# XuZhang1211/PVPUFormer

Hardware: AMD Instinct MI355X
Metric: 448x448 images/sec fwd+bwd, ViT-B VPUFormer (higher is better)
Workload: dtype bf16

## Files before the change

### include/vpu_hip.h

```cpp
#ifndef VPU_HIP_H
#define VPU_HIP_H
#include <stdint.h>

#ifdef __cplusplus
extern "C" {
#endif

#define VPU_BF16 0
#define VPU_F32 1

#define VPU_EPI_BIAS 1
#define VPU_EPI_PREACT 2
#define VPU_EPI_GELU 4
#define VPU_EPI_RELU 8
#define VPU_EPI_DGELU 16
#define VPU_EPI_DRELU 32
#define VPU_EPI_RESID 64
#define VPU_EPI_AFFINE 128
#define VPU_EPI_ACCUM 256
#define VPU_EPI_OUT_F32 512
#define VPU_EPI_SAVE_DGELU 1024
#define VPU_EPI_MULAUX 2048

typedef struct vpu_gemm_desc {
    const void* A;
    const void* B;
    void* C;
    const float* bias;
    const void* resid;
    const void* aux;
    void* preact;
    int32_t M, N, K;
    int32_t lda, ldb, ldc, ldr, ldaux;
    int32_t batch, inner;
    int64_t sAo, sAi, sBo, sBi, sCo, sCi, sRo, sRi;
    int32_t transA, transB;
    int32_t dtype, flags;
    int32_t resid_period;
    float alpha, post_mul, post_add;
    void* workspace;
    int64_t workspace_bytes;
    float* colsum;
    int32_t cs_tn, cs_t0;
    int64_t cs_ld;
} vpu_gemm_desc;

#define VPU_GEMM_GROUP_MAX 16
typedef struct vpu_gemm_group {
    int32_t n;
    int32_t start[VPU_GEMM_GROUP_MAX + 1];
    vpu_gemm_desc d[VPU_GEMM_GROUP_MAX];
} vpu_gemm_group;

const char* vpu_last_error(void);
int vpu_abi_version(void);

int vpu_gemm(const vpu_gemm_desc* d, void* stream);
int vpu_gemm_set_option(const char* name, int32_t value);
int vpu_gemm_get_option(const char* name, int32_t* value);
const char* vpu_gemm_last_kernel(void);
int vpu_gemm_grouped(const vpu_gemm_desc* d, int32_t n, void* stream);

int vpu_layernorm_fwd(const void* x, const float* w, const float* b, void* y, float* mean, float* rstd,
                      int64_t rows, int32_t C, float eps, int32_t dtype, void* stream);
int vpu_layernorm_bwd_nblk(int64_t rows);
int vpu_layernorm_bwd(const void* dy, const void* x, const float* w, const float* mean, const float* rstd,
                      const void* dres, void* dx, float* part, int64_t rows, int32_t C, int32_t dtype, void* stream);
int vpu_layernorm_fwd_pe(const void* x, const float* w, const float* b, void* y, float* mean, float* rstd,
                         int64_t rows, int32_t C, float eps, const void* pe, int64_t pe_rows, void* y2,
                         int32_t dtype, void* stream);
int vpu_layernorm_bwd2(const void* dy, const void* dy2, const void* x, const float* w, const float* mean,
                       const float* rstd, const void* dres, void* dx, float* part, int64_t rows, int32_t C,
                       int32_t dtype, void* stream);
#define VPU_COLSUM_BATCH_MAX 64
typedef struct vpu_colsum_job { const float* in; float* out; int32_t nrows, ncols, row_len, out_ld; } vpu_colsum_job;
typedef struct vpu_colsum_batch { vpu_colsum_job job[VPU_COLSUM_BATCH_MAX]; } vpu_colsum_batch;
int vpu_colsum_batched(const vpu_colsum_job* jobs, int32_t n, void* stream);
int vpu_colsum_f32(const float* in, float* out, int64_t rows, int32_t C, float beta, void* stream);
int vpu_colsum(const void* in, int32_t ld, float* out, float* part, int64_t rows, int32_t C, float beta,
               int32_t dtype, void* stream);
int vpu_softmax_fwd(const float* S, int32_t lds, void* P, int32_t ldp, int64_t rows, int32_t ncols,
                    int32_t dtype, void* stream);
int vpu_softmax_bwd(const void* P, int32_t ldp, const float* dP, int32_t lddp, void* dS, int64_t rows,
                    int32_t ncols, float scale, int32_t dtype, void* stream);
int vpu_l2norm_fwd(const void* x, void* y, float* inv, int64_t rows, int32_t C, int32_t dtype, void* stream);
int vpu_l2norm_bwd(const void* dy, const void* y, const float* inv, void* dx, int64_t rows, int32_t C,
                   int32_t dtype, void* stream);

int vpu_attn_fwd(const void* q, const void* k, const void* v, void* out, float* lse, int32_t nb, int32_t H, int32_t n,
                 int32_t hd, int32_t ld, int32_t ldo, float scale, void* stream);
int vpu_attn_bwd(const void* q, const void* k, const void* v, const void* o, const void* d_o, const float* lse,
                 float* delta, void* dq, void* dk, void* dv, int32_t nb, int32_t H, int32_t n, int32_t hd, int32_t ld,
                 int32_t ldo, int32_t ldg, float scale, void* stream);
int vpu_attn_set_option(const char* name, int32_t value);
const char* vpu_attn_last_kernel(void);
int vpu_xattn_fwd(const void* q, const void* k, const void* v, void* out, float* lse, int32_t nb, int32_t H, int32_t nq,
                  int32_t nk, int32_t hd, int32_t ldq, int32_t ldk, int32_t ldo, float scale, void* stream);
int vpu_xattn_bwd(const void* q, const void* k, const void* v, const void* o, const void* d_o, const float* lse,
                  float* delta, void* dq, void* dk, void* dv, int32_t nb, int32_t H, int32_t nq, int32_t nk, int32_t hd,
                  int32_t ldq, int32_t ldk, int32_t ldo, int32_t ldgq, int32_t ldgk, float scale, void* stream);
int vpu_xattn_fwd_split(const void* q, const void* k, const void* v, void* out, float* lse, int32_t nb, int32_t H, int32_t nq,
                        int32_t nk, int32_t hd, int32_t ldq, int32_t ldk, int32_t ldo, float scale, int32_t qdiv, int32_t kdiv,
                        void* stream);
int vpu_xattn_bwd_split(const void* q, const void* k, const void* v, const void* o, const void* d_o, const float* lse,
                        float* delta, void* dq, void* dk, void* dv, int32_t nb, int32_t H, int32_t nq, int32_t nk, int32_t hd,
                        int32_t ldq, int32_t ldk, int32_t ldo, int32_t ldgq, int32_t ldgk, float scale, int32_t qdiv, int32_t kdiv,
                        void* stream);
int vpu_attn_combine(const void* o_s, const float* lse_s, void* out, float* lse, int32_t nb, int32_t H, int32_t nq, int32_t hd,
                     int32_t S, int32_t ld_s, int32_t ldo, void* stream);
int vpu_sum_groups(const void* in, void* out, int64_t G, int32_t S, int64_t n, int32_t dtype, void* stream);

int vpu_add_bcast(const void* a, const void* b, void* out, int64_t n, int64_t period_b, int32_t dtype, void* stream);
int vpu_add4(const void* a, const void* b, const void* c, const void* d, void* out, int64_t n, int32_t dtype,
             void* stream);
int vpu_fanout_add(const void* src, void* const* dst, const int32_t* accum, int32_t ndst, int64_t n, int32_t dtype, void* stream);
int vpu_cast2d(const void* src, int32_t src_dtype, int64_t ld_src, void* dst, int32_t dst_dtype, int64_t ld_dst,
               int64_t rows, int32_t cols, int32_t cols_pad, void* stream);
typedef struct vpu_cast_job {
    const float* src;
    const float* src2;
    void* dst;
    int64_t ld_src, ld_dst, rows;
    int32_t cols, cols_pad, dst_dtype, perm_g, perm_wg;
} vpu_cast_job;
int vpu_cast2d_batched(const vpu_cast_job* jobs, int32_t n, void* stream);
int vpu_dropout_mask(float* out, int32_t n, float keep, uint64_t seed, uint64_t* state, void* stream);
int vpu_fill_f32(float* p, float v, int64_t n, void* stream);
int vpu_fill_ranges_f32(float* base, const int64_t* off, const int64_t* len, int32_t n, float v, void* stream);
int vpu_debug_spin(float* sink, int32_t wgs, int64_t cycles, void* stream);
int vpu_debug_gemm_times(void* dev_buf);
int vpu_sigmoid_to_channel(const float* logits, float* out, int32_t B, int64_t HW, int32_t channels, int32_t channel,
                           void* stream);
int vpu_act_bwd(const void* dy, int64_t ld_dy, const void* aux, int64_t ld_aux, void* dz, int64_t ld_dz, int64_t rows,
                int32_t cols, int32_t kind, int32_t dtype, void* stream);

int vpu_pue_encode(const float* points, const int32_t* boxes, const float* lut, void* out, double* out64,
                   int32_t B, int32_t n, int32_t num_max, int32_t img, int32_t ld, int32_t dtype, void* stream);
int vpu_pue_scribble_rows(const float* points, const double* vec, void* out, double* out64, int32_t B, int32_t n,
                          int32_t num_max, int32_t img, int32_t ld, int32_t dtype, void* stream);
int vpu_draw_polyline(const int32_t* curve, float* disks, int32_t B, int32_t P, int32_t H, int32_t W, void* stream);
int vpu_pue_encode_rows(const float* points, const int32_t* kinds, const int32_t* boxes, const double* vec, const float* lut,
                        void* out, double* out64, int32_t B, int32_t n, int32_t num_max, int32_t img, int32_t ld,
                        int32_t dtype, void* stream);
int vpu_draw_prompt_rows(const int32_t* kinds, const int32_t* boxes, const int32_t* curve, const int32_t* counts, float* disks,
                         int32_t B, int32_t Pmax, int32_t n, int32_t H, int32_t W, void* stream);
int vpu_edt(const uint8_t* mask, int32_t* scratch, float* dist, int32_t B, int32_t H, int32_t W, int32_t zero_border,
            void* stream);
int vpu_chamfer5(const uint8_t* mask, int32_t* scratch, float* dist, int32_t B, int32_t H, int32_t W, int32_t zero_border,
                 void* stream);
int vpu_mask_bbox(const float* prob, float thr, const int32_t* pos_clicks, int32_t nclicks, int32_t* out, int32_t B,
                  int32_t H, int32_t W, void* stream);
int vpu_error_masks(const uint8_t* pred, const uint8_t* gt, const uint8_t* valid, uint8_t* out, int32_t H, int32_t W,
                    void* stream);
int vpu_masked_argmax(const float* dist, const uint8_t* keep, uint64_t* out, int32_t planes, int32_t H, int32_t W,
                      void* stream);
typedef struct vpu_eval_obj {
    const float* image;
    const float* prev;
    float* canvas;
    uint8_t* mask;
    const uint8_t* gt;
    const uint8_t* valid;
    uint8_t* keep;
    int64_t* out;
    int32_t H, W, r0, r1, c0, c1, src, clear_at;
} vpu_eval_obj;
int vpu_roi_resize_batched(const vpu_eval_obj* objs, int32_t n, float* out, int32_t S_h, int32_t S_w, int32_t flip,
                           int32_t channels, void* stream);
int vpu_roi_paste_batched(const vpu_eval_obj* objs, int32_t n, const float* probs, int32_t S_h, int32_t S_w, float pred_thr,
                          float box_thr, int32_t max_hw, void* stream);
int vpu_click_keys_batched(const vpu_eval_obj* objs, int32_t n, uint8_t* err, int32_t* scratch, float* dist, int32_t Hm,
                           int32_t Wm, int32_t max_hw, void* stream);
typedef struct vpu_session_obj {
    float* canvas;
    uint64_t* bits;
    int32_t* rec;
    int32_t H, W, r0, r1, c0, c1, src, reserved;
} vpu_session_obj;
int vpu_session_paste_batched(const vpu_session_obj* objs, int32_t n, const float* probs, int32_t S_h, int32_t S_w,
                              float pred_thr, float box_thr, int32_t max_hw, int32_t form, void* stream);
typedef struct vpu_annot_obj {
    const float* add;
    float* total;
    uint16_t* labels;
    uint64_t* bits;
    int32_t* rec;
    int32_t H, W, label, mode;
} vpu_annot_obj;
int vpu_annot_compose_batched(const vpu_annot_obj* objs, int32_t n, float thr, int32_t max_hw, void* stream);
int vpu_label_extract(uint16_t* labels, float* out, int32_t* rec, int32_t H, int32_t W, int32_t label, void* stream);
typedef struct vpu_runs_obj {
    const void* src;
    int32_t H, W, kind;
    float thr;
} vpu_runs_obj;
#define VPU_RUNS_BAND_ROWS 64
#define VPU_RUNS_COLS 64
int vpu_runs_count_batched(const vpu_runs_obj* objs, const vpu_runs_obj* host_objs, int32_t n, int32_t* scratch,
                           int64_t scratch_len, int32_t* header, void* stream);
int vpu_runs_write_batched(const vpu_runs_obj* objs, const vpu_runs_obj* host_objs, int32_t n, const int32_t* scratch,
                           int64_t scratch_len, int32_t* entries, int32_t cap, void* stream);
typedef struct vpu_unrun_obj {
    void* dst;
    const int32_t* entries;
    int32_t H, W, n_runs, kind, label, pad;
} vpu_unrun_obj;
int vpu_runs_decode_batched(const vpu_unrun_obj* objs, const vpu_unrun_obj* host_objs, int32_t n, void* stream);
#define VPU_TIDY_ALL 0
#define VPU_TIDY_SEEDED 1
#define VPU_TIDY_LARGEST 2
#define VPU_TIDY_SCRATCH_INTS(hw) (3 * (int64_t)(hw) + 4)
// ... 141 lines not shown
```

### pvpuformer_amd/_lib.py

```python
import ctypes as C
import os

_HERE = os.path.dirname(os.path.abspath(__file__))
LIB_PATH = os.path.join(_HERE, os.environ.get("VPU_LIB_FILE") or
                        ("libvpu_hip_diag.so" if os.environ.get("VPU_LIB_DIAG", "0") == "1" else "libvpu_hip.so"))

BF16, F32 = 0, 1

EPI_BIAS, EPI_PREACT, EPI_GELU, EPI_RELU, EPI_DGELU, EPI_DRELU = 1, 2, 4, 8, 16, 32
EPI_RESID, EPI_AFFINE, EPI_ACCUM, EPI_OUT_F32 = 64, 128, 256, 512
EPI_SAVE_DGELU, EPI_MULAUX = 1024, 2048


class GemmDesc(C.Structure):
    _fields_ = [
        ("A", C.c_void_p), ("B", C.c_void_p), ("C", C.c_void_p), ("bias", C.c_void_p), ("resid", C.c_void_p),
        ("aux", C.c_void_p), ("preact", C.c_void_p),
        ("M", C.c_int32), ("N", C.c_int32), ("K", C.c_int32),
        ("lda", C.c_int32), ("ldb", C.c_int32), ("ldc", C.c_int32), ("ldr", C.c_int32), ("ldaux", C.c_int32),
        ("batch", C.c_int32), ("inner", C.c_int32),
        ("sAo", C.c_int64), ("sAi", C.c_int64), ("sBo", C.c_int64), ("sBi", C.c_int64),
        ("sCo", C.c_int64), ("sCi", C.c_int64), ("sRo", C.c_int64), ("sRi", C.c_int64),
        ("transA", C.c_int32), ("transB", C.c_int32), ("dtype", C.c_int32), ("flags", C.c_int32),
        ("resid_period", C.c_int32),
        ("alpha", C.c_float), ("post_mul", C.c_float), ("post_add", C.c_float),
        ("workspace", C.c_void_p), ("workspace_bytes", C.c_int64), ("colsum", C.c_void_p),
        ("cs_tn", C.c_int32), ("cs_t0", C.c_int32), ("cs_ld", C.c_int64),
    ]


_P, _I, _L, _F = C.c_void_p, C.c_int32, C.c_int64, C.c_float

class ColsumJob(C.Structure):
    _fields_ = [("inp", C.c_void_p), ("out", C.c_void_p), ("nrows", C.c_int32), ("ncols", C.c_int32),
                ("row_len", C.c_int32), ("out_ld", C.c_int32)]


class CastJob(C.Structure):
    _fields_ = [("src", C.c_void_p), ("src2", C.c_void_p), ("dst", C.c_void_p), ("ld_src", C.c_int64), ("ld_dst", C.c_int64),
                ("rows", C.c_int64), ("cols", C.c_int32), ("cols_pad", C.c_int32), ("dst_dtype", C.c_int32),
                ("perm_g", C.c_int32), ("perm_wg", C.c_int32)]


class EvalObj(C.Structure):
    _fields_ = [("image", C.c_void_p), ("prev", C.c_void_p), ("canvas", C.c_void_p), ("mask", C.c_void_p),
                ("gt", C.c_void_p), ("valid", C.c_void_p), ("keep", C.c_void_p), ("out", C.c_void_p),
                ("H", C.c_int32), ("W", C.c_int32), ("r0", C.c_int32), ("r1", C.c_int32), ("c0", C.c_int32),
                ("c1", C.c_int32), ("src", C.c_int32), ("clear_at", C.c_int32)]


class BoxRow(C.Structure):
    _fields_ = [("prev", C.c_void_p), ("gt", C.c_void_p), ("valid", C.c_void_p),
                ("H", C.c_int32), ("W", C.c_int32), ("r0", C.c_int32), ("r1", C.c_int32), ("c0", C.c_int32),
                ("c1", C.c_int32), ("mirror", C.c_int32), ("n_obj", C.c_int32)]


class SessionObj(C.Structure):
    _fields_ = [("canvas", C.c_void_p), ("bits", C.c_void_p), ("rec", C.c_void_p),
                ("H", C.c_int32), ("W", C.c_int32), ("r0", C.c_int32), ("r1", C.c_int32), ("c0", C.c_int32),
                ("c1", C.c_int32), ("src", C.c_int32), ("reserved", C.c_int32)]


class AnnotObj(C.Structure):
    _fields_ = [("add", C.c_void_p), ("total", C.c_void_p), ("labels", C.c_void_p), ("bits", C.c_void_p), ("rec", C.c_void_p),
                ("H", C.c_int32), ("W", C.c_int32), ("label", C.c_int32), ("mode", C.c_int32)]


class RunsObj(C.Structure):
    _fields_ = [("src", C.c_void_p), ("H", C.c_int32), ("W", C.c_int32), ("kind", C.c_int32), ("thr", C.c_float)]


class UnrunObj(C.Structure):
    _fields_ = [("dst", C.c_void_p), ("entries", C.c_void_p), ("H", C.c_int32), ("W", C.c_int32), ("n_runs", C.c_int32),
                ("kind", C.c_int32), ("label", C.c_int32), ("pad", C.c_int32)]


class OutlineObj(C.Structure):
    _fields_ = [("src", C.c_void_p), ("H", C.c_int32), ("W", C.c_int32), ("kind", C.c_int32), ("thr", C.c_float),
                ("label", C.c_int32), ("pad", C.c_int32)]


class TidyObj(C.Structure):
    _fields_ = [("add", C.c_void_p), ("total", C.c_void_p), ("add_out", C.c_void_p), ("total_out", C.c_void_p),
                ("bits", C.c_void_p), ("rec", C.c_void_p), ("seeds", C.c_void_p), ("scratch", C.c_void_p),
                ("H", C.c_int32), ("W", C.c_int32), ("n_seeds", C.c_int32), ("min_area", C.c_int32), ("max_hole", C.c_int32),
                ("keep", C.c_int32), ("pad0", C.c_int32), ("pad1", C.c_int32)]


SIGNATURES = {
    "vpu_gemm": [C.POINTER(GemmDesc), _P],
    "vpu_layernorm_fwd": [_P, _P, _P, _P, _P, _P, _L, _I, _F, _I, _P],
    "vpu_layernorm_bwd_nblk": [_L],
    "vpu_layernorm_bwd": [_P, _P, _P, _P, _P, _P, _P, _P, _L, _I, _I, _P],
    "vpu_layernorm_fwd_pe": [_P, _P, _P, _P, _P, _P, _L, _I, _F, _P, _L, _P, _I, _P],
    "vpu_layernorm_bwd2": [_P, _P, _P, _P, _P, _P, _P, _P, _P, _L, _I, _I, _P],
    "vpu_colsum_batched": [C.POINTER(ColsumJob), _I, _P],
    "vpu_colsum_f32": [_P, _P, _L, _I, _F, _P],
    "vpu_colsum": [_P, _I, _P, _P, _L, _I, _F, _I, _P],
    "vpu_softmax_fwd": [_P, _I, _P, _I, _L, _I, _I, _P],
    "vpu_softmax_bwd": [_P, _I, _P, _I, _P, _L, _I, _F, _I, _P],
    "vpu_l2norm_fwd": [_P, _P, _P, _L, _I, _I, _P],
    "vpu_l2norm_bwd": [_P, _P, _P, _P, _L, _I, _I, _P],
    "vpu_attn_fwd": [_P, _P, _P, _P, _P, _I, _I, _I, _I, _I, _I, _F, _P],
    "vpu_attn_bwd": [_P, _P, _P, _P, _P, _P, _P, _P, _P, _P, _I, _I, _I, _I, _I, _I, _I, _F, _P],
    "vpu_xattn_fwd": [_P, _P, _P, _P, _P, _I, _I, _I, _I, _I, _I, _I, _I, _F, _P],
    "vpu_xattn_bwd": [_P, _P, _P, _P, _P, _P, _P, _P, _P, _P, _I, _I, _I, _I, _I, _I, _I, _I, _I, _I, _F, _P],
    "vpu_xattn_fwd_split": [_P, _P, _P, _P, _P, _I, _I, _I, _I, _I, _I, _I, _I, _F, _I, _I, _P],
    "vpu_xattn_bwd_split": [_P, _P, _P, _P, _P, _P, _P, _P, _P, _P, _I, _I, _I, _I, _I, _I, _I, _I, _I, _I, _F, _I, _I, _P],
    "vpu_attn_combine": [_P, _P, _P, _P, _I, _I, _I, _I, _I, _I, _I, _P],
    "vpu_sum_groups": [_P, _P, _L, _I, _L, _I, _P],
    "vpu_add_bcast": [_P, _P, _P, _L, _L, _I, _P],
    "vpu_add4": [_P, _P, _P, _P, _P, _L, _I, _P],
    "vpu_cast2d": [_P, _I, _L, _P, _I, _L, _L, _I, _I, _P],
    "vpu_cast2d_batched": [C.POINTER(CastJob), _I, _P],
    "vpu_fanout_add": [_P, C.POINTER(C.c_void_p), C.POINTER(C.c_int32), _I, _L, _I, _P],
    "vpu_dropout_mask": [_P, _I, _F, C.c_uint64, _P, _P],
    "vpu_fill_f32": [_P, _F, _L, _P],
    "vpu_fill_ranges_f32": [_P, C.POINTER(C.c_int64), C.POINTER(C.c_int64), _I, _F, _P],
    "vpu_debug_spin": [_P, _I, _L, _P],
    "vpu_debug_gemm_times": [_P],
    "vpu_sigmoid_to_channel": [_P, _P, _I, _L, _I, _I, _P],
    "vpu_act_bwd": [_P, _L, _P, _L, _P, _L, _L, _I, _I, _I, _P],
    "vpu_pue_encode": [_P, _P, _P, _P, _P, _I, _I, _I, _I, _I, _I, _P],
    "vpu_cc_roots": [_P, _P, _I, _I, _I, _P],
    "vpu_cc_table": [_P, _P, _P, _I, _I, _I, _I, _P],
    "vpu_edt": [_P, _P, _P, _I, _I, _I, _I, _P],
    "vpu_chamfer5": [_P, _P, _P, _I, _I, _I, _I, _P],
    "vpu_pue_scribble_rows": [_P, _P, _P, _P, _I, _I, _I, _I, _I, _I, _P],
    "vpu_draw_polyline": [_P, _P, _I, _I, _I, _I, _P],
    "vpu_pue_encode_rows": [_P, _P, _P, _P, _P, _P, _P, _I, _I, _I, _I, _I, _I, _P],
    "vpu_draw_prompt_rows": [_P, _P, _P, _P, _P, _I, _I, _I, _I, _I, _P],
    "vpu_mask_bbox": [_P, _F, _P, _I, _P, _I, _I, _I, _P],
    "vpu_masked_argmax": [_P, _P, _P, _I, _I, _I, _P],
    "vpu_error_masks": [_P, _P, _P, _P, _I, _I, _P],
    "vpu_roi_resize_batched": [_P, _I, _P, _I, _I, _I, _I, _P],
    "vpu_roi_paste_batched": [_P, _I, _P, _I, _I, _F, _F, _I, _P],
    "vpu_session_paste_batched": [_P, _I, _P, _I, _I, _F, _F, _I, _I, _P],
    "vpu_annot_compose_batched": [_P, _I, _F, _I, _P],
    "vpu_label_extract": [_P, _P, _P, _I, _I, _I, _P],
    "vpu_runs_count_batched": [_P, _P, _I, _P, _L, _P, _P],
    "vpu_runs_write_batched": [_P, _P, _I, _P, _L, _P, _I, _P],
    "vpu_runs_decode_batched": [_P, _P, _I, _P],
    "vpu_regions_tidy_batched": [_P, _P, _I, _F, _P],
    "vpu_outline_count_batched": [_P, _P, _I, _P, _L, _P, _P],
    "vpu_outline_trace_batched": [_P, _P, _I, _P, _L, _P, _P, _P, _L, _P, _I, _P, _I, _P, _P],
    "vpu_outline_simplify_batched": [_P, _P, _P, _I, _I, _I, _I, _I, _P, _L, _P, _I, _P, _I, _P, _P, _P],
    "vpu_click_keys_batched": [_P, _I, _P, _P, _P, _I, _I, _I, _P],
    "vpu_box_prompts_batched": [_P, _I, _P, _I, _I, _I, _F, _P, _P, _P, _P, _P, _I, _P, _P, _P],
    "vpu_crops_gather": [_P, _P, _P, _P, _I, _I, _I, _I, _I, _I, _I, _P],
    "vpu_crops_blend": [_P, _P, _P, _P, _I, _I, _I, _I, _I, _I, _P],
    "vpu_disk_maps": [_P, _P, _P, _I, _I, _I, _I, _F, _P],
    "vpu_patch_im2col": [_P, _P, _P, _I, _I, _I, _I, _I, _I, _P],
    "vpu_patch_im2col_prenorm": [_P, _P, _P, _I, _I, _I, _I, _I, _I, _P],
    "vpu_patch_im2col_floor": [_P, _P, _P, _I, _I, _I, _I, _I, _I, _I, _P],
    "vpu_window_permute": [_P, _P, _I, _I, _I, _I, _I, _I, _P],
    "vpu_space_to_depth2_crop": [_P, _P, _I, _I, _I, _I, _I, _P],
    "vpu_pixel_shuffle2": [_P, _P, _P, _I, _I, _I, _I, _I, _I, _P],
    "vpu_pixel_shuffle2_gn_stats": [_P, _P, _P, _P, _I, _I, _I, _I, _I, _P],
    "vpu_groupnorm_apply": [_P, _P, _P, _P, _P, _P, _P, _I, _L, _I, _F, _I, _I, _P],
    "vpu_pixel_unshuffle2_nblk": [_I],
    "vpu_pixel_unshuffle2_sums": [_P, _P, _P, _I, _I, _I, _I, _I, _P],
    "vpu_groupnorm_nchunk": [],
    "vpu_groupnorm_fwd": [_P, _P, _P, _P, _P, _P, _P, _I, _L, _I, _F, _I, _I, _P],
    "vpu_groupnorm_bwd": [_P, _P, _P, _P, _P, _P, _P, _P, _P, _I, _L, _I, _I, _I, _P],
    "vpu_bilinear_cl_fwd": [_P, _I, _P, _I, _I, _I, _I, _I, _I, _I, _I, _P],
    "vpu_bilinear_cl_bwd": [_P, _I, _P, _I, _I, _I, _I, _I, _I, _I, _I, _P],
    "vpu_head_grad_fused": [_P, _P, _P, _P, _P, _P, _P, _P, _P, _P, _L, _L, _I, _I, _P],
    "vpu_upsum_relu": [_P, C.POINTER(C.c_void_p), C.POINTER(C.c_int32), C.POINTER(C.c_int32), _I, _I, _I, _I, _I, _I, _P],
    "vpu_gate_stats": [_P, _P, _P, _P, _P, _P, _I, _I, _I, _I, _I, _P],
    "vpu_gate_apply": [_P, _P, _P, _P, _I, _I, _I, _I, _P],
    "vpu_gate_bwd": [_P, _P, _P, _P, _P, _P, _P, _I, _P, _P, _P, _I, _I, _I, _I, _I, _P],
    "vpu_gate_fwd_n": [C.POINTER(C.c_void_p), C.POINTER(C.c_void_p), _P, C.POINTER(C.c_void_p), _P, _P, _P, _P, _I, _I, _I, _I, _I, _I, _P],
    "vpu_gate_bwd_n": [C.POINTER(C.c_void_p), _P, _P, _P, _P, _P, _P, _I, C.POINTER(C.c_void_p), C.POINTER(C.c_void_p), _P, _I, _I, _I,
                       _I, _I, _I, _P],
    "vpu_convseg_fwd": [_P, _P, _P, _P, _P, _L, _L, _I, _I, _P],
    "vpu_convseg_bwd_nblk": [_L],
    "vpu_convseg_bwd": [_P, _P, _P, _P, _P, _I, _P, _P, _L, _L, _I, _I, _P],
    "vpu_upsample_ac_fwd": [_P, _P, _L, _I, _I, _I, _I, _P],
    "vpu_upsample_ac_bwd": [_P, _P, _L, _I, _I, _I, _I, _P],
    "vpu_p2cl_fwd_bwd": [_P, _P, _P, _P, _P, _P, _F, _I, _I, _I, _I, _P],
    "vpu_p2cl_up_nband": [_I, _I],
    "vpu_p2cl_up_fwd_bwd": [_P, _P, _P, _P, _P, _P, _F, _I, _I, _I, _I, _I, _I, _P],
    "vpu_nfl_dice_scratch_doubles": [_I],
    "vpu_nfl_dice_fwd_bwd": [_P, _P, _P, _P, _P, _F, _F, _I, _L, _P],
    "vpu_loss_finalize": [_P, _P, _I, _I, C.c_double, _F, _F, _F, _F, _P, _P],
    "vpu_adam_step": [_P, _P, _P, _P, _P, _L, _F, _F, _F, _F, _F, _I, _F, _P],
    "vpu_adam_step_groups": [_P, _P, _P, _P, _P, _L, _P, _P, _P, _I, _F, _F, _F, _I, _I, _F, _P],
    "vpu_adam_step_hyper": [_P, _P, _P, _P, _P, _L, _P, _P, _P, _P, _I, _F, _F, _F, _F, _I, _P],
    "vpu_gemm_set_option": [C.c_char_p, _I],
    "vpu_gemm_get_option": [C.c_char_p, C.POINTER(C.c_int32)],
    "vpu_gemm_last_kernel": [],
    "vpu_attn_last_kernel": [],
    "vpu_attn_set_option": [C.c_char_p, _I],
    "vpu_gemm_grouped": [C.POINTER(GemmDesc), _I, _P],
    "vpu_last_error": [],
    "vpu_abi_version": [],
}
_RET = {"vpu_last_error": C.c_char_p, "vpu_gemm_last_kernel": C.c_char_p, "vpu_attn_last_kernel": C.c_char_p}

_lib = None

# ... 29 lines not shown
```

### pvpuformer_amd/csrc/gemm.hip

```cpp
#include <stdio.h>
#include <stdlib.h>
#include <string.h>
#include <atomic>
#include "vpu_common.h"
#include "../../include/vpu_hip.h"
#include "gemm_tiles.h"

int vpu_k5_option();
void vpu_k5_set_option(int v);
void vpu_k5_set_grid(int v);
void vpu_k5_set_split(int v);
void vpu_k5_set_noepi(int v);
int vpu_k5_launch(const vpu_gemm_desc* d, int rb, int ncu, int vec, void* stream, char* name, size_t name_len);
#ifdef VPU_DIAG
void vpu_k5_set_dbg(unsigned long long* p);
#endif

namespace {


template <typename T>
__device__ __forceinline__ void epilogue_store(const vpu_gemm_desc& p, int64_t coff, int64_t roff, int m, int n,
                                               float acc) {
    const int flags = p.flags;
// ... 417 lines not shown
    if (CS && TA == 1 && p.colsum != nullptr && tile_n == 0) {
        float* red = reinterpret_cast<float*>(lds);
        if (do_cs && fr == 0) {
#pragma unroll
            for (int i = 0; i < 4; ++i)
#pragma unroll
                for (int r = 0; r < 4; ++r) red[wm * 64 + i * 16 + fq * 4 + r] = acc_cs[i][r];
        }
        __syncthreads();
        if (tid < 128 && m0 + tid < p.M) {
            const float t = red[tid];
            if (splitk > 1) {
                float* cp = ws + (int64_t)nbatch * splitk * p.M * p.N + ((int64_t)z * splitk + split) * p.M + m0 + tid;
                if (SLAB && cnt) __hip_atomic_store(cp, t, __ATOMIC_RELAXED, __HIP_MEMORY_SCOPE_AGENT);
                else *cp = t;
            } else p.colsum[m0 + tid] += t;
        }
        __syncthreads();
    }
    const __amdgpu_buffer_rsrc_t rws = __builtin_amdgcn_make_buffer_rsrc(wsz, 0, 0x7FFFFFFF, 0x00020000);
#pragma unroll
    for (int pass = 0; pass < 2; ++pass) {
#pragma unroll
        for (int ii = 0; ii < 2; ++ii)
#pragma unroll
            for (int j = 0; j < 4; ++j)
#pragma unroll
                for (int r = 0; r < 4; ++r) {
                    const int row = ii * 16 + fq * 4 + r;
                    wl[row * 64 + ((j * 16 + fr) ^ (fq << 4))] = acc[pass * 2 + ii][j][r];
                }
        asm volatile("s_waitcnt lgkmcnt(0)" ::: "memory");
#pragma unroll
        for (int t = 0; t < 4; ++t) {
            const int u = lane + 64 * t;
            const int row = u >> 3, c8 = (u & 7) * 8;
            const int m = m0 + wm * 64 + pass * 32 + row;
            const int n = n0 + wn * 64 + c8;
            if (SLAB) {
                if (m < p.M && n < p.N) {
                    float v[8];
                    load8(wl + row * 64 + (c8 ^ (((row >> 2) & 3) << 4)), v);
                    if (cnt) store8_sc1(rws, (m * p.N + n) * 4, v);
                    else store8(wsz + (int64_t)m * p.N + n, v);
                }
            } else if (!GEN) {
                if (m < p.M && n < p.N) {
                    float v[8];
                    load8(wl + row * 64 + (c8 ^ (((row >> 2) & 3) << 4)), v);
                    EpiPre e;
                    e.has_pre = use_pre; e.has_bias = use_bias8; e.pre = pre[pass][t];
#pragma unroll
                    for (int j = 0; j < 8; ++j) e.bias[j] = bias8[j];
                    epilogue_store8(p, FLG, coff, roff, m, n, v, e);
                }
            } else if (m < p.M && n < p.N) {
                float v[8];
                load8(wl + row * 64 + (c8 ^ (((row >> 2) & 3) << 4)), v);
                if (splitk > 1) {
                    float* o = wsz + (int64_t)m * p.N + n;
                    if ((p.N & 3) == 0 && n + 8 <= p.N) store8(o, v);
                    else
                        for (int j = 0; j < 8 && n + j < p.N; ++j) o[j] = v[j];
                } else if (vec == 8) {
                    float tsum = 0.f;
#pragma unroll
                    for (int j = 0; j < 8; ++j) tsum += v[j];
                    if (tsum == 1.2345678e30f) reinterpret_cast<float*>(p.C)[0] = tsum;
                } else if (vec && n + 8 <= p.N) {
                    {
                        EpiPre e;
                        e.has_pre = use_pre; e.has_bias = use_bias8; e.pre = pre[pass][t];
#pragma unroll
                        for (int j = 0; j < 8; ++j) e.bias[j] = bias8[j];
                        epilogue_store8(p, FLG, coff, roff, m, n, v, e);
                    }
                } else {
                    for (int j = 0; j < 8 && n + j < p.N; ++j) epilogue_store<bf16_t>(p, coff, roff, m, n + j, v[j]);
                }
            }
        }
        asm volatile("s_waitcnt lgkmcnt(0)" ::: "memory");
    }
    if constexpr (SLAB) {
        if (cnt) {
            asm volatile("s_waitcnt vmcnt(0)" ::: "memory");
            __syncthreads();
            unsigned* flag = reinterpret_cast<unsigned*>(lds);
            unsigned* tc = cnt + (int64_t)z * ntiles + tile_lin;
            if (tid == 0) *flag = __hip_atomic_fetch_add(tc, 1u, __ATOMIC_RELAXED, __HIP_MEMORY_SCOPE_AGENT);
            __syncthreads();
            const bool last = *flag == (unsigned)(splitk - 1);
            if (last) {
                if (tid == 0) __hip_atomic_store(tc, 0u, __ATOMIC_RELAXED, __HIP_MEMORY_SCOPE_AGENT);
                __builtin_amdgcn_fence(__ATOMIC_ACQUIRE, "wavefront");
                const int64_t mn = (int64_t)p.M * p.N;
#pragma unroll
                for (int pass = 0; pass < 2; ++pass)
#pragma unroll
                    for (int t = 0; t < 4; ++t) {
                        const int u = lane + 64 * t;
                        const int row = u >> 3, c8 = (u & 7) * 8;
                        const int m = m0 + wm * 64 + pass * 32 + row;
                        const int n = n0 + wn * 64 + c8;
                        if (m < p.M && n < p.N) {
                            float v[8] = {0.f, 0.f, 0.f, 0.f, 0.f, 0.f, 0.f, 0.f};
                            for (int sl = 0; sl < splitk; ++sl) {
                                const unsigned long long* sp = reinterpret_cast<const unsigned long long*>(
                                    ws + ((int64_t)z * splitk + sl) * mn + (int64_t)m * p.N + n);
#pragma unroll
                                for (int j = 0; j < 4; ++j) {
                                    const unsigned long long q = __hip_atomic_load(sp + j, __ATOMIC_RELAXED, __HIP_MEMORY_SCOPE_AGENT);
                                    v[2 * j] += __builtin_bit_cast(float, (unsigned)(q & 0xFFFFFFFFull));
                                    v[2 * j + 1] += __builtin_bit_cast(float, (unsigned)(q >> 32));
                                }
                            }
                            if (vec) {
                                EpiPre e;
                                e.has_pre = false; e.has_bias = false; e.pre = make_uint4(0, 0, 0, 0);
                                epilogue_store8(p, p.flags, coff, roff, m, n, v, e);
                            } else {
                                for (int j = 0; j < 8; ++j) epilogue_store<bf16_t>(p, coff, roff, m, n + j, v[j]);
                            }
                        }
                    }
                if (CS && TA == 1 && p.colsum != nullptr && tile_n == 0 && tid < 128 && m0 + tid < p.M) {
                    const float* wb = ws + (int64_t)nbatch * splitk * mn + (int64_t)z * splitk * p.M + m0 + tid;
                    float t = 0.f;
                    for (int sl = 0; sl < splitk; ++sl)
                        t += __hip_atomic_load(wb + (int64_t)sl * p.M, __ATOMIC_RELAXED, __HIP_MEMORY_SCOPE_AGENT);
                    p.colsum[m0 + tid] += t;
                }
            }
            __syncthreads();
        }
    }
    __builtin_amdgcn_s_barrier();
    }
}

template <int TA, int TB, bool DMA, bool CS, int FL, int RING = 0>
__global__ __launch_bounds__(256, 2) void gemm_bf16_kernel(const vpu_gemm_desc p, const int tiles_n, const int splitk,
                                                        const int kchunk, float* __restrict__ ws, const int vec_in,
                                                        const int tiles_m_arg, const int nbatch,
                                                        unsigned* __restrict__ cnt) {
    gemm_bf16_body<TA, TB, DMA, CS, FL, RING, false>(p, nullptr, tiles_n, splitk, kchunk, ws, vec_in, tiles_m_arg, nbatch, cnt);
}
template <int TA, int TB, bool CS>
__global__ __launch_bounds__(256, 2) void gemm_bf16_grouped_kernel(const vpu_gemm_group ga, const int vec_in) {
    gemm_bf16_body<TA, TB, true, CS, -1, 0, true>(ga.d[0], &ga, 0, 1, 0, nullptr, vec_in, 0, 1, nullptr);
}

constexpr int BM2 = 256;
constexpr int STAGE2 = 3 * TILE_BYTES;

template <int TA, int TB>
__global__ __launch_bounds__(512) void gemm_bf16_big_kernel(const vpu_gemm_desc p, const int tiles_n, const int splitk,
                                                            const int kchunk, float* __restrict__ ws, const int vec) {
    extern __shared__ __attribute__((aligned(16))) char lds[];
    const int tid = threadIdx.x, lane = tid & 63;
    const int wave = __builtin_amdgcn_readfirstlane(tid >> 6);
    const int wm = wave >> 1, wn = wave & 1;
    int tile_m, tile_n;
    tile_coords(blockIdx.x, gridDim.x, tiles_n, tile_m, tile_n);
    const int m0 = tile_m * BM2, n0 = tile_n * BN;
    const int z = blockIdx.z, zo = z / p.inner, zi = z % p.inner;
    const bf16_t* A = reinterpret_cast<const bf16_t*>(p.A) + zo * p.sAo + zi * p.sAi;
    const bf16_t* B = reinterpret_cast<const bf16_t*>(p.B) + zo * p.sBo + zi * p.sBi;
    const int64_t coff = zo * p.sCo + zi * p.sCi;
    const int64_t roff = zo * p.sRo + zi * p.sRi;
    const int kbeg = blockIdx.y * kchunk;
    const int kend = (kbeg + kchunk < p.K) ? kbeg + kchunk : p.K;
    const __amdgpu_buffer_rsrc_t rA = __builtin_amdgcn_make_buffer_rsrc(const_cast<bf16_t*>(A), 0, 0x7FFFFFFF, 0x00020000);
    const __amdgpu_buffer_rsrc_t rB = __builtin_amdgcn_make_buffer_rsrc(const_cast<bf16_t*>(B), 0, 0x7FFFFFFF, 0x00020000);

    const int FLG = p.flags;
    const bool use_pre = false && vec == 1 && splitk == 1 &&
                         (p.flags & (VPU_EPI_RESID | VPU_EPI_MULAUX | VPU_EPI_DGELU | VPU_EPI_DRELU)) != 0 &&
                         !((p.flags & VPU_EPI_RESID) && (p.flags & (VPU_EPI_MULAUX | VPU_EPI_DGELU | VPU_EPI_DRELU)));
    uint4 pre[2][4];
    if (use_pre) prefetch_epi(p, FLG, coff, roff, m0 + wm * 64, n0 + wn * 64, lane, pre);

    f32x4_t acc[4][4];
#pragma unroll
    for (int i = 0; i < 4; ++i)
#pragma unroll
        for (int j = 0; j < 4; ++j) acc[i][j] = (f32x4_t){0.f, 0.f, 0.f, 0.f};
    const bool do_cs = TA == 1 && p.colsum != nullptr && tile_n == 0 && wn == 0;
    f32x4_t acc_cs[4];
#pragma unroll
    for (int i = 0; i < 4; ++i) acc_cs[i] = (f32x4_t){0.f, 0.f, 0.f, 0.f};
    bf16x8_t ones;
#pragma unroll
    for (int j = 0; j < 8; ++j) ones[j] = (bf16_t)(((lane & 15) == 0) ? 1.0f : 0.0f);

    auto issue = [&](int kt_, char* st) {
        const int k0 = kbeg + kt_ * BK;
#pragma unroll
        for (int i = 0; i < 6; ++i) {
            const int pc = wave + 8 * i;
            if (i < 4) stage_piece<TA>(rA, p.lda, m0 + (pc >> 4) * 128, p.M, k0, kend, st + (pc >> 4) * TILE_BYTES, pc & 15, lane);
            else stage_piece<TB>(rB, p.ldb, n0, p.N, k0, kend, st + 2 * TILE_BYTES, pc - 32, lane);
        }
    };
    const int nk = (kend - kbeg + BK - 1) / BK;
    char* s0 = lds;
    char* s1 = lds + STAGE2;
    char* s2 = lds + 2 * STAGE2;
    issue(0, s0);
    if (nk > 1) {
        issue(1, s1);
        asm volatile("s_waitcnt vmcnt(6)" ::: "memory");
    } else {
// ... 1388 lines not shown
    const int64_t coff = zo * p.sCo + zi * p.sCi;
    const int64_t roff = zo * p.sRo + zi * p.sRi;

    f32x4_t acc[2][2];
#pragma unroll
    for (int i = 0; i < 2; ++i)
#pragma unroll
        for (int j = 0; j < 2; ++j) acc[i][j] = (f32x4_t){0.f, 0.f, 0.f, 0.f};
    const int fr = lane & 15, fq = lane >> 4;
    const int nk = (p.K + FK - 1) / FK;
    for (int kt = 0; kt < nk; ++kt) {
        f32_stage<TA>(A, p.lda, m0, p.M, kt * FK, p.K, ldsA, tid);
        f32_stage<TB>(B, p.ldb, n0, p.N, kt * FK, p.K, ldsB, tid);
        __syncthreads();
#pragma unroll
        for (int ks = 0; ks < 4; ++ks) {
            const int k = ks * 4 + fq;
            float a[2], b[2];
#pragma unroll
            for (int i = 0; i < 2; ++i) a[i] = ldsA[k * FLD + wm * 32 + i * 16 + fr];
#pragma unroll
            for (int j = 0; j < 2; ++j) b[j] = ldsB[k * FLD + wn * 32 + j * 16 + fr];
#pragma unroll
            for (int i = 0; i < 2; ++i)
#pragma unroll
                for (int j = 0; j < 2; ++j)
                    acc[i][j] = __builtin_amdgcn_mfma_f32_16x16x4f32(a[i], b[j], acc[i][j], 0, 0, 0);
        }
        __syncthreads();
    }
#pragma unroll
    for (int i = 0; i < 2; ++i)
#pragma unroll
        for (int r = 0; r < 4; ++r) {
            const int m = m0 + wm * 32 + i * 16 + fq * 4 + r;
            if (m >= p.M) continue;
#pragma unroll
            for (int j = 0; j < 2; ++j) {
                const int n = n0 + wn * 32 + j * 16 + fr;
                if (n < p.N) epilogue_store<float>(p, coff, roff, m, n, acc[i][j][r]);
            }
        }
}

inline bool aligned_to(const void* p, size_t a) { return (reinterpret_cast<uintptr_t>(p) % a) == 0; }

thread_local char g_last_kernel[160] = "";
#define NOTE_KERNEL(...) snprintf(g_last_kernel, sizeof(g_last_kernel), __VA_ARGS__)
std::atomic<int> g_opt_ring{-1};
std::atomic<int> g_opt_inlaunch{-1};
std::atomic<int> g_opt_skinny{-1};
std::atomic<int> g_opt_skinny_group{-1};
std::atomic<int> g_opt_k2{-1};
std::atomic<int> g_opt_k3{-1};
inline int k3_env0() {
    static const int v = [] { const char* e = getenv("VPU_GEMM_K3"); return e ? atoi(e) : 28; }();
    return v;
}
inline int k3_opt() {
    int v = g_opt_k3.load(std::memory_order_relaxed);
    v = v >= 0 ? v : k3_env0();
#ifndef VPU_LAB
    v &= ~3;
    if (v & 8) v |= 16;
#endif
    return v;
}
inline int k2_env0() {
    static const int v = [] { const char* e = getenv("VPU_GEMM_K2"); return e ? atoi(e) : 2; }();
    return v;
}
inline int k2_opt() { const int v = g_opt_k2.load(std::memory_order_relaxed); return v >= 0 ? v : k2_env0(); }
std::atomic<int> g_opt_reserve{0};
#ifdef VPU_DIAG
std::atomic<unsigned long long*> g_dbg_times{nullptr};
#endif
inline int cu_count() {
    static const int v = [] { int dev = 0, n = 0; (void)hipGetDevice(&dev); (void)hipDeviceGetAttribute(&n, hipDeviceAttributeMultiprocessorCount, dev); return n > 0 ? n : 256; }();
    const int r = g_opt_reserve.load(std::memory_order_relaxed);
    const int left = (v - r) & ~7;
    return left >= 64 ? left : v;
}
inline int inlaunch_env0() {
    static const int v = [] { const char* e = vpu_lab_getenv("VPU_GEMM_INLAUNCH"); return e ? atoi(e) : 0; }();
    return v;
}
constexpr int64_t CNT_BYTES = 256 << 10;
inline int ring_env0() {
    static const int v = [] { const char* e = vpu_lab_getenv("VPU_GEMM_RING"); return e ? atoi(e) : 0; }();
    return v;
}

}

extern "C" int vpu_gemm(const vpu_gemm_desc* d, void* stream) {
    vpu_clear_stale_error();
    if (!d || !d->A || !d->B || !d->C) { vpu_set_error("vpu_gemm: null operand"); return VPU_ERR_ARG; }
    if (d->M <= 0 || d->N <= 0 || d->K <= 0 || d->batch <= 0 || d->inner <= 0 || d->batch % d->inner) {
        vpu_set_error("vpu_gemm: bad sizes (M,N,K,batch > 0; batch % inner == 0)");
        return VPU_ERR_ARG;
    }
    if (d->colsum && d->cs_tn > 1) {
        vpu_set_error("vpu_gemm: cs_tn > 1 (distributed column sums) is a vpu_gemm_grouped form");
        return VPU_ERR_ARG;
    }
    const int f = d->flags;
    if (((f & VPU_EPI_BIAS) && !d->bias) || ((f & VPU_EPI_RESID) && !d->resid) ||
        ((f & (VPU_EPI_DGELU | VPU_EPI_DRELU | VPU_EPI_MULAUX)) && !d->aux) ||
        ((f & (VPU_EPI_PREACT | VPU_EPI_SAVE_DGELU)) && !d->preact) ||
        ((f & VPU_EPI_SAVE_DGELU) && (!(f & VPU_EPI_GELU) || (f & VPU_EPI_PREACT)))) {
        vpu_set_error("vpu_gemm: epilogue flag set but its pointer is null");
        return VPU_ERR_ARG;
    }
    const bool bf = d->dtype == VPU_BF16;
    if (!bf && d->dtype != VPU_F32) { vpu_set_error("vpu_gemm: dtype"); return VPU_ERR_ARG; }
    if (d->colsum && (!bf || !d->transA || d->batch != 1)) {
        vpu_set_error("vpu_gemm: colsum needs the bf16 path, transA=1 and batch=1");
        return VPU_ERR_ARG;
    }
    const int64_t q = bf ? 8 : 4;
    const bool strides_ok = d->lda % q == 0 && d->ldb % q == 0 && d->sAo % q == 0 && d->sAi % q == 0 &&
                            d->sBo % q == 0 && d->sBi % q == 0;
    if (!strides_ok || !aligned_to(d->A, 16) || !aligned_to(d->B, 16)) {
        vpu_set_error("vpu_gemm: A/B base, leading dimensions and batch strides must be 16-byte multiples");
        return VPU_ERR_ALIGN;
    }
    if (bf) {
        const int64_t ea = d->transA ? (int64_t)d->K * d->lda : (int64_t)d->M * d->lda;
        const int64_t eb = d->transB ? (int64_t)d->K * d->ldb : (int64_t)d->N * d->ldb;
        if (ea * 2 >= 0x7FFFFFF0LL || eb * 2 >= 0x7FFFFFF0LL) {
            vpu_set_error("vpu_gemm: an operand spans more than 2 GiB per batch entry");
            return VPU_ERR_ARG;
        }
    }
    hipStream_t s = reinterpret_cast<hipStream_t>(stream);
    static const int force_big = [] { const char* e = vpu_lab_getenv("VPU_GEMM_BIG"); return e ? (e[0] == '1' ? 1 : 0) : -1; }();
#ifdef VPU_LAB
    const bool big = bf && force_big == 1 && d->M >= 1024 && d->N >= 128 && d->K >= 256;
#else
    const bool big = false;
    (void)force_big;
#endif
    const int tm = bf ? (big ? BM2 : BM) : FM, tn = bf ? BN : FN;
    const int tiles_m = (d->M + tm - 1) / tm, tiles_n = (d->N + tn - 1) / tn;
    const int key = (d->transA ? 2 : 0) | (d->transB ? 1 : 0);
    if (bf) {
        const size_t cbytes = (f & VPU_EPI_OUT_F32) ? 32 : 16;
        bool vec = d->ldc % 8 == 0 && d->sCo % 8 == 0 && d->sCi % 8 == 0 && aligned_to(d->C, cbytes);
        if (f & VPU_EPI_BIAS) vec = vec && aligned_to(d->bias, 32);
        if (f & (VPU_EPI_PREACT | VPU_EPI_SAVE_DGELU)) vec = vec && aligned_to(d->preact, 16);
        if (f & (VPU_EPI_DGELU | VPU_EPI_DRELU | VPU_EPI_MULAUX)) vec = vec && d->ldaux % 8 == 0 && aligned_to(d->aux, 16);
        if (f & VPU_EPI_RESID)
            vec = vec && d->ldr % 8 == 0 && d->sRo % 8 == 0 && d->sRi % 8 == 0 && aligned_to(d->resid, 16);
        const int64_t tiles = (int64_t)tiles_m * tiles_n * d->batch;
        int splitk = 1, kchunk = (d->K + BK - 1) / BK * BK;
        const int ring_env = g_opt_ring.load(std::memory_order_relaxed) >= 0 ? g_opt_ring.load(std::memory_order_relaxed) : ring_env0();
        static const int ring_min = [] { const char* e = vpu_lab_getenv("VPU_GEMM_RING_MIN"); return e ? atoi(e) : 96; }();
#ifdef VPU_LAB
        const bool ring = !big && (ring_env == 2 || (ring_env == 1 && tiles >= ring_min && tiles <= 256 && d->K <= 24 * BK && d->K > 2 * BK));
#else
        const bool ring = false;
        (void)ring_env; (void)ring_min;
#endif
        if (!ring && d->workspace && (tiles < 192 || (tiles <= 256 && d->K >= 32 * BK)) && d->K >= 8 * BK) {
            int64_t want = (384 + tiles - 1) / tiles;
            const int64_t max_by_k = d->K / (4 * BK);
            const int64_t max_by_ws = (d->workspace_bytes - CNT_BYTES) / ((int64_t)d->batch * d->M * (d->N + 1) * 4);
// ... 121 lines not shown
        else if (rb_ == 7) VPU_LAUNCH_K2_RB(TA_, TB_, 2, FL_, 7);                                                     \
        else VPU_LAUNCH_K2_RB(TA_, TB_, 2, FL_, 8);                                                                   \
    } while (0)
#define VPU_K2_BOTH(TA_, TB_, FL_) do { if (wide) VPU_LAUNCH_K2(TA_, TB_, 4, FL_); else if (narrow_ok) VPU_LAUNCH_K2N(TA_, TB_, FL_); else done = false; } while (0)
                {
                    const int k5 = vpu_k5_option();
                    if (k5 > 0 && (k2 == 2 || k5 == 2) && d->K >= 9 * BK && !((f & VPU_EPI_RESID) && d->resid_period > 0)) {
                        int rb5 = 8;
                        int64_t best5 = cost(256, 128);
                        for (int rb = 7; rb >= 6; --rb) {
                            const int64_t c5 = cost(32 * rb, 128);
                            if (c5 < best5) { best5 = c5; rb5 = rb; }
                        }
                        const bool gelu5 = (f & VPU_EPI_GELU) != 0 && d->M > 6272;
                        if (k5 == 2 || !gelu5) {
                            const int r5 = vpu_k5_launch(d, rb5, ncu, vec2, stream, g_last_kernel, sizeof(g_last_kernel));
                            if (r5 < 0) return r5;
                            if (r5 == 1) return vpu_check_launch("vpu_gemm");
                        }
                    }
                }
                if (key == 0 && f == F_B) VPU_K2_BOTH(0, 0, F_B);
                else if (key == 0 && f == F_BR) VPU_K2_BOTH(0, 0, F_BR);
                else if (key == 0 && f == F_G) VPU_K2_BOTH(0, 0, F_G);
                else if (key == 0 && f == 0) VPU_K2_BOTH(0, 0, 0);
                else if (key == 1 && f == 0) VPU_K2_BOTH(0, 1, 0);
                else if (key == 1 && f == F_M) VPU_K2_BOTH(0, 1, F_M);
                else done = false;
#undef VPU_K2_BOTH
#undef VPU_LAUNCH_K2N
#undef VPU_LAUNCH_K2
#undef VPU_LAUNCH_K2_RB
#undef VPU_LAUNCH_K2_SW
                if (done) return vpu_check_launch("vpu_gemm");
            }
        }
        static const int skinny_env = [] { const char* e = vpu_lab_getenv("VPU_GEMM_SKINNY"); return e ? atoi(e) : 1; }();
        const int skinny_opt = g_opt_skinny.load(std::memory_order_relaxed) >= 0 ? g_opt_skinny.load(std::memory_order_relaxed) : skinny_env;
        static const int skinny_m = [] { const char* e = vpu_lab_getenv("VPU_GEMM_SKINNY_M"); return e ? atoi(e) : 4096; }();
        static const int skinny_n = [] { const char* e = vpu_lab_getenv("VPU_GEMM_SKINNY_N"); return e ? atoi(e) : 4096; }();
        static const int skinny_k = [] { const char* e = vpu_lab_getenv("VPU_GEMM_SKINNY_K"); return e ? atoi(e) : 4096; }();
        if (skinny_opt && !big && !d->transA && d->batch == 1 && !d->colsum && d->M <= skinny_m && d->N <= skinny_n &&
            d->K >= 64 && d->K <= skinny_k && (int64_t)tiles_m * tiles_n < 192) {
            const int tn64 = (d->N + SK_T - 1) / SK_T, tm64 = (d->M + SK_T - 1) / SK_T;
            const int kw = (int)(((d->K + 3) / 4 + 63) / 64 * 64);
            static VpuDevOnce attr_sk;
            if (auto todo_ = attr_sk.pending()) {
                VPU_SET_LDS(4 * TILE_BYTES, gemm_bf16_skinny_kernel<0>);
                VPU_SET_LDS(8 * TILE_BYTES, gemm_bf16_skinny_kernel<1>);
            }
            dim3 sgrid((unsigned)(tm64 * tn64)), sblock(256);
            NOTE_KERNEL("gemm_bf16_skinny_kernel<%d>", d->transB ? 1 : 0);
            if (d->transB) gemm_bf16_skinny_kernel<1><<<sgrid, sblock, 8 * TILE_BYTES, s>>>(*d, tn64, kw, vec ? 1 : 0);
            else gemm_bf16_skinny_kernel<0><<<sgrid, sblock, 4 * TILE_BYTES, s>>>(*d, tn64, kw, vec ? 1 : 0);
            return vpu_check_launch("vpu_gemm");
        }
        static const bool noepi = [] { const char* e = vpu_lab_getenv("VPU_GEMM_NOEPI"); return e && e[0] == '1'; }();
        static const bool nostore = [] { const char* e = vpu_lab_getenv("VPU_GEMM_NOSTORE"); return e && e[0] == '1'; }();
        static const int stagger = [] { const char* e = vpu_lab_getenv("VPU_GEMM_STAGGER"); return e ? atoi(e) : 0; }();
        const int vec_arg = (noepi ? 9 : (nostore ? 8 : (vec ? 1 : 0))) | (stagger << 8);
        float* ws = splitk > 1 ? reinterpret_cast<float*>(d->workspace) : nullptr;
        dim3 grid((unsigned)(tiles_m * tiles_n), (unsigned)splitk, (unsigned)d->batch), block(256);
        const int64_t total_work = (int64_t)tiles_m * tiles_n * splitk * d->batch;
        static const int persist_env = [] { const char* e = vpu_lab_getenv("VPU_GEMM_PERSIST"); return e ? atoi(e) : 0; }();
        const int persist_cap = persist_env > 0 ? persist_env : 2 * cu_count();
        dim3 pgrid((unsigned)(total_work < persist_cap ? total_work : persist_cap), 1, 1);
        static const int force_dma = [] { const char* e = vpu_lab_getenv("VPU_GEMM_DMA"); return e ? (e[0] == '1' ? 1 : 0) : -1; }();
        const bool use_dma = force_dma != 0;
#define VPU_LAUNCH(TA_, TB_)                                                                                         \
    do {                                                                                                             \
        NOTE_KERNEL("gemm_bf16_kernel<%d, %d, %s, false, -1, 0>", TA_, TB_, use_dma ? "true" : "false");              \
        if (use_dma) gemm_bf16_kernel<TA_, TB_, true, false, -1><<<pgrid, block, 4 * TILE_BYTES, s>>>(*d, tiles_n, splitk, kchunk, ws, vec_arg, tiles_m, d->batch, cnt_arg); \
        else gemm_bf16_kernel<TA_, TB_, false, false, -1><<<pgrid, block, 2 * TILE_BYTES, s>>>(*d, tiles_n, splitk, kchunk, ws, vec_arg, tiles_m, d->batch, cnt_arg);       \
    } while (0)
#define VPU_LAUNCH_FL(TA_, TB_, FL_)                                                                  \
    do {                                                                                              \
        NOTE_KERNEL("gemm_bf16_kernel<%d, %d, true, false, %d, 0>", TA_, TB_, FL_);                    \
        gemm_bf16_kernel<TA_, TB_, true, false, FL_><<<pgrid, block, 4 * TILE_BYTES, s>>>(*d, tiles_n, splitk, kchunk, ws, vec_arg, tiles_m, d->batch, cnt_arg); \
    } while (0)
        static const bool no_spec = [] { const char* e = vpu_lab_getenv("VPU_GEMM_GENERIC"); return e && e[0] == '1'; }();
        const bool spec_ok = use_dma && !no_spec && !big && !d->colsum && vec && splitk == 1 && d->N % 8 == 0 && (vec_arg & 255) == 1;
        bool launched = false, inlaunch = false;
        unsigned* cnt_arg = nullptr;
#define VPU_LAUNCH_RING(TA_, TB_, CS_, FL_)                                                                            \
    do {                                                                                                             \
        static VpuDevOnce attr_;                                                                                   \
        auto kern_ = gemm_bf16_kernel<TA_, TB_, true, CS_, FL_, 3>;                                                   \
        if (auto todo_ = attr_.pending()) {                                                                                                \
            VPU_SET_LDS(6 * TILE_BYTES, kern_); \
        }                                                                                                            \
        NOTE_KERNEL("gemm_bf16_kernel<%d, %d, true, %s, %d, 3>", TA_, TB_, CS_ ? "true" : "false", FL_);              \
        kern_<<<pgrid, block, 6 * TILE_BYTES, s>>>(*d, tiles_n, splitk, kchunk, ws, vec_arg, tiles_m, d->batch, cnt_arg);       \
    } while (0)
#ifdef VPU_LAB
        if (ring && use_dma && vec_arg <= 1) {
            launched = true;
            if (d->colsum && key == 3) VPU_LAUNCH_RING(1, 1, true, -1);
            else if (d->colsum) launched = false;
            else if (key == 0) VPU_LAUNCH_RING(0, 0, false, -1);
            else if (key == 1) VPU_LAUNCH_RING(0, 1, false, -1);
            else if (key == 2) VPU_LAUNCH_RING(1, 0, false, -1);
            else VPU_LAUNCH_RING(1, 1, false, -1);
        }
#endif
#undef VPU_LAUNCH_RING
        if (!launched && spec_ok && (k3_opt() & 4) && (d->K <= 384 || (k3_opt() & 32)) && d->batch == 1 && d->K % K3_BK == 0 && d->K >= 128 && d->alpha == 1.0f &&
            (int64_t)d->M * d->ldc * 2 < 0x7FFFFFF0LL && (int64_t)d->M * (d->ldr > d->ldaux ? d->ldr : d->ldaux) * 2 < 0x7FFFFFF0LL) {
            constexpr int F_B = VPU_EPI_BIAS, F_BR = VPU_EPI_BIAS | VPU_EPI_RESID, F_BL = VPU_EPI_BIAS | VPU_EPI_RELU,
                          F_G = VPU_EPI_BIAS | VPU_EPI_GELU | VPU_EPI_SAVE_DGELU, F_M = VPU_EPI_MULAUX, F_D = VPU_EPI_DRELU;
            const int cap3s = 3 * cu_count();
            const int tot3s = tiles_m * tiles_n;
            launched = true;
            vpu_gemm_desc dacc = *d;
            const bool acc_as_res = key == 1 && f == VPU_EPI_ACCUM && d->dtype == VPU_BF16 && !d->resid;
            if (acc_as_res) {
                dacc.flags = VPU_EPI_RESID; dacc.resid = d->C; dacc.ldr = d->ldc; dacc.resid_period = 0;
                dacc.sRo = d->sCo; dacc.sRi = d->sCi;
            }
            const vpu_gemm_desc* dk = acc_as_res ? &dacc : d;
#define VPU_LAUNCH_K3S(TA_, TB_, FL_)                                                                                \
    do {                                                                                                             \
        static VpuDevOnce attr_;                                                                                   \
        auto kern_ = gemm_bf16_k3s_kernel<TA_, TB_, FL_>;                                                             \
        if (auto todo_ = attr_.pending()) {                                                                                                \
            VPU_SET_LDS((K3Cfg<2, 128>::LDS), kern_); \
        }                                                                                                            \
        NOTE_KERNEL("gemm_bf16_k3s_kernel<%d, %d, %d>", TA_, TB_, FL_);                                                \
        kern_<<<dim3((unsigned)(tot3s < cap3s ? tot3s : cap3s)), dim3(256), K3Cfg<2, 128>::LDS, s>>>(*dk, tiles_m, tiles_n, 1); \
    } while (0)
            if (key == 0 && f == F_B) VPU_LAUNCH_K3S(0, 0, F_B);
            else if (key == 0 && f == F_BR) VPU_LAUNCH_K3S(0, 0, F_BR);
            else if (key == 0 && f == F_G) VPU_LAUNCH_K3S(0, 0, F_G);
            else if (key == 0 && f == F_BL) VPU_LAUNCH_K3S(0, 0, F_BL);
            else if (key == 0 && f == 0) VPU_LAUNCH_K3S(0, 0, 0);
            else if (key == 1 && f == F_D) VPU_LAUNCH_K3S(0, 1, F_D);
            else if (key == 1 && f == 0) VPU_LAUNCH_K3S(0, 1, 0);
            else if (key == 1 && f == F_M) VPU_LAUNCH_K3S(0, 1, F_M);
            else if (acc_as_res) VPU_LAUNCH_K3S(0, 1, VPU_EPI_RESID);
            else launched = false;
#undef VPU_LAUNCH_K3S
        }
        if (!launched && spec_ok) {
            launched = true;
            constexpr int F_B = VPU_EPI_BIAS, F_BR = VPU_EPI_BIAS | VPU_EPI_RESID,
                          F_G = VPU_EPI_BIAS | VPU_EPI_GELU | VPU_EPI_SAVE_DGELU, F_M = VPU_EPI_MULAUX;
            if (key == 0 && f == F_B) VPU_LAUNCH_FL(0, 0, F_B);
            else if (key == 0 && f == F_BR) VPU_LAUNCH_FL(0, 0, F_BR);
            else if (key == 0 && f == F_G) VPU_LAUNCH_FL(0, 0, F_G);
            else if (key == 0 && f == (VPU_EPI_BIAS | VPU_EPI_RELU)) VPU_LAUNCH_FL(0, 0, VPU_EPI_BIAS | VPU_EPI_RELU);
            else if (key == 0 && f == 0) VPU_LAUNCH_FL(0, 0, 0);
            else if (key == 1 && f == VPU_EPI_DRELU) VPU_LAUNCH_FL(0, 1, VPU_EPI_DRELU);
            else if (key == 1 && f == 0) VPU_LAUNCH_FL(0, 1, 0);
            else if (key == 1 && f == F_M) VPU_LAUNCH_FL(0, 1, F_M);
            else if (key == 1 && f == VPU_EPI_ACCUM) VPU_LAUNCH_FL(0, 1, VPU_EPI_ACCUM);
            else launched = false;
        }
        const bool slab_ok = use_dma && !no_spec && !big && splitk > 1 && d->N % 8 == 0 && vec_arg <= 1;
        if (!launched && slab_ok) {
            launched = true;
            const int inl = g_opt_inlaunch.load(std::memory_order_relaxed) >= 0 ? g_opt_inlaunch.load(std::memory_order_relaxed) : inlaunch_env0();
            const int64_t slab_bytes = (int64_t)d->batch * splitk * d->M * d->N * 4;
            if (inl && (inl == 1 || slab_bytes <= ((int64_t)inl << 20)) && tiles <= CNT_BYTES / 4 &&
                (int64_t)d->M * d->N * 4 < 0x7FFFFFF0LL && d->workspace_bytes > 2 * CNT_BYTES) {
                cnt_arg = reinterpret_cast<unsigned*>(reinterpret_cast<char*>(d->workspace) + d->workspace_bytes - CNT_BYTES);
                inlaunch = true;
            }
            if (d->colsum && key == 3) NOTE_KERNEL("gemm_bf16_kernel<1, 1, true, true, 65536, 0>");
            if (d->colsum && key == 3) gemm_bf16_kernel<1, 1, true, true, FL_SLAB><<<pgrid, block, 4 * TILE_BYTES, s>>>(*d, tiles_n, splitk, kchunk, ws, vec_arg, tiles_m, d->batch, cnt_arg);
            else if (d->colsum) launched = false;
            else if (key == 3) VPU_LAUNCH_FL(1, 1, FL_SLAB);
            else if (key == 0) VPU_LAUNCH_FL(0, 0, FL_SLAB);
            else if (key == 1) VPU_LAUNCH_FL(0, 1, FL_SLAB);
            else launched = false;
            if (!launched) { inlaunch = false; cnt_arg = nullptr; }
        }
        if (launched) {
        } else
#ifdef VPU_LAB
        if (big) {
            static VpuDevOnce attr_done;
            if (auto todo_ = attr_done.pending()) {
                const int sz = 3 * STAGE2;
                VPU_SET_LDS(sz, gemm_bf16_big_kernel<0, 0>);
                VPU_SET_LDS(sz, gemm_bf16_big_kernel<0, 1>);
                VPU_SET_LDS(sz, gemm_bf16_big_kernel<1, 0>);
                VPU_SET_LDS(sz, gemm_bf16_big_kernel<1, 1>);
            }
            dim3 block2(512);
            NOTE_KERNEL("gemm_bf16_big_kernel<%d, %d>", key >> 1, key & 1);
            switch (key) {
                case 0: gemm_bf16_big_kernel<0, 0><<<grid, block2, 3 * STAGE2, s>>>(*d, tiles_n, splitk, kchunk, ws, vec_arg); break;
                case 1: gemm_bf16_big_kernel<0, 1><<<grid, block2, 3 * STAGE2, s>>>(*d, tiles_n, splitk, kchunk, ws, vec_arg); break;
                case 2: gemm_bf16_big_kernel<1, 0><<<grid, block2, 3 * STAGE2, s>>>(*d, tiles_n, splitk, kchunk, ws, vec_arg); break;
                default: gemm_bf16_big_kernel<1, 1><<<grid, block2, 3 * STAGE2, s>>>(*d, tiles_n, splitk, kchunk, ws, vec_arg); break;
            }
        } else
#endif
        {
            if (d->colsum) {
                NOTE_KERNEL("gemm_bf16_kernel<1, %d, true, true, -1, 0>", key == 3 ? 1 : 0);
                if (key == 3) gemm_bf16_kernel<1, 1, true, true, -1><<<pgrid, block, 4 * TILE_BYTES, s>>>(*d, tiles_n, splitk, kchunk, ws, vec_arg, tiles_m, d->batch, cnt_arg);
                else gemm_bf16_kernel<1, 0, true, true, -1><<<pgrid, block, 4 * TILE_BYTES, s>>>(*d, tiles_n, splitk, kchunk, ws, vec_arg, tiles_m, d->batch, cnt_arg);
            } else
            switch (key) {
                case 0: VPU_LAUNCH(0, 0); break;
                case 1: VPU_LAUNCH(0, 1); break;
                case 2: VPU_LAUNCH(1, 0); break;
                default: VPU_LAUNCH(1, 1); break;
            }
        }
#undef VPU_LAUNCH
#undef VPU_LAUNCH_FL
        if (splitk > 1 && !inlaunch) {
            const int64_t mn = (int64_t)d->M * d->N;
            int vec8 = vec && d->N % 8 == 0 ? 1 : 0;
            if (vec8 && splitk >= 16 && mn / 8 <= 8 * 65535) vec8 = 2;
            dim3 rgrid((unsigned)(vec8 == 2 ? (mn / 8 + 7) / 8 : vpu_grid_for(vec8 ? mn / 8 : mn, 256, 4096)), 1,
                       (unsigned)d->batch);
            splitk_reduce_kernel<bf16_t><<<rgrid, block, 0, s>>>(*d, splitk, ws, vec8);
        }
    } else {
        dim3 grid((unsigned)(tiles_m * tiles_n), 1, (unsigned)d->batch), block(256);
        NOTE_KERNEL("gemm_f32_kernel<%d, %d>", key >> 1, key & 1);
        switch (key) {
            case 0: gemm_f32_kernel<0, 0><<<grid, block, 0, s>>>(*d, tiles_n); break;
            case 1: gemm_f32_kernel<0, 1><<<grid, block, 0, s>>>(*d, tiles_n); break;
            case 2: gemm_f32_kernel<1, 0><<<grid, block, 0, s>>>(*d, tiles_n); break;
            default: gemm_f32_kernel<1, 1><<<grid, block, 0, s>>>(*d, tiles_n); break;
        }
    }
    return vpu_check_launch("vpu_gemm");
}

extern "C" const char* vpu_gemm_last_kernel(void) { return g_last_kernel; }

extern "C" int vpu_gemm_set_option(const char* name, int32_t value) {
    vpu_clear_stale_error();
#ifndef VPU_LAB
    if (name && ((!strcmp(name, "ring") && value > 0) || (!strcmp(name, "k3") && value > 0 && (value & 3)))) {
        vpu_set_error("vpu_gemm_set_option: the three-stage ring forms and the K3 forward / grouped forms (k3 bits 0-1) are compiled "
                      "into the laboratory library only (build.sh diag, VPU_LIB_DIAG=1)");
        return VPU_ERR_ARG;
    }
#endif
    if (name && !strcmp(name, "ring") && value >= -1 && value <= 2) {
        g_opt_ring.store(value, std::memory_order_relaxed);
        return VPU_OK;
    }
    if (name && !strcmp(name, "skinny") && value >= -1 && value <= 1) {
        g_opt_skinny.store(value, std::memory_order_relaxed);
        return VPU_OK;
    }
    if (name && !strcmp(name, "k2") && value >= -1 && value <= 3) {
        g_opt_k2.store(value, std::memory_order_relaxed);
        return VPU_OK;
    }
    if (name && !strcmp(name, "k3") && value >= -1 && value <= 63) {
// ... 308 lines not shown
```

### pvpuformer_amd/csrc/rowops.hip

```cpp
#include <stdlib.h>
#include "vpu_common.h"
#include "../../include/vpu_hip.h"

#define DISPATCH_T(dtype, ...)                                   \
    if ((dtype) == VPU_BF16) { using T = bf16_t; __VA_ARGS__ }   \
    else if ((dtype) == VPU_F32) { using T = float; __VA_ARGS__ } \
    else { vpu_set_error("bad dtype"); return VPU_ERR_ARG; }

namespace {

constexpr int LN_MAXCH = 4;
constexpr int LN_BWD_WAVES = 8;

template <typename T, int NCH, bool PE, int RW>
__global__ __launch_bounds__(256) void layernorm_fwd_kernel(const T* __restrict__ x, const float* __restrict__ w,
                                                            const float* __restrict__ b, T* __restrict__ y,
                                                            float* __restrict__ mean, float* __restrict__ rstd,
                                                            int64_t rows, int C, float eps, const T* __restrict__ pe,
                                                            int64_t pe_rows, T* __restrict__ y2) {
    const int lane = threadIdx.x & 63;
    const int64_t half = (int64_t)gridDim.x * 4, stride = half * RW;
    int64_t row0 = (int64_t)blockIdx.x * 4 + (threadIdx.x >> 6);
    if (row0 >= rows) return;
    float ww[NCH][8], bb[NCH][8];
// ... 6 lines not shown
#pragma unroll
            for (int k = 0; k < RW; ++k)
                if (row0 + k * half < rows) cur[k][i].load(x + (row0 + k * half) * C + c);
        }
    }
    for (; row0 < rows; row0 += stride) {
        const int64_t nr = row0 + stride;
#pragma unroll
        for (int k = 0; k < RW; ++k)
            if (nr + k * half < rows) {
#pragma unroll
                for (int i = 0; i < NCH; ++i) {
                    const int c = (lane + i * 64) * 8;
                    if (c < C) nxt[k][i].load(x + (nr + k * half) * C + c);
                }
            }
        float v[RW][NCH][8];
        float s[RW], q[RW], mu[RW], rs[RW];
#pragma unroll
        for (int k = 0; k < RW; ++k) {
            s[k] = 0.f;
            if (row0 + k * half < rows) {
#pragma unroll
                for (int i = 0; i < NCH; ++i) {
                    const int c = (lane + i * 64) * 8;
                    if (c < C) {
                        cur[k][i].get(v[k][i]);
#pragma unroll
                        for (int j = 0; j < 8; ++j) s[k] += v[k][i][j];
                    }
                }
            }
        }
#pragma unroll
        for (int k = 0; k < RW; ++k) mu[k] = wave_sum(s[k]) / C;
#pragma unroll
        for (int k = 0; k < RW; ++k) {
            q[k] = 0.f;
            if (row0 + k * half < rows) {
#pragma unroll
                for (int i = 0; i < NCH; ++i) {
                    const int c = (lane + i * 64) * 8;
                    if (c < C) {
#pragma unroll
                        for (int j = 0; j < 8; ++j) { const float d = v[k][i][j] - mu[k]; q[k] += d * d; }
                    }
                }
            }
        }
#pragma unroll
        for (int k = 0; k < RW; ++k) rs[k] = rsqrtf(wave_sum(q[k]) / C + eps);
#pragma unroll
        for (int k = 0; k < RW; ++k) {
            const int64_t row = row0 + k * half;
            if (row < rows) {
                if (lane == 0) { mean[row] = mu[k]; rstd[row] = rs[k]; }
                T* yr = y + row * C;
#pragma unroll
                for (int i = 0; i < NCH; ++i) {
                    const int c = (lane + i * 64) * 8;
                    if (c < C) {
                        float o[8];
#pragma unroll
                        for (int j = 0; j < 8; ++j) o[j] = (v[k][i][j] - mu[k]) * rs[k] * ww[i][j] + bb[i][j];
                        store8(yr + c, o);
                        if (PE) {
                            float pv[8];
                            load8(pe + (row % pe_rows) * C + c, pv);
#pragma unroll
                            for (int j = 0; j < 8; ++j) o[j] = to_f32(from_f32<T>(o[j])) + pv[j];
                            store8(y2 + row * C + c, o);
                        }
                    }
                }
            }
        }
#pragma unroll
        for (int k = 0; k < RW; ++k)
#pragma unroll
            for (int i = 0; i < NCH; ++i) cur[k][i] = nxt[k][i];
    }
}

template <typename T, int NCH, int NW, bool PF, bool D2, int RW>
__global__ __launch_bounds__(64 * NW) void layernorm_bwd_kernel(const T* __restrict__ dy, const T* __restrict__ dy2,
                                                            const T* __restrict__ x,
                                                            const float* __restrict__ w,
                                                            const float* __restrict__ mean,
                                                            const float* __restrict__ rstd, const T* __restrict__ dres,
                                                            T* __restrict__ dx, float* __restrict__ part, int64_t rows,
                                                            int C, int nblk) {
    __shared__ float red[NW][8 * 64];
    const int lane = threadIdx.x & 63, wave = threadIdx.x >> 6;
    float dwa[NCH][8], dba[NCH][8];
#pragma unroll
    for (int i = 0; i < NCH; ++i)
#pragma unroll
        for (int j = 0; j < 8; ++j) { dwa[i][j] = 0.f; dba[i][j] = 0.f; }
    float ww[NCH][8];
#pragma unroll
    for (int i = 0; i < NCH; ++i) {
        const int c = (lane + i * 64) * 8;
        if (c < C) load8(w + c, ww[i]);
    }
    const int64_t half = (int64_t)nblk * NW, stride = half * RW;
    int64_t row0 = (int64_t)blockIdx.x * NW + wave;
    Raw8<T> cx[RW][NCH], cd[RW][NCH], cr[RW][NCH], nx[RW][NCH], nd[RW][NCH], nres[RW][NCH];
    Raw8<T> cd2[RW][D2 ? NCH : 1], nd2[RW][D2 ? NCH : 1];
    float mu[RW], rs[RW], nmu[RW], nrs[RW];
#pragma unroll
    for (int k = 0; k < RW; ++k) { mu[k] = 0.f; rs[k] = 0.f; nmu[k] = 0.f; nrs[k] = 0.f; }
    auto request = [&](int64_t r0, Raw8<T> (&ox)[RW][NCH], Raw8<T> (&od)[RW][NCH], Raw8<T> (&orr)[RW][NCH],
                       Raw8<T> (&od2)[RW][D2 ? NCH : 1], float (&om)[RW], float (&os)[RW]) {
#pragma unroll
        for (int k = 0; k < RW; ++k) {
            const int64_t r = r0 + k * half;
            if (r < rows) {
                om[k] = mean[r]; os[k] = rstd[r];
#pragma unroll
                for (int i = 0; i < NCH; ++i) {
                    const int c = (lane + i * 64) * 8;
                    if (c < C) {
                        ox[k][i].load(x + r * C + c);
                        od[k][i].load(dy + r * C + c);
                        if (D2) od2[k][i].load(dy2 + r * C + c);
                        if (dres) orr[k][i].load(dres + r * C + c);
                    }
                }
            }
        }
    };
    if (PF && row0 < rows) request(row0, cx, cd, cr, cd2, mu, rs);
    for (; row0 < rows; row0 += stride) {
        if (PF && row0 + stride < rows) request(row0 + stride, nx, nd, nres, nd2, nmu, nrs);
        if (!PF) request(row0, cx, cd, cr, cd2, mu, rs);
        float s1[RW], s2[RW];
#pragma unroll
        for (int k = 0; k < RW; ++k) {
            s1[k] = 0.f; s2[k] = 0.f;
            if (row0 + k * half < rows) {
#pragma unroll
                for (int i = 0; i < NCH; ++i) {
                    const int c = (lane + i * 64) * 8;
                    if (c < C) {
                        float xv[8], dv[8];
                        cx[k][i].get(xv);
                        cd[k][i].get(dv);
                        if (D2) {
                            float d2[8];
                            cd2[k][i].get(d2);
#pragma unroll
                            for (int j = 0; j < 8; ++j) dv[j] += d2[j];
                        }
#pragma unroll
                        for (int j = 0; j < 8; ++j) {
                            const float xh = (xv[j] - mu[k]) * rs[k], g = dv[j] * ww[i][j];
                            s1[k] += g;
                            s2[k] += g * xh;
                            dwa[i][j] += dv[j] * xh;
                            dba[i][j] += dv[j];
                        }
                    }
                }
            }
        }
#pragma unroll
        for (int k = 0; k < RW; ++k) { s1[k] = wave_sum(s1[k]) / C; s2[k] = wave_sum(s2[k]) / C; }
#pragma unroll
        for (int k = 0; k < RW; ++k) {
            const int64_t row = row0 + k * half;
            if (row < rows) {
#pragma unroll
                for (int i = 0; i < NCH; ++i) {
                    const int c = (lane + i * 64) * 8;
                    if (c < C) {
                        float o[8], xv[8], dv[8];
                        if (dres) cr[k][i].get(o);
                        else {
#pragma unroll
                            for (int j = 0; j < 8; ++j) o[j] = 0.f;
                        }
                        cx[k][i].get(xv);
                        cd[k][i].get(dv);
                        if (D2) {
                            float d2[8];
                            cd2[k][i].get(d2);
#pragma unroll
                            for (int j = 0; j < 8; ++j) dv[j] += d2[j];
                        }
#pragma unroll
                        for (int j = 0; j < 8; ++j) {
                            const float xh = (xv[j] - mu[k]) * rs[k], g = dv[j] * ww[i][j];
                            o[j] += rs[k] * (g - s1[k] - xh * s2[k]);
                        }
                        store8(dx + row * C + c, o);
                    }
                }
            }
        }
        if (PF) {
#pragma unroll
            for (int k = 0; k < RW; ++k) {
                mu[k] = nmu[k]; rs[k] = nrs[k];
#pragma unroll
                for (int i = 0; i < NCH; ++i) {
                    cx[k][i] = nx[k][i]; cd[k][i] = nd[k][i]; cr[k][i] = nres[k][i];
                    if (D2) cd2[k][i] = nd2[k][i];
                }
            }
        }
    }
#pragma unroll
    for (int which = 0; which < 2; ++which) {
#pragma unroll
        for (int i = 0; i < NCH; ++i) {
            const int c = (lane + i * 64) * 8;
            __syncthreads();
#pragma unroll
            for (int j = 0; j < 8; ++j) red[wave][j * 64 + lane] = which ? dba[i][j] : dwa[i][j];
            __syncthreads();
            if (wave == 0 && c < C) {
                float o[8];
#pragma unroll
                for (int j = 0; j < 8; ++j) {
                    float t = 0.f;
#pragma unroll
                    for (int w_ = 0; w_ < NW; ++w_) t += red[w_][j * 64 + lane];
                    o[j] = t;
                }
                store8(part + ((int64_t)blockIdx.x * 2 + which) * C + c, o);
            }
        }
    }
}

__global__ __launch_bounds__(256) void colsum_f32_kernel(const float* __restrict__ in, float* __restrict__ out,
                                                         int64_t rows, int C, float beta) {
    __shared__ float red[8][33];
    const int cl = threadIdx.x & 31, grp = threadIdx.x >> 5;
    const int c = blockIdx.x * 32 + cl;
    float s0 = 0.f, s1 = 0.f;
    if (c < C) {
        int64_t r = grp;
        for (; r + 8 < rows; r += 16) { s0 += in[r * C + c]; s1 += in[(r + 8) * C + c]; }
        if (r < rows) s0 += in[r * C + c];
    }
    red[grp][cl] = s0 + s1;
    __syncthreads();
    if (grp == 0 && c < C) {
        float t = 0.f;
#pragma unroll
        for (int g = 0; g < 8; ++g) t += red[g][cl];
        out[c] = (beta != 0.f ? beta * out[c] : 0.f) + t;
    }
}

__global__ __launch_bounds__(256) void colsum_batched_kernel(const vpu_colsum_batch jb) {
    __shared__ float red[8][33];
    const vpu_colsum_job& j = jb.job[blockIdx.y];
    const int cl = threadIdx.x & 31, grp = threadIdx.x >> 5;
    const int C = j.ncols;
    const int64_t rows = j.nrows;
    const float* __restrict__ in = j.in;
    if (rows <= 16 && (C & 3) == 0 && !(j.row_len > 0 && ((j.row_len | j.out_ld) & 3)) &&
        ((reinterpret_cast<uintptr_t>(in) | reinterpret_cast<uintptr_t>(j.out)) & 15) == 0) {
        const int C4 = C >> 2;
        const int rl = j.row_len;
        for (int c4 = blockIdx.x * 256 + threadIdx.x; c4 < C4; c4 += gridDim.x * 256) {
            const int64_t c = 4 * (int64_t)c4;
            float* o = j.out + (rl > 0 ? (c / rl) * j.out_ld + c % rl : c);
            f32x4_t a = *reinterpret_cast<const f32x4_t*>(o);
            for (int64_t r = 0; r < rows; ++r) a += *reinterpret_cast<const f32x4_t*>(in + r * C + c);
            *reinterpret_cast<f32x4_t*>(o) = a;
        }
        return;
    }
    for (int c0 = blockIdx.x * 32; c0 < C; c0 += gridDim.x * 32) {
        const int c = c0 + cl;
// ... 301 lines not shown
    const float* src2;
    void* dst;
    long long ld_src, ld_dst, rows;
    int cols, cols_pad, dst_dtype, perm_g, perm_wg;
};
struct CastBatch { CastJob j[CAST_MAXJ]; };
__global__ __launch_bounds__(256) void cast2d_batched_kernel(const CastBatch b) {
    const CastJob& q = b.j[blockIdx.y];
    const int64_t total = q.rows * q.cols_pad;
    for (int64_t i = (int64_t)blockIdx.x * 256 + threadIdx.x; i < total; i += (int64_t)gridDim.x * 256) {
        const int64_t r = i / q.cols_pad;
        const int c = (int)(i - r * q.cols_pad);
        float v = 0.f;
        if (c < q.cols) {
            v = q.src[r * q.ld_src + c];
            if (q.src2) v += q.src2[r * q.ld_src + c];
        }
        int64_t ro = r;
        if (q.perm_g > 0) {
            const int g = q.perm_g, wg = q.perm_wg, nw = g / wg, t = (int)r, ty = t / g, tx = t % g;
            ro = ((ty / wg) * nw + tx / wg) * wg * wg + (ty % wg) * wg + tx % wg;
        }
        if (q.dst_dtype == VPU_BF16) reinterpret_cast<bf16_t*>(q.dst)[ro * q.ld_dst + c] = (bf16_t)v;
        else reinterpret_cast<float*>(q.dst)[ro * q.ld_dst + c] = v;
    }
}
template <typename T>
__global__ __launch_bounds__(256) void act_bwd_kernel(const T* __restrict__ dy, int64_t ld_dy, const T* __restrict__ aux,
                                                      int64_t ld_aux, T* __restrict__ dz, int64_t ld_dz, int64_t rows,
                                                      int cols, int kind) {
    const int chunks = cols / 8;
    const int64_t total = rows * chunks;
    for (int64_t i = (int64_t)blockIdx.x * 256 + threadIdx.x; i < total; i += (int64_t)gridDim.x * 256) {
        const int64_t r = i / chunks;
        const int c = (int)(i - r * chunks) * 8;
        float d[8], a[8];
        load8(dy + r * ld_dy + c, d);
        load8(aux + r * ld_aux + c, a);
#pragma unroll
        for (int j = 0; j < 8; ++j) d[j] *= kind ? dgelu_f(a[j]) : (a[j] > 0.f ? 1.f : 0.f);
        store8(dz + r * ld_dz + c, d);
    }
}
__global__ __launch_bounds__(256) void sigmoid_to_channel_kernel(const float* __restrict__ logits, float* __restrict__ out,
                                                                 int64_t HW, int64_t batch_stride, int64_t ch_off,
                                                                 int64_t total) {
    for (int64_t i = (int64_t)blockIdx.x * 256 + threadIdx.x; i < total; i += (int64_t)gridDim.x * 256) {
        const int64_t b = i / HW, r = i - b * HW;
        out[b * batch_stride + ch_off + r] = 1.0f / (1.0f + expf(-logits[i]));
    }
}
__global__ __launch_bounds__(256) void dropout_mask_kernel(float* __restrict__ out, int n, float keep, float inv_keep,
                                                           unsigned long long seed, unsigned long long* __restrict__ state) {
    const unsigned long long call = state[0];
    seed ^= state[1];
    __syncthreads();
    if (threadIdx.x == 0) state[0] = call + 1;
    for (int i = threadIdx.x; i < n; i += 256) {
        unsigned long long x = seed + call * 0x9E3779B97F4A7C15ULL + (unsigned long long)(i + 1) * 0xD1B54A32D192ED03ULL;
        x ^= x >> 30; x *= 0xBF58476D1CE4E5B9ULL;
        x ^= x >> 27; x *= 0x94D049BB133111EBULL;
        x ^= x >> 31;
        const float u = (float)(x >> 40) * (1.0f / 16777216.0f);
        out[i] = u < keep ? inv_keep : 0.f;
    }
}
__global__ __launch_bounds__(256) void fill_kernel(float* p, float v, int64_t n) {
    const int64_t head = ((16 - (reinterpret_cast<uintptr_t>(p) & 15)) & 15) >> 2;
    const int64_t h = head < n ? head : n, n4 = (n - h) >> 2;
    float4* q = reinterpret_cast<float4*>(p + h);
    const float4 v4 = make_float4(v, v, v, v);
    const int64_t tid = (int64_t)blockIdx.x * 256 + threadIdx.x, nth = (int64_t)gridDim.x * 256;
    for (int64_t i = tid; i < n4; i += nth) q[i] = v4;
    if (tid < h) p[tid] = v;
    const int64_t tail = h + 4 * n4;
    if (tail + tid < n) p[tail + tid] = v;
}

constexpr int FILL_MAX_RANGES = 160;
constexpr int FILL_CHUNK = 16384;
struct FillRanges {
    int n;
    int first_chunk[FILL_MAX_RANGES + 1];
    long long off[FILL_MAX_RANGES], len[FILL_MAX_RANGES];
};
__global__ __launch_bounds__(256) void fill_ranges_kernel(float* __restrict__ base, const FillRanges r, const float v) {
    const int c = blockIdx.x;
    int lo = 0, hi = r.n;
    while (hi - lo > 1) {
        const int mid = (lo + hi) >> 1;
        if (r.first_chunk[mid] <= c) lo = mid; else hi = mid;
    }
    const long long start = (long long)(c - r.first_chunk[lo]) * FILL_CHUNK;
    const long long end = start + FILL_CHUNK < r.len[lo] ? start + FILL_CHUNK : r.len[lo];
    float4* q = reinterpret_cast<float4*>(base + r.off[lo]);
    const float4 v4 = make_float4(v, v, v, v);
    for (long long i = (start >> 2) + threadIdx.x; i < (end >> 2); i += 256) q[i] = v4;
}

}

#define ST reinterpret_cast<hipStream_t>(stream)

extern "C" int vpu_layernorm_fwd_pe(const void* x, const float* w, const float* b, void* y, float* mean, float* rstd,
                                    int64_t rows, int32_t C, float eps, const void* pe, int64_t pe_rows, void* y2,
                                    int32_t dtype, void* stream) {
    vpu_clear_stale_error();
    if (C % 8 || C > LN_MAXCH * 512 || rows <= 0) { vpu_set_error("layernorm: C % 8 == 0, C <= 2048"); return VPU_ERR_ARG; }
    if ((pe != nullptr) != (y2 != nullptr) || (pe && pe_rows <= 0)) {
        vpu_set_error("layernorm_fwd_pe: pe, pe_rows > 0 and y2 go together");
        return VPU_ERR_ARG;
    }
    static const int64_t capf = [] { const char* e = vpu_lab_getenv("VPU_LN_FWD_CAP"); const int v = e ? atoi(e) : 2048; return (int64_t)(v < 256 ? 256 : v); }();
    static const int rwf = [] { const char* e = vpu_lab_getenv("VPU_LN_FWD_RW"); return e ? atoi(e) : 1; }();
    const int rw = (rwf == 2 && C <= 1024 && dtype == VPU_BF16 && !pe && rows >= 4096) ? 2 : 1;
    const int64_t nb = (rows + 4 * rw - 1) / (4 * rw), trips = (nb + capf - 1) / capf;
    const unsigned grid = (unsigned)((nb + trips - 1) / trips);
#define VPU_LN_FWD_(NCH_, RW_)                                                                                        \
    if (pe) { DISPATCH_T(dtype, (layernorm_fwd_kernel<T, NCH_, true, RW_><<<grid, 256, 0, ST>>>((const T*)x, w, b, (T*)y, mean, rstd, rows, C, eps, (const T*)pe, pe_rows, (T*)y2));) } \
    else { DISPATCH_T(dtype, (layernorm_fwd_kernel<T, NCH_, false, RW_><<<grid, 256, 0, ST>>>((const T*)x, w, b, (T*)y, mean, rstd, rows, C, eps, (const T*)nullptr, 1, (T*)nullptr));) }
#define VPU_LN_FWD(NCH_) if (rw == 2) { VPU_LN_FWD_(NCH_, 2) } else { VPU_LN_FWD_(NCH_, 1) }
    if (C <= 512) { VPU_LN_FWD(1) } else if (C <= 1024) { VPU_LN_FWD(2) } else { VPU_LN_FWD_(4, 1) }
#undef VPU_LN_FWD
#undef VPU_LN_FWD_
    return vpu_check_launch("vpu_layernorm_fwd");
}
extern "C" int vpu_layernorm_fwd(const void* x, const float* w, const float* b, void* y, float* mean, float* rstd,
                                 int64_t rows, int32_t C, float eps, int32_t dtype, void* stream) {
    return vpu_layernorm_fwd_pe(x, w, b, y, mean, rstd, rows, C, eps, nullptr, 0, nullptr, dtype, stream);
}
extern "C" int vpu_layernorm_bwd_nblk(int64_t rows) {
    vpu_clear_stale_error();
    int64_t n = rows / (2 * LN_BWD_WAVES);
    static const int cap = [] { const char* e = vpu_lab_getenv("VPU_LN_BWD_WGS"); const int v = e ? atoi(e) : 2; return 256 * (v < 1 ? 1 : (v > 4 ? 4 : v)); }();
    return (int)(n < 1 ? 1 : (n > cap ? cap : n));
}
extern "C" int vpu_layernorm_bwd2(const void* dy, const void* dy2, const void* x, const float* w, const float* mean,
                                  const float* rstd, const void* dres, void* dx, float* part, int64_t rows, int32_t C,
                                  int32_t dtype, void* stream) {
    vpu_clear_stale_error();
    if (C % 8 || C > LN_MAXCH * 512 || rows <= 0) { vpu_set_error("layernorm_bwd: C"); return VPU_ERR_ARG; }
    const int nblk = vpu_layernorm_bwd_nblk(rows);
    static const int rw2 = [] { const char* e = vpu_lab_getenv("VPU_LN_BWD_RW"); return e ? atoi(e) : 2; }();
#define VPU_LN_BWD_(NCH_, NW_, RW_)                                                                                   \
    if (dy2) { DISPATCH_T(dtype, (layernorm_bwd_kernel<T, NCH_, NW_, (NCH_ <= 2), true, RW_><<<nblk, 64 * NW_, 0, ST>>>(   \
                          (const T*)dy, (const T*)dy2, (const T*)x, w, mean, rstd, (const T*)dres, (T*)dx, part, rows, C, nblk));) } \
    else { DISPATCH_T(dtype, (layernorm_bwd_kernel<T, NCH_, NW_, (NCH_ <= 2), false, RW_><<<nblk, 64 * NW_, 0, ST>>>(      \
                          (const T*)dy, (const T*)nullptr, (const T*)x, w, mean, rstd, (const T*)dres, (T*)dx, part, rows, C, nblk));) }
#define VPU_LN_BWD(NCH_, NW_)                                                                                         \
    if (NCH_ <= 2 && rw2 == 2 && dtype == VPU_BF16 && !dy2) { VPU_LN_BWD_(NCH_, NW_, 2) } else { VPU_LN_BWD_(NCH_, NW_, 1) }
    if (C <= 512) { VPU_LN_BWD(1, 4) } else if (C <= 1024) { VPU_LN_BWD(2, 4) } else { VPU_LN_BWD(4, 8) }
#undef VPU_LN_BWD
#undef VPU_LN_BWD_
    return vpu_check_launch("vpu_layernorm_bwd");
}
extern "C" int vpu_layernorm_bwd(const void* dy, const void* x, const float* w, const float* mean, const float* rstd,
                                 const void* dres, void* dx, float* part, int64_t rows, int32_t C, int32_t dtype,
                                 void* stream) {
    return vpu_layernorm_bwd2(dy, nullptr, x, w, mean, rstd, dres, dx, part, rows, C, dtype, stream);
}
extern "C" int vpu_colsum_f32(const float* in, float* out, int64_t rows, int32_t C, float beta, void* stream) {
    vpu_clear_stale_error();
    colsum_f32_kernel<<<(C + 31) / 32, 256, 0, ST>>>(in, out, rows, C, beta);
    return vpu_check_launch("vpu_colsum_f32");
}
extern "C" int vpu_colsum_batched(const vpu_colsum_job* jobs, int32_t n, void* stream) {
    vpu_clear_stale_error();
    if (!jobs || n < 1 || n > VPU_COLSUM_BATCH_MAX) { vpu_set_error("colsum_batched: 1 <= n <= VPU_COLSUM_BATCH_MAX"); return VPU_ERR_ARG; }
    vpu_colsum_batch jb;
    int cmax = 0;
    for (int i = 0; i < n; ++i) {
        if (!jobs[i].in || !jobs[i].out || jobs[i].nrows < 1 || jobs[i].ncols < 1) {
            vpu_set_error("colsum_batched: null pointer or empty job");
            return VPU_ERR_ARG;
        }
        if (jobs[i].row_len < 0 || (jobs[i].row_len > 0 && (jobs[i].ncols % jobs[i].row_len || jobs[i].out_ld < jobs[i].row_len))) {
            vpu_set_error("colsum_batched: row_len must divide ncols and out_ld >= row_len");
            return VPU_ERR_ARG;
        }
        jb.job[i] = jobs[i];
        const bool few = jobs[i].nrows <= 16 && (jobs[i].ncols & 3) == 0 && !(jobs[i].row_len > 0 && ((jobs[i].row_len | jobs[i].out_ld) & 3)) &&
                         ((reinterpret_cast<uintptr_t>(jobs[i].in) | reinterpret_cast<uintptr_t>(jobs[i].out)) & 15) == 0;
        const int need = few ? (jobs[i].ncols + 1023) / 1024 : (jobs[i].ncols + 31) / 32;
        cmax = need > cmax ? need : cmax;
    }
    dim3 grid(cmax, n);
    colsum_batched_kernel<<<grid, 256, 0, ST>>>(jb);
    return vpu_check_launch("vpu_colsum_batched");
}
extern "C" int vpu_colsum(const void* in, int32_t ld, float* out, float* part, int64_t rows, int32_t C, float beta,
                          int32_t dtype, void* stream) {
    vpu_clear_stale_error();
    if (C % 8 || ld % 8) { vpu_set_error("colsum: C, ld % 8"); return VPU_ERR_ARG; }
    if (rows <= 64) {
        const unsigned g = (unsigned)((C / 8 + 255) / 256);
        DISPATCH_T(dtype, colsum_small_kernel<T><<<g, 256, 0, ST>>>((const T*)in, ld, out, (int)rows, C, beta);)
        return vpu_check_launch("vpu_colsum");
    }
    if (C <= 128) {
        dim3 grid((C + 31) / 32, CS_SLABS);
        DISPATCH_T(dtype, colsum_part_kernel<T, 4><<<grid, 256, 0, ST>>>((const T*)in, ld, part, rows, C);)
    } else if (C <= 256) {
        dim3 grid((C + 63) / 64, CS_SLABS);
        DISPATCH_T(dtype, colsum_part_kernel<T, 8><<<grid, 256, 0, ST>>>((const T*)in, ld, part, rows, C);)
    } else {
        dim3 grid((C + 127) / 128, CS_SLABS);
        DISPATCH_T(dtype, colsum_part_kernel<T, 16><<<grid, 256, 0, ST>>>((const T*)in, ld, part, rows, C);)
    }
    colsum_f32_kernel<<<(C + 31) / 32, 256, 0, ST>>>(part, out, CS_SLABS, C, beta);
    return vpu_check_launch("vpu_colsum");
}
extern "C" int vpu_softmax_fwd(const float* S, int32_t lds_, void* P, int32_t ldp, int64_t rows, int32_t ncols,
                               int32_t dtype, void* stream) {
    vpu_clear_stale_error();
    if (ncols > 4096 || ldp > 4096 || ldp < ncols) { vpu_set_error("softmax: ncols <= 4096"); return VPU_ERR_ARG; }
    if (ldp <= 1024) { DISPATCH_T(dtype, (softmax_fwd_kernel<T, 16><<<(unsigned)((rows + 3) / 4), 256, 0, ST>>>(S, lds_, (T*)P, ldp, rows, ncols));) }
    else { DISPATCH_T(dtype, (softmax_fwd_kernel<T, 64><<<(unsigned)((rows + 3) / 4), 256, 0, ST>>>(S, lds_, (T*)P, ldp, rows, ncols));) }
    return vpu_check_launch("vpu_softmax_fwd");
}
extern "C" int vpu_softmax_bwd(const void* P, int32_t ldp, const float* dP, int32_t lddp, void* dS, int64_t rows,
                               int32_t ncols, float scale, int32_t dtype, void* stream) {
    vpu_clear_stale_error();
    if (ncols > 4096 || ldp > 4096 || ldp < ncols) { vpu_set_error("softmax_bwd: ncols <= 4096"); return VPU_ERR_ARG; }
    if (ldp <= 1024) { DISPATCH_T(dtype, (softmax_bwd_kernel<T, 16><<<(unsigned)((rows + 3) / 4), 256, 0, ST>>>((const T*)P, ldp, dP, lddp, (T*)dS, rows, ncols, scale));) }
    else { DISPATCH_T(dtype, (softmax_bwd_kernel<T, 64><<<(unsigned)((rows + 3) / 4), 256, 0, ST>>>((const T*)P, ldp, dP, lddp, (T*)dS, rows, ncols, scale));) }
    return vpu_check_launch("vpu_softmax_bwd");
}
extern "C" int vpu_l2norm_fwd(const void* x, void* y, float* inv, int64_t rows, int32_t C, int32_t dtype, void* stream) {
    vpu_clear_stale_error();
    if ((C == 64 || C == 128 || C == 256 || C == 512) && (reinterpret_cast<uintptr_t>(x) | reinterpret_cast<uintptr_t>(y)) % 32 == 0) {
        const int64_t trips = (rows * (C / 8) + 63) / 64;
        const unsigned grid = (unsigned)(trips / 4 < 1 ? 1 : (trips / 4 > 8192 ? 8192 : trips / 4));
        DISPATCH_T(dtype, l2norm_fwd_vec_kernel<T><<<grid, 256, 0, ST>>>((const T*)x, (T*)y, inv, rows, C);)
        return vpu_check_launch("vpu_l2norm_fwd");
    }
    DISPATCH_T(dtype, l2norm_fwd_kernel<T><<<(unsigned)((rows + 3) / 4), 256, 0, ST>>>((const T*)x, (T*)y, inv, rows, C);)
    return vpu_check_launch("vpu_l2norm_fwd");
// ... 51 lines not shown
extern "C" int vpu_cast2d(const void* src, int32_t src_dtype, int64_t ld_src, void* dst, int32_t dst_dtype,
                          int64_t ld_dst, int64_t rows, int32_t cols, int32_t cols_pad, void* stream) {
    vpu_clear_stale_error();
    const int grid = vpu_grid_for(rows * cols_pad, 256, 8192);
    if (src_dtype == VPU_F32 && dst_dtype == VPU_BF16)
        cast2d_kernel<float, bf16_t><<<grid, 256, 0, ST>>>((const float*)src, ld_src, (bf16_t*)dst, ld_dst, rows, cols, cols_pad);
    else if (src_dtype == VPU_F32 && dst_dtype == VPU_F32)
        cast2d_kernel<float, float><<<grid, 256, 0, ST>>>((const float*)src, ld_src, (float*)dst, ld_dst, rows, cols, cols_pad);
    else if (src_dtype == VPU_BF16 && dst_dtype == VPU_F32)
        cast2d_kernel<bf16_t, float><<<grid, 256, 0, ST>>>((const bf16_t*)src, ld_src, (float*)dst, ld_dst, rows, cols, cols_pad);
    else if (src_dtype == VPU_BF16 && dst_dtype == VPU_BF16)
        cast2d_kernel<bf16_t, bf16_t><<<grid, 256, 0, ST>>>((const bf16_t*)src, ld_src, (bf16_t*)dst, ld_dst, rows, cols, cols_pad);
    else { vpu_set_error("cast2d: dtype"); return VPU_ERR_ARG; }
    return vpu_check_launch("vpu_cast2d");
}
extern "C" int vpu_cast2d_batched(const vpu_cast_job* jobs, int32_t n, void* stream) {
    vpu_clear_stale_error();
    if (!jobs || n < 1 || n > CAST_MAXJ) { vpu_set_error("cast2d_batched: 1 <= n <= 8 jobs"); return VPU_ERR_ARG; }
    CastBatch b{};
    int64_t most = 1;
    for (int i = 0; i < n; ++i) {
        const vpu_cast_job& j = jobs[i];
        if (!j.src || !j.dst || j.rows < 1 || j.cols < 1 || j.cols_pad < j.cols || (j.dst_dtype != VPU_BF16 && j.dst_dtype != VPU_F32) ||
            (j.perm_g > 0 && (j.perm_wg < 1 || j.perm_g % j.perm_wg || j.rows != (int64_t)j.perm_g * j.perm_g))) {
            vpu_set_error("cast2d_batched: null operand, empty job, dtype, or a row map that does not fit the rows");
            return VPU_ERR_ARG;
        }
        b.j[i] = CastJob{j.src, j.src2, j.dst, j.ld_src, j.ld_dst, j.rows, j.cols, j.cols_pad, j.dst_dtype, j.perm_g, j.perm_wg};
        most = most > j.rows * j.cols_pad ? most : j.rows * j.cols_pad;
    }
    cast2d_batched_kernel<<<dim3(vpu_grid_for(most, 256, 2048), n), 256, 0, ST>>>(b);
    return vpu_check_launch("vpu_cast2d_batched");
}
extern "C" int vpu_act_bwd(const void* dy, int64_t ld_dy, const void* aux, int64_t ld_aux, void* dz, int64_t ld_dz,
                           int64_t rows, int32_t cols, int32_t kind, int32_t dtype, void* stream) {
    vpu_clear_stale_error();
    if (cols % 8 || ld_dy % 8 || ld_aux % 8 || ld_dz % 8) { vpu_set_error("act_bwd: cols, ld % 8"); return VPU_ERR_ARG; }
    const int grid = vpu_grid_for(rows * (cols / 8), 256, 8192);
    DISPATCH_T(dtype, act_bwd_kernel<T><<<grid, 256, 0, ST>>>((const T*)dy, ld_dy, (const T*)aux, ld_aux, (T*)dz, ld_dz,
                                                             rows, cols, kind);)
    return vpu_check_launch("vpu_act_bwd");
}
extern "C" int vpu_sigmoid_to_channel(const float* logits, float* out, int32_t B, int64_t HW, int32_t channels,
                                      int32_t channel, void* stream) {
    vpu_clear_stale_error();
    const int64_t total = (int64_t)B * HW;
    sigmoid_to_channel_kernel<<<vpu_grid_for(total, 256, 4096), 256, 0, ST>>>(logits, out, HW, (int64_t)channels * HW,
                                                                             (int64_t)channel * HW, total);
    return vpu_check_launch("vpu_sigmoid_to_channel");
}
namespace {
__global__ __launch_bounds__(512) void debug_spin_kernel(float* sink, long long cycles) {
    __shared__ float pad[4096];
    float r[80];
#pragma unroll
    for (int i = 0; i < 80; ++i) r[i] = (float)(threadIdx.x + i);
    pad[threadIdx.x] = r[3];
    const long long t0 = wall_clock64();
    while (wall_clock64() - t0 < cycles / 24) {
#pragma unroll
        for (int i = 0; i < 80; ++i) r[i] = r[i] * 1.0001f + pad[(threadIdx.x + i) & 4095];
    }
    float t = 0.f;
#pragma unroll
    for (int i = 0; i < 80; ++i) t += r[i];
    if (t == 1.2345e30f) sink[0] = t;
}
}
extern "C" int vpu_debug_spin(float* sink, int32_t wgs, int64_t cycles, void* stream) {
    vpu_clear_stale_error();
    if (wgs < 1 || wgs > 256 || cycles < 0 || cycles > 240000000LL) { vpu_set_error("debug_spin: 1 <= wgs <= 256, cycles <= 2.4e8"); return VPU_ERR_ARG; }
    debug_spin_kernel<<<wgs, 512, 0, ST>>>(sink, (long long)cycles);
    return vpu_check_launch("vpu_debug_spin");
}
extern "C" int vpu_dropout_mask(float* out, int32_t n, float keep, uint64_t seed, uint64_t* state, void* stream) {
    vpu_clear_stale_error();
    if (!out || !state || n < 1 || n > (1 << 22) || !(keep > 0.f && keep <= 1.f)) {
        vpu_set_error("dropout_mask: non-null out / state, 1 <= n <= 2^22, 0 < keep <= 1");
        return VPU_ERR_ARG;
    }
    dropout_mask_kernel<<<1, 256, 0, ST>>>(out, n, keep, 1.0f / keep, (unsigned long long)seed, reinterpret_cast<unsigned long long*>(state));
    return vpu_check_launch("vpu_dropout_mask");
}
extern "C" int vpu_fill_ranges_f32(float* base, const int64_t* off, const int64_t* len, int32_t n, float v, void* stream) {
    vpu_clear_stale_error();
    if (!base || !off || !len || n < 1 || n > FILL_MAX_RANGES || (reinterpret_cast<uintptr_t>(base) & 15)) {
        vpu_set_error("fill_ranges: 1 <= n <= 160 ranges, 16-byte aligned base");
        return VPU_ERR_ARG;
    }
    FillRanges r;
    r.n = n;
    int chunks = 0;
    for (int i = 0; i < n; ++i) {
        if (off[i] < 0 || len[i] <= 0 || (off[i] & 3) || (len[i] & 3)) {
            vpu_set_error("fill_ranges: offsets and lengths must be positive multiples of 4 floats");
            return VPU_ERR_ARG;
        }
        r.first_chunk[i] = chunks;
        r.off[i] = off[i];
        r.len[i] = len[i];
        chunks += (int)((len[i] + FILL_CHUNK - 1) / FILL_CHUNK);
    }
    r.first_chunk[n] = chunks;
    fill_ranges_kernel<<<(unsigned)chunks, 256, 0, ST>>>(base, r, v);
    return vpu_check_launch("vpu_fill_ranges_f32");
}
extern "C" int vpu_fill_f32(float* p, float v, int64_t n, void* stream) {
    vpu_clear_stale_error();
    const int64_t n4 = (n >> 2) + 8;
    fill_kernel<<<(unsigned)((n4 + 255) / 256 < 0x7FFFFFFF ? (n4 + 255) / 256 : 0x7FFFFFFF), 256, 0, ST>>>(p, v, n);
    return vpu_check_launch("vpu_fill_f32");
}
```

### pvpuformer_amd/engine.py

```python
import contextlib
import math
import os
from collections import OrderedDict
from types import SimpleNamespace

import numpy as np
import torch

from . import ops
from ._lib import (BF16, F32, EPI_BIAS, EPI_PREACT, EPI_GELU, EPI_RELU, EPI_DGELU, EPI_DRELU, EPI_RESID, EPI_AFFINE,
                   EPI_ACCUM, EPI_OUT_F32, EPI_SAVE_DGELU, EPI_MULAUX)


class Tape:
    __slots__ = ("fns", "out_grads", "done", "sim_low", "lane")

    def __init__(self):
        self.fns = []
        self.out_grads = [None, None, None]
        self.done = False
        self.sim_low = None
        self.lane = None

    def append(self, fn):
        s = self.lane
        if s is not None:
            inner = fn

            def fn():
                with torch.cuda.stream(s):
                    inner()
        self.fns.append(fn)

    def __len__(self):
        return len(self.fns)


class Var:
    __slots__ = ("t", "g", "gn_stats")

    def __init__(self, t):
        self.t = t
        self.g = None
        self.gn_stats = None


def _rup(x, m):
    return (x + m - 1) // m * m


def click_lut():
    t = np.arange(0, 19, 1, np.float32)
    lut = np.exp(-((t - 9) ** 2) / (2 * 3 ** 2))
    lut[9] += 1
    return lut


def pos2d_table(d_model, height, width):
    pe = torch.zeros(d_model, height, width)
    half = d_model // 2
    div = torch.exp(torch.arange(0., half, 2) * -(math.log(10000.0) / half))
    pw = torch.arange(0., width).unsqueeze(1) * div
    ph = torch.arange(0., height).unsqueeze(1) * div
    pe[0:half:2] = torch.sin(pw).t().unsqueeze(1).expand(-1, height, -1)
    pe[1:half:2] = torch.cos(pw).t().unsqueeze(1).expand(-1, height, -1)
    pe[half::2] = torch.sin(ph).t().unsqueeze(2).expand(-1, -1, width)
    pe[half + 1::2] = torch.cos(ph).t().unsqueeze(2).expand(-1, -1, width)
    return pe.reshape(d_model, height * width).t().contiguous()


def window_geometry(S, P):
    S, P = int(S), int(P)
    wg = 224 // P
    g = S // P if P > 0 else 0
    if P < 1 or wg < 1 or g < wg:
        raise ValueError(f"input side {S} with patch {P}: the token grid S // P = {g} must hold at least one "
                         f"{wg}-token window (S >= {wg * P})")
    nwin = g // wg
    if g % nwin:
        raise ValueError(f"input side {S} with patch {P}: the token grid g = S // P = {g} must split into nwin = g // {wg} = "
                         f"{nwin} equal windows per side (g % nwin == 0), as the reference's patchify requires")
    return g, nwin, g // nwin


def check_square(H, W):
    if H != W:
        raise ValueError(f"input {H}x{W}: only square inputs are supported (the reference's neck takes h = w = sqrt(HW))")


class Engine:
    def __init__(self, cfg, dtype="bf16", device="cuda"):
        self.cfg = dict(cfg)
        self.dt = BF16 if dtype in ("bf16", BF16) else F32
        self.td = torch.bfloat16 if self.dt == BF16 else torch.float32
        self.dev = torch.device(device)
        c = self.cfg
        self.D, self.P, self.img = c["embed_dim"], c["patch"], c["img"]
        self.g, _, self.wside = window_geometry(self.img, self.P)
        self.NT = self.g * self.g
        self.heads = c["num_heads"]
        self.depth = c["depth"]
        self.group = 6 if self.depth == 12 else self.depth // 4
        self.nmax = c["num_max_points"]
        self.E = 2 * self.img + 3
        self.Epad = _rup(self.E, 8)
        self.C = c["head_channels"]
        self.out_dims = tuple(c["out_dims"])
        self.names = None
        self.tape = Tape()
        self.last_tape = None
        self.params = []
        self.norm_radius = float(c.get("norm_radius", 5))
        self.training = False
        self.shadow_valid = False
        self._const_ready = False
        self.use_flash = True
        self.use_side = os.environ.get("VPU_WGRAD_STREAM", "0") == "1"
        self.side = None
        self.fuse_ln_pe = True
        self.group_wgrad = True
        self.ride_wgrad = True
        self.wgrad_fill = 0.8
        hid = self.D * c["mlp_ratio"]
        blk = sum(((n + 255) // 256) * ((k + 127) // 128) for n, k in ((3 * self.D, self.D), (self.D, self.D), (hid, self.D), (self.D, hid)))
        pk = os.environ.get("VPU_WGRAD_PACK", "")
        k3 = ops.gemm_get_option("k3")
        k4_default = (k3 & 8) != 0
        self.pack_wgrad = pk == "1" or (pk != "0" and (blk < 0.95 * 256 or k4_default))
        self.k3_wgrad = (k3 & 1) != 0
        self.k4_wgrad = (k3 & 8) != 0
        self.wgrad_round = 256 if (self.k4_wgrad or not self.k3_wgrad) else 512
        self.wgrad_tn = 256 if self.k4_wgrad else 128
        self.unify_wgrad = True
        self.lazy_zero = True
        self.xattn_split = max(1, int(os.environ.get("VPU_XATTN_SPLIT", "1")))
        self.neck_lanes = int(os.environ.get("VPU_NECK_LANES", "0"))
        self._tok_stream = None
        self._in_lanes = False
        self.dist_colsum = True
        self._pack_seen, self._pack_total = {}, {}
        self._pending_reports, self._reporting = [], False
        self.group_tiles = 256
        self.split_wgrad = True
        self._wq = []
        self._csq = []
        self._gq = []
        self._gq_out = set()
        self._frozen = set()
        self._token_rows = 0
        self.grad_ready_hook = None
        self.report_lag = max(1, int(os.environ.get("VPU_DIST_REPORT_LAG", "2")))

    def bind(self, named_params):
        self.names = OrderedDict()
        off = 0
        for n, p in named_params.items():
            self.names[n] = (off, tuple(p.shape), p.numel())
            off = _rup(off + p.numel(), 8)
        self.total = off
        self.flat = torch.zeros(off, device=self.dev, dtype=torch.float32)
        self.gflat = torch.zeros(off, device=self.dev, dtype=torch.float32)
        self.params = []
        for n, p in named_params.items():
            o, shape, numel = self.names[n]
            view = self.flat[o:o + numel].view(shape)
            view.copy_(p.data)
            p.data = view
            p.grad = self.gflat[o:o + numel].view(shape)
            self.params.append((p, o, shape, numel))
        self.shadow = torch.zeros(off, device=self.dev, dtype=torch.bfloat16) if self.dt == BF16 else None
        self._lazy = set()
        self._lazy_names, self._lazy_ranges = self._lazy_plan()
        D, P = self.D, self.P
        self.k3p = _rup(3 * P * P, 8)
        self.w_patch = torch.zeros(D, 2 * self.k3p, device=self.dev, dtype=self.td)
        self.b_patch = torch.zeros(D, device=self.dev, dtype=torch.float32)
        self.w_lin1p = torch.zeros(2048, self.Epad, device=self.dev, dtype=self.td)
        self.pos_win = torch.zeros(self.NT, D, device=self.dev, dtype=self.td)
        self._pos_cache, self._kpe_cache, self._regrid_cache = {}, {}, {}
        self.shadow_valid = False
        if not self._const_ready:
            self.kpe = pos2d_table(D, self.g, self.g).to(self.dev).to(self.td)
            self.lut = torch.from_numpy(click_lut()).to(self.dev)
            self._const_ready = True

    def W(self, name):
        o = self.names[name][0]
        return (self.shadow, o) if self.dt == BF16 else (self.flat, o)

    def Pm(self, name):
        return (self.flat, self.names[name][0])

    def G(self, name):
        return (self.gflat, self.names[name][0])

    def refresh_weights(self, shadow_is_fresh=False):
        D, P = self.D, self.P
        if self.dt == BF16 and not shadow_is_fresh:
            ops.cast2d(self.flat, self.total, self.shadow, self.total, 1, self.total)
        k3 = 3 * P * P
        po = self.names["backbone.pos_embed"][0]
        ops.cast2d_batched([
            dict(src=self.Pm("backbone.patch_embed.proj.weight"), dst=(self.w_patch, 0), ld_src=k3, ld_dst=2 * self.k3p, rows=D, cols=k3),
            dict(src=self.Pm("patch_embed_coords.proj.weight"), dst=(self.w_patch, self.k3p), ld_src=k3, ld_dst=2 * self.k3p, rows=D,
                 cols=k3),
            dict(src=self.Pm("backbone.patch_embed.proj.bias"), src2=self.Pm("patch_embed_coords.proj.bias"), dst=self.b_patch,
                 ld_src=D, ld_dst=D, rows=1, cols=D),
            dict(src=self.Pm("neck.ffn_layer.lin1.weight"), dst=self.w_lin1p, ld_src=self.E, ld_dst=self.Epad, rows=2048, cols=self.E,
                 cols_pad=self.Epad),
            dict(src=(self.flat, po + D), dst=self.pos_win, ld_src=D, ld_dst=D, rows=self.NT, cols=D, perm=(self.g, self.wside)),
        ])
        self._pos_cache = {(self.g, self.wside): self.pos_win}
        self.shadow_valid = True

    def _regrid_adjoint(self, g):
        Rt = self._regrid_cache.get(g)
        if Rt is None:
            import torch.nn.functional as F
            g0 = self.g
            basis = torch.eye(g0 * g0, dtype=torch.float32).view(1, g0 * g0, g0, g0)
            Rt = F.interpolate(basis, size=(g, g), mode="bicubic", align_corners=False).reshape(g0 * g0, g * g)
            Rt = Rt.contiguous().to(self.dev)
            self._regrid_cache[g] = Rt
        return Rt

    def _pos_for(self, g, wside):
        pw = self._pos_cache.get((g, wside))
        if pw is None:
            import torch.nn.functional as F
            D, g0 = self.D, self.g
            po = self.names["backbone.pos_embed"][0]
            grid = self.flat[po + D: po + D + g0 * g0 * D].view(1, g0, g0, D).permute(0, 3, 1, 2)
            new = F.interpolate(grid, size=(g, g), mode="bicubic", align_corners=False).permute(0, 2, 3, 1)
            tmp = new.reshape(g * g, D).to(self.td).contiguous()
            pw = torch.empty(g * g, D, device=self.dev, dtype=self.td)
            ops.window_permute(tmp, pw, 1, g, wside, D, to_raster=False)
            self._pos_cache[(g, wside)] = pw
        return pw

    def _kpe_for(self, g):
        k = self._kpe_cache.get(g)
        if k is None:
            k = self.kpe if g == self.g else pos2d_table(self.D, g, g).to(self.dev).to(self.td)
            self._kpe_cache[g] = k
        return k

    def zero_grad(self, lazy=False):
        self._lazy = set()
        if (lazy and self.lazy_zero and self.group_wgrad and self.dt == BF16 and not self.use_side and self.pack_wgrad
                and self._lazy_ranges is not None):
            ops.zero_ranges_(self.gflat, self._lazy_ranges)
            self._lazy = set(self._lazy_names)
        else:
            ops.zero_(self.gflat)

    def _lazy_plan(self):
        names = [n for n in self.names if n.startswith("backbone.blocks.") and
                 n.endswith((".attn.qkv.weight", ".attn.proj.weight", ".mlp.fc1.weight", ".mlp.fc2.weight"))]
        ranges, pos = [], 0
        for n in names:
            o, _, numel = self.names[n]
            if o % 4 or numel % 4:
                return [], None
            if o > pos:
                ranges.append((pos, o - pos))
            pos = o + numel
        if self.total > pos:
            ranges.append((pos, self.total - pos))
        return names, (ranges if names else None)

    def _lazy_finish(self):
        if self._lazy:
            ops.zero_ranges_(self.gflat, [(self.names[n][0], self.names[n][2]) for n in sorted(self._lazy, key=lambda k: self.names[k][0])])
            self._lazy = set()

    def attach_grads(self):
        if not self.params:
            return
        def ok(e):
            p, o, shape, numel = e
            return p.grad is not None and p.grad.data_ptr() == self.gflat.data_ptr() + 4 * o
        if ok(self.params[0]) and ok(self.params[-1]):
            return
        for e in self.params:
            p, o, shape, numel = e
            if ok(e):
                continue
            seg = self.gflat[o:o + numel]
            if p.grad is None:
                seg.zero_()
            else:
                seg.copy_(p.grad.reshape(-1))
            p.grad = seg.view(shape)

    def _new(self, *shape, dtype=None):
        return torch.empty(shape, device=self.dev, dtype=dtype or self.td)

    def _upload(self, t, dtype):
        if t.is_cuda:
            return t.to(dtype=dtype).contiguous()
        return t.to(dtype).contiguous().pin_memory().to(self.dev, non_blocking=True)

    def acc(self, var, g, take=False):
        if var.g is None:
            if take:
                var.g = g
            else:
                var.g = torch.empty_like(g)
                ops.add4(g, None, None, None, var.g, g.numel())
        else:
            self._writable(var.g)
            ops.add4(var.g, g, None, None, var.g, g.numel())

    def _reduce_wb(self, part, nrows, prefix, Cdim):
        ow, ob = self.names[prefix + ".weight"][0], self.names[prefix + ".bias"][0]
        if ob == ow + Cdim:
            self._csq.append((part, self.G(prefix + ".weight"), nrows, 2 * Cdim))
        else:
            ops.colsum_f32(part.view(nrows, 2 * Cdim)[:, :Cdim].contiguous(), self.G(prefix + ".weight"), nrows, Cdim, beta=1.0)
            ops.colsum_f32(part.view(nrows, 2 * Cdim)[:, Cdim:].contiguous(), self.G(prefix + ".bias"), nrows, Cdim, beta=1.0)

    def _colsum_to(self, dy, ld, gname, rows, N):
        part = self._new(64, N, dtype=torch.float32)
        ops.colsum(dy, ld, self.G(gname), part, rows, N, beta=1.0)

    def _wgrad(self, dy, ld_dy, x, ld_x, gname, N, K, M, ldc=None, bias=None):
        fuse = bias is not None and self.dt == BF16
        gout = self.G(gname) if isinstance(gname, str) else gname
        if self.group_wgrad and self.dt == BF16 and not self.use_side:
            ldc_ = K if ldc is None else ldc
            args = (dy, x, gout, N, K, M, ld_dy, ld_x, ldc_, self.dt)
            acc = EPI_ACCUM
            if isinstance(gname, str) and gname in self._lazy:
                self._lazy.discard(gname)
                acc = 0
            kw = dict(transA=True, transB=True, flags=EPI_OUT_F32 | acc, colsum=self.G(bias) if fuse else None)
            L = self._token_rows
            ctn = (K + 255) // 256
            al16 = lambda t: (ops.ptr(t) & 15) == 0
            dcs = (fuse and self.dist_colsum and self.k4_wgrad and self.pack_wgrad and ctn > 1 and M % 64 == 0 and M > 2048
                   and N % 8 == 0 and K % 8 == 0 and ld_dy % 8 == 0 and ld_x % 8 == 0 and al16(dy) and al16(x))
            if (self.unify_wgrad and self.pack_wgrad and (self.k3_wgrad or self.k4_wgrad) and L > 2048 and M > L and M % L == 0
                    and L % 64 == 0 and N % 8 == 0 and K % 8 == 0 and ld_dy % 8 == 0 and ld_x % 8 == 0 and ldc_ % 4 == 0):
                S = M // L
                slab = self._new(S * N * K, dtype=torch.float32)
                post = [((slab, 0), gout, S, N * K, K, ldc_)]
                cs = None
                if fuse and dcs:
                    cs = (self._new(S * ctn * N, dtype=torch.float32), 0)
                    post.append((cs, self.G(bias), S * ctn, N))
                elif fuse:
                    cs = (ops.zero_(self._new(S * N, dtype=torch.float32)), 0)
                    post.append((cs, self.G(bias), S, N))
                args = (dy, x, (slab, 0), N, K, L, ld_dy, ld_x, K, self.dt)
                kw = dict(transA=True, transB=True, flags=EPI_OUT_F32, colsum=cs, batch=S, sA=(L * ld_dy, 0), sB=(L * ld_x, 0),
                          sC=(N * K, 0), _post=post, _target=[gout] + ([self.G(bias)] if fuse else []))
                if fuse and dcs:
                    kw.update(cs_tn=ctn, cs_t0=0, cs_ld=N)
                M = L
            elif dcs and self.unify_wgrad:
                cs = (self._new(ctn * N, dtype=torch.float32), 0)
                kw.update(colsum=cs, cs_tn=ctn, cs_t0=0, cs_ld=N, _post=[(cs, self.G(bias), ctn, N)],
                          _target=[gout, self.G(bias)])
            self._wq.append((args, kw, ((N + 127) // 128) * ((K + 127) // 128) * kw.get("batch", 1), M))
            for t in (dy, x):
                tt = t[0] if isinstance(t, tuple) else t
                self._frozen.add(tt.data_ptr())
            kind = 0 if M <= 2048 else M
            if kind and self.ride_wgrad and self.pack_wgrad:
                self._pack_seen[kind] = self._pack_seen.get(kind, 0) + self._k2_tiles(self._wq[-1])
            if not self._in_lanes:
                self._wgrad_autoflush(kind)
            return
        if not self.use_side:
            ops.gemm(dy, x, gout, N, K, M, ld_dy, ld_x, K if ldc is None else ldc, self.dt, transA=True,
                     transB=True, flags=EPI_OUT_F32 | EPI_ACCUM, colsum=self.G(bias) if fuse else None)
            if bias is not None and not fuse:
                self._colsum_to(dy, ld_dy, bias, M, N)
            return
        if self.side is None:
            self.side = torch.cuda.Stream(device=self.dev)
        main = torch.cuda.current_stream(self.dev)
        self.side.wait_stream(main)
        for t in (dy, x):
            tt = t[0] if isinstance(t, tuple) else t
            tt.record_stream(self.side)
            self._frozen.add(tt.data_ptr())
        with torch.cuda.stream(self.side):
            ops.gemm(dy, x, gout, N, K, M, ld_dy, ld_x, K if ldc is None else ldc, self.dt, transA=True,
                     transB=True, flags=EPI_OUT_F32 | EPI_ACCUM, colsum=self.G(bias) if fuse else None)
            if bias is not None and not fuse:
                self._colsum_to(dy, ld_dy, bias, M, N)

    def _wgrad_autoflush(self, kind):
        same = [e for e in self._wq if (0 if e[3] <= 2048 else e[3]) == kind]
        if kind and self.ride_wgrad:
            anchors = [e for e in same if not self._is_rider(e)]
            T = sum(self._k2_tiles(e) for e in anchors)
            if self.pack_wgrad:
                budget = self.pack_tiles(None, self.wgrad_round - (self.wgrad_round // 256) * self._reserved_cus())
                while True:
                    mine = [e for e in self._wq if e[3] == kind]
                    T = sum(self._k2_tiles(e) for e in mine)
                    t_small = sum(self._k2_tiles(e) for e in [e for e in mine if self._pack_small(e)][:9])
                    t_big = sum(self._k2_tiles(e) for e in mine if not self._pack_small(e))
                    if not (T >= budget and (t_small + t_big >= budget or T >= 2 * budget)):
                        break
                    self.flush_wgrads(kind, ride=True, budget=budget)
                    if sum(self._k2_tiles(e) for e in self._wq if e[3] == kind) >= T:
                        break
            elif (T >= 200 and T >= self.wgrad_fill * 256 * ((T + 255) // 256)) or len(anchors) >= 8:
                self.flush_wgrads(kind, ride=True)
        elif len(same) >= 16:
            self.flush_wgrads(kind)

    def _dgrad(self, dy, ld_dy, w, ldw, xvar, M, K, N, flags=0, aux=None, ldaux=0, defer=False):
        f = flags
        if xvar.g is None:
            xvar.g = torch.empty_like(xvar.t)
        else:
            self._writable(xvar.g)
            f |= EPI_ACCUM
        args = (dy, w, xvar.g, M, K, N, ld_dy, ldw, K, self.dt)
        kw = dict(transB=True, flags=f, aux=aux, ldaux=ldaux)
        if defer:
            self._gemm_deferred(xvar.g.data_ptr(), args, kw)
        else:
            ops.gemm(*args, **kw)

    def _gemm_deferred(self, out_ptr, args, kw):
        if out_ptr in self._gq_out:
            self.flush_group()
        self._gq.append((args, kw))
        self._gq_out.add(out_ptr)

    def flush_group(self):
        q, self._gq = self._gq, []
        self._gq_out = set()
        is_small = [((a[3] + 127) // 128) * ((a[4] + 127) // 128) <= self.group_tiles and a[5] <= 2048 for a, _ in q]
        if sum(is_small) >= 2:
            ops.gemm_grouped([e for e, sm in zip(q, is_small) if sm])
            q = [e for e, sm in zip(q, is_small) if not sm]
        for args, kw in q:
            ops.gemm(*args, **kw)

    @contextlib.contextmanager
    def _lane(self, s):
        if s is None:
            yield
            return
        prev, self.tape.lane = self.tape.lane, s
        try:
            with torch.cuda.stream(s):
                yield
        finally:
            self.tape.lane = prev

    def _cur(self, s):
        return torch.cuda.current_stream(self.dev) if s is None else s

    def _xrec(self, src, on_bwd=None):
        h = {"ev": torch.cuda.Event(), "bev": None}
        h["ev"].record(self._cur(src))
        if self.training:
            def bwd():
                if h["bev"] is not None:
                    self._cur(src).wait_event(h["bev"])
                if on_bwd is not None:
                    on_bwd()
            self.tape.fns.append(bwd)
        return h

    def _xwait(self, h, dst, on_bwd=None):
        self._cur(dst).wait_event(h["ev"])
        if self.training:
            def bwd():
                if on_bwd is not None:
                    on_bwd()
                h["bev"] = torch.cuda.Event()
                h["bev"].record(self._cur(dst))
            self.tape.fns.append(bwd)

    def linear(self, x, wname, bname, M, N, K, act=None, resid=None, out=None, x_grad=True, group=False, pre_masked=None):
        assert not (act and resid is not None)
        if out is None:
            y = Var(self._new(M, N))
            yt, yoff, ldc = y.t, 0, N
        else:
            y, yoff, ldc = out
            yt = y.t
        flags = EPI_BIAS | (EPI_RELU if act == "relu" else 0) | (EPI_RESID if resid is not None else 0)
        group = group and self.dt == BF16 and act is None and resid is None and out is None
        g_args = (x.t, self.W(wname), (yt, yoff), M, N, K, K, K, ldc, self.dt)
        g_kw = dict(flags=flags, bias=self.Pm(bname), resid=None if resid is None else resid.t, ldr=N)
        if group:
            self._gemm_deferred(yt.data_ptr(), g_args, g_kw)
        else:
            ops.gemm(*g_args, **g_kw)
        if self.training:
            def bwd():
                if y.g is None:
                    return
                dy = (y.g, yoff)
                if resid is not None:
                    assert out is None
                    self.acc(resid, y.g, take=True)
                if act == "relu" and not (pre_masked is not None and pre_masked[0]):
                    dz = self._new(M, N)
                    ops.act_bwd(dy, ldc, (yt, yoff), ldc, dz, N, M, N, 0, self.dt)
                    dy, ld = dz, N
                else:
                    ld = ldc
                self._wgrad(dy, ld, x.t, K, wname, N, K, M, bias=bname)
                if x_grad:
                    self._dgrad(dy, ld, self.W(wname), K, x, M, K, N, defer=group)
            self.tape.append(bwd)
        return y

    def mlp(self, x, p1, p2, M, K, Hd, N, act, resid=None, w1=None, k_grad=None, x_grad=True):
        Kp = K
        h = self._new(M, Hd)
        if act == "gelu":
            pre = self._new(M, Hd)
            ops.gemm(x.t, self.W(p1 + ".weight") if w1 is None else w1, h, M, Hd, Kp, Kp, Kp, Hd, self.dt,
                     flags=EPI_BIAS | EPI_SAVE_DGELU | EPI_GELU, bias=self.Pm(p1 + ".bias"), preact=pre)
        else:
            pre = None
            ops.gemm(x.t, self.W(p1 + ".weight") if w1 is None else w1, h, M, Hd, Kp, Kp, Kp, Hd, self.dt,
                     flags=EPI_BIAS | EPI_RELU, bias=self.Pm(p1 + ".bias"))
        y = Var(self._new(M, N))
        ops.gemm(h, self.W(p2 + ".weight"), y.t, M, N, Hd, Hd, Hd, N, self.dt,
                 flags=EPI_BIAS | (EPI_RESID if resid is not None else 0), bias=self.Pm(p2 + ".bias"),
                 resid=None if resid is None else resid.t, ldr=N)
        if self.training:
            def bwd():
                dy = y.g
                if dy is None:
                    return
                if resid is not None:
                    self.acc(resid, dy, take=True)
                self._wgrad(dy, N, h, Hd, p2 + ".weight", N, Hd, M, bias=p2 + ".bias")
                dpre = self._new(M, Hd)
                ops.gemm(dy, self.W(p2 + ".weight"), dpre, M, Hd, N, N, Hd, Hd, self.dt, transB=True,
                         flags=EPI_MULAUX if act == "gelu" else EPI_DRELU, aux=pre if act == "gelu" else h, ldaux=Hd)
                kg = K if k_grad is None else k_grad
                self._wgrad(dpre, Hd, x.t, Kp, p1 + ".weight", Hd, kg, M, bias=p1 + ".bias")
                if x_grad:
                    self._dgrad(dpre, Hd, self.W(p1 + ".weight") if w1 is None else w1, Kp, x, M, Kp, Hd)
            self.tape.append(bwd)
        return y

    def layernorm(self, x, prefix, rows, Cdim, eps, pe=None, pe_rows=0, pe_var=None):
        if pe is not None and not self.fuse_ln_pe:
            y = self.layernorm(x, prefix, rows, Cdim, eps)
            return y, self.add_pe(y, pe, rows * Cdim, pe_rows * Cdim, pe_var=pe_var)
        y = Var(self._new(rows, Cdim))
        yy = Var(self._new(rows, Cdim)) if pe is not None else None
        mean, rstd = self._new(rows, dtype=torch.float32), self._new(rows, dtype=torch.float32)
        if pe is None:
            ops.layernorm_fwd(x.t, self.Pm(prefix + ".weight"), self.Pm(prefix + ".bias"), y.t, mean, rstd, rows, Cdim, eps)
        else:
            ops.layernorm_fwd_pe(x.t, self.Pm(prefix + ".weight"), self.Pm(prefix + ".bias"), y.t, mean, rstd, rows, Cdim,
                                 eps, pe, pe_rows, yy.t)
        if self.training:
            def bwd():
                dy, dy2 = y.g, (yy.g if yy is not None else None)
                if dy is None and dy2 is None:
                    return
                if dy2 is not None and pe_var is not None:
                    self.acc(pe_var, dy2)
                if dy is None:
                    dy, dy2 = dy2, None
                nblk = ops.layernorm_bwd_nblk(rows)
                part = self._new(nblk, 2, Cdim, dtype=torch.float32)
                dres = x.g
                if x.g is None or x.g.data_ptr() in self._frozen:
                    x.g = torch.empty_like(x.t)
                ops.layernorm_bwd(dy, x.t, self.Pm(prefix + ".weight"), mean, rstd, dres, x.g, part, rows, Cdim, dy2=dy2)
                self._reduce_wb(part, nblk, prefix, Cdim)
            self.tape.append(bwd)
        return y if pe is None else (y, yy)

    def sdpa(self, q, k, v, o, nb, H, nq, nk, hd, scale):
        (qv, qo, qld, qrows), (kv, ko, kld, krows), (vv, vo, vld, vrows), (ov, oo, old, orows) = q, k, v, o
        ldS = _rup(nk, 8)
        S = self._new(nb * H, nq, ldS, dtype=torch.float32)
        sS = (H * nq * ldS, nq * ldS)
        ops.gemm((qv.t, qo), (kv.t, ko), S, nq, nk, hd, qld, kld, ldS, self.dt, flags=EPI_OUT_F32, alpha=scale,
                 batch=nb * H, inner=H, sA=(qrows * qld, hd), sB=(krows * kld, hd), sC=sS)
        Pm = self._new(nb * H, nq, ldS)
        ops.softmax_fwd(S, ldS, Pm, ldS, nb * H * nq, nk)
        del S
        ops.gemm(Pm, (vv.t, vo), (ov.t, oo), nq, hd, nk, ldS, vld, old, self.dt, transB=True, batch=nb * H, inner=H,
                 sA=sS, sB=(vrows * vld, hd), sC=(orows * old, hd))
        if self.training:
            def bwd():
                if ov.g is None:
                    return
                for var in {id(qv): qv, id(kv): kv, id(vv): vv}.values():
                    assert var.g is None, "sdpa inputs must be single-use projections"
                    var.g = torch.empty_like(var.t)
                dO = (ov.g, oo)
                dP = self._new(nb * H, nq, ldS, dtype=torch.float32)
                ops.gemm(dO, (vv.t, vo), dP, nq, nk, hd, old, vld, ldS, self.dt, flags=EPI_OUT_F32, batch=nb * H,
                         inner=H, sA=(orows * old, hd), sB=(vrows * vld, hd), sC=sS)
                ops.gemm(Pm, dO, (vv.g, vo), nk, hd, nq, ldS, old, vld, self.dt, transA=True, transB=True, batch=nb * H,
                         inner=H, sA=sS, sB=(orows * old, hd), sC=(vrows * vld, hd))
                dS = self._new(nb * H, nq, ldS)
                ops.softmax_bwd(Pm, ldS, dP, ldS, dS, nb * H * nq, nk, scale)
                del dP
                ops.gemm(dS, (kv.t, ko), (qv.g, qo), nq, hd, nk, ldS, kld, qld, self.dt, transB=True, batch=nb * H,
                         inner=H, sA=sS, sB=(krows * kld, hd), sC=(qrows * qld, hd))
                ops.gemm(dS, (qv.t, qo), (kv.g, ko), nk, hd, nq, ldS, qld, kld, self.dt, transA=True, transB=True,
                         batch=nb * H, inner=H, sA=sS, sB=(qrows * qld, hd), sC=(krows * kld, hd))
            self.tape.append(bwd)

    def flash_attention(self, qkv, O, nb, H, n, hd, D, scale):
        lse = self._new(nb * H, n, dtype=torch.float32)
        ops.attn_fwd((qkv.t, 0), (qkv.t, D), (qkv.t, 2 * D), O.t, lse, nb, H, n, hd, 3 * D, D, scale)
        if self.training:
            def bwd():
                if O.g is None:
                    return
                assert qkv.g is None
                qkv.g = torch.empty_like(qkv.t)
                delta = self._new(nb * H, n, dtype=torch.float32)
                ops.attn_bwd((qkv.t, 0), (qkv.t, D), (qkv.t, 2 * D), O.t, O.g, lse, delta, (qkv.g, 0), (qkv.g, D),
                             (qkv.g, 2 * D), nb, H, n, hd, 3 * D, D, 3 * D, scale)
            self.tape.append(bwd)

    def cross_attention(self, Qp, Kp, Vp, O, nb, H, nq, nk, hd, ld, scale):
        S = self.xattn_split
        long_q = S > 1 and nq >= 4 * nk and nq % (4 * S) == 0 and nq // S >= 64
        long_k = S > 1 and not long_q and nk >= 4 * nq and nk % S == 0 and nk // S >= 64 and nq % 4 == 0
        if long_q:
            lse = self._new(nb * S * H, nq // S, dtype=torch.float32)
            ops.xattn_fwd_split(Qp.t, Kp.t, Vp.t, O.t, lse, nb * S, H, nq // S, nk, hd, ld, ld, ld, scale, 1, S)
        elif long_k:
            lse = self._new(nb * H, nq, dtype=torch.float32)
            o_s, lse_s = self._new(nb * S * nq, ld), self._new(nb * S * H, nq, dtype=torch.float32)
            ops.xattn_fwd_split(Qp.t, Kp.t, Vp.t, o_s, lse_s, nb * S, H, nq, nk // S, hd, ld, ld, ld, scale, S, 1)
            ops.attn_combine(o_s, lse_s, O.t, lse, nb, H, nq, hd, S, ld, ld)
        else:
            lse = self._new(nb * H, nq, dtype=torch.float32)
            ops.xattn_fwd(Qp.t, Kp.t, Vp.t, O.t, lse, nb, H, nq, nk, hd, ld, ld, ld, scale)
        if self.training:
            def bwd():
                if O.g is None:
                    return
                for var in {id(Qp): Qp, id(Kp): Kp, id(Vp): Vp}.values():
                    assert var.g is None, "attention inputs must be single-use projections"
                    var.g = torch.empty_like(var.t)
                if long_q:
                    delta = self._new(nb * S * H, nq // S, dtype=torch.float32)
                    dkp, dvp = self._new(nb * S * nk, ld), self._new(nb * S * nk, ld)
                    ops.xattn_bwd_split(Qp.t, Kp.t, Vp.t, O.t, O.g, lse, delta, Qp.g, dkp, dvp, nb * S, H, nq // S, nk, hd, ld, ld,
                                        ld, ld, ld, scale, 1, S)
                    ops.sum_groups(dkp, Kp.g, nb, S, nk * ld)
                    ops.sum_groups(dvp, Vp.g, nb, S, nk * ld)
                elif long_k:
                    delta = self._new(nb * H, nq, dtype=torch.float32)
# ... 212 lines not shown
        else:
            ops.patch_im2col_floor(image4, disks, cols, B, H, W_, P, wside, prenorm=prenorm)
        x = Var(self._new(M, D))
        ops.gemm(cols, self.w_patch, x.t, M, D, KP, KP, KP, D, self.dt,
                 flags=EPI_BIAS | EPI_RESID, bias=self.b_patch, resid=pos_win, ldr=D, resid_period=NT)
        if cx.training:
            def bwd_patch():
                if x.g is None:
                    return
                k3 = 3 * P * P
                for nm, co in (("backbone.patch_embed.proj", 0), ("patch_embed_coords.proj", self.k3p)):
                    self._wgrad(x.g, D, (cols, co), KP, nm + ".weight", D, k3, M, bias=nm + ".bias")
                s = self._new(NT * D, dtype=torch.float32)
                ops.colsum(x.g, NT * D, s, None, B, NT * D, beta=0.0)
                r = self._new(NT * D, dtype=torch.float32)
                ops.window_permute(s, r, 1, g, wside, D, to_raster=True)
                gp = (self.gflat, self.names["backbone.pos_embed"][0] + D)
                if g == self.g:
                    ops.add4(gp, r, None, None, gp, NT * D)
                else:
                    ops.gemm(self._regrid_adjoint(g), r, gp, self.g * self.g, D, NT, NT, D, D, F32, transB=True,
                             flags=EPI_OUT_F32 | EPI_ACCUM)
            self.tape.append(bwd_patch)
        if cx.taps is not None:
            cx.taps["tokens0_win"] = x.t
        return x

    def _blocks(self, cx, x):
        B, g, wside, NT, M, D, heads = cx.B, cx.g, cx.wside, cx.NT, cx.M, self.D, self.heads
        hd = D // heads
        for i in range(1, self.depth + 1):
            if cx.training:
                self._mark_ready(f"backbone.blocks.{i - 1}.norm1.weight",
                                 f"backbone.blocks.{i}.norm1.weight" if i < self.depth else "backbone.fc_norm.weight")
            nwin = 1 if i % self.group == 0 else cx.nw_side * cx.nw_side
            nt = NT // nwin
            p = f"backbone.blocks.{i - 1}."
            h1 = self.layernorm(x, p + "norm1", M, D, 1e-6)
            qkv = self.linear(h1, p + "attn.qkv.weight", p + "attn.qkv.bias", M, 3 * D, D)
            O = Var(self._new(M, D))
            if self.dt == BF16 and hd % 16 == 0 and hd <= 128 and self.use_flash:
                self.flash_attention(qkv, O, B * nwin, heads, nt, hd, D, hd ** -0.5)
            else:
                self.sdpa((qkv, 0, 3 * D, nt), (qkv, D, 3 * D, nt), (qkv, 2 * D, 3 * D, nt), (O, 0, D, nt), B * nwin,
                          heads, nt, nt, hd, hd ** -0.5)
            x1 = self.linear(O, p + "attn.proj.weight", p + "attn.proj.bias", M, D, D, resid=x)
            h2 = self.layernorm(x1, p + "norm2", M, D, 1e-6)
            x = self.mlp(h2, p + "mlp.fc1", p + "mlp.fc2", M, D, D * self.cfg["mlp_ratio"], D, "gelu", resid=x1)
        xr = Var(self._new(M, D))
        ops.window_permute(x.t, xr.t, B, g, wside, D, to_raster=True)
        if cx.training:
            def bwd_perm():
                if xr.g is None:
                    return
                gw = torch.empty_like(xr.g)
                ops.window_permute(xr.g, gw, B, g, wside, D, to_raster=False)
                self.acc(x, gw, take=True)
            self.tape.append(bwd_perm)
        if cx.taps is not None:
            cx.taps["backbone"] = xr.t
        if cx.training:
            self._mark_ready("backbone.fc_norm.weight", None)
        return xr

    def _prompt_vectors(self, cx, prompts):
        B, n, nq = cx.B, cx.n, cx.nq
        points, boxes, _, prof = prompts
        pue = Var(self._new(B * nq, self.Epad))
        if cx.rows is not None:
            ops.pue_encode_rows(points, cx.rows[0], boxes, prof, self.lut, pue.t, None, B, n, self.nmax, self.img, self.Epad)
        else:
            ops.pue_encode(points, boxes, self.lut, pue.t, None, B, n, self.nmax, self.img, self.Epad)
            if prof is not None:
                ops.pue_scribble_rows(points, prof, pue.t, None, B, n, self.nmax, self.img, self.Epad)
        return self.mlp(pue, "neck.ffn_layer.lin1", "neck.ffn_layer.lin2", B * nq, self.Epad, 2048, self.D, "relu",
                        w1=self.w_lin1p, k_grad=self.E, x_grad=False)

    def _neck_layer_tokens(self, cx, l, q, qq, q0):
        B, nq, D, p = cx.B, cx.nq, self.D, f"neck.att.layers.{l}"
        if l == 0:
            q = self.mha(p + ".self_attn", q, q, q, B, nq, nq, D)
        else:
            q = self.mha(p + ".self_attn", qq, qq, q, B, nq, nq, D, resid=q)
        return self.layernorm(q, p + ".norm1", B * nq, D, 1e-5, pe=q0.t, pe_rows=B * nq, pe_var=q0)

    def _neck(self, cx, prompts, xr, kpe_tab):
        B, NT, M, nq, D = cx.B, cx.NT, cx.M, cx.nq, self.D
        q0 = self._prompt_vectors(cx, prompts)
        q, k, qq, hs = q0, xr, None, []
        kk = self.add_pe(k, kpe_tab, M * D, NT * D)
        for l in range(3):
            p = f"neck.att.layers.{l}"
            q, qq = self._neck_layer_tokens(cx, l, q, qq, q0)
            q = self.mha(p + ".cross_attn_token_to_image", qq, kk, k, B, nq, NT, D // 2, resid=q)
            q = self.layernorm(q, p + ".norm2", B * nq, D, 1e-5)
            q = self.mlp(q, p + ".mlp.lin1", p + ".mlp.lin2", B * nq, D, 1024, D, "relu", resid=q)
            q, qq = self.layernorm(q, p + ".norm3", B * nq, D, 1e-5, pe=q0.t, pe_rows=B * nq, pe_var=q0)
            k2 = self.mha(p + ".cross_attn_image_to_token", kk, qq, q, B, NT, nq, D // 2, resid=k)
            k, kk = self.layernorm(k2, p + ".norm4", M, D, 1e-5, pe=kpe_tab, pe_rows=NT)
            if l != 2:
                hs.append((q, k))
        q = self.mha("neck.att.final_attn_token_to_image", qq, kk, k, B, nq, NT, D // 2, resid=q)
        q = self.layernorm(q, "neck.att.norm_final_attn", B * nq, D, 1e-5)
        hs.append((q, k))
        return q0, hs

    def _start_token_lane(self, cx, prompts):
        T = cx.T
        fns_main, self.tape.fns = self.tape.fns, []

        def lanes_done():
            self._in_lanes = False
            for kind in sorted({0 if e[3] <= 2048 else e[3] for e in self._wq}):
                self._wgrad_autoflush(kind)
        h_fork = self._xrec(None, on_bwd=lanes_done)
        self._xwait(h_fork, T)
        with self._lane(T):
            q0 = self._prompt_vectors(cx, prompts)
            q, qq = self._neck_layer_tokens(cx, 0, q0, None, q0)
            Qt = self._group(lambda: self._proj("neck.att.layers.0.cross_attn_token_to_image", "q", qq, cx.B * cx.nq, self.D // 2))
        early, self.tape.fns = self.tape.fns, fns_main
        return early, q0, (q, qq, Qt)

    def _neck_two_lane(self, cx, prompts, xr, kpe_tab, started):
        B, NT, M, nq, D, T = cx.B, cx.NT, cx.M, cx.nq, self.D, cx.T
        group, proj = self._group, self._proj
        if started is None:
            started = self._start_token_lane(cx, prompts)
        early, q0, (q, qq, Qt) = started
        self.tape.fns.extend(early)
        if self.neck_lanes == 2:
            h_early = self._xrec(T)
            self._xwait(h_early, None)
            T = None
        k, hs = xr, []
        kk = self.add_pe(k, kpe_tab, M * D, NT * D)
        for l in range(4):
            p = f"neck.att.layers.{l}"
            t2i = p + ".cross_attn_token_to_image" if l < 3 else "neck.att.final_attn_token_to_image"
            i2t = p + ".cross_attn_image_to_token"
            Kt, Vt = group(lambda: (proj(t2i, "k", kk, M, D // 2), proj(t2i, "v", k, M, D // 2)))
            h_kv = self._xrec(None)
            if l < 3:
                Qi = group(lambda: proj(i2t, "q", kk, M, D // 2))
            with self._lane(T):
                if 0 < l < 3:
                    q, qq = self._neck_layer_tokens(cx, l, q, qq, q0)
                if l > 0:
                    Qt = group(lambda: proj(t2i, "q", qq, B * nq, D // 2))
            self._xwait(h_kv, T)
            with self._lane(T):
                q = self._attend(B, t2i, Qt, Kt, Vt, nq, NT, D // 2, q)
                if l == 3:
                    q = self.layernorm(q, "neck.att.norm_final_attn", B * nq, D, 1e-5)
                else:
                    q = self.layernorm(q, p + ".norm2", B * nq, D, 1e-5)
                    q = self.mlp(q, p + ".mlp.lin1", p + ".mlp.lin2", B * nq, D, 1024, D, "relu", resid=q)
                    q, qq = self.layernorm(q, p + ".norm3", B * nq, D, 1e-5, pe=q0.t, pe_rows=B * nq, pe_var=q0)
                    Ki, Vi = group(lambda: (proj(i2t, "k", qq, B * nq, D // 2), proj(i2t, "v", q, B * nq, D // 2)))
            if l == 3:
                break
            h_tok = self._xrec(T)
            self._xwait(h_tok, None)
            k2 = self._attend(B, i2t, Qi, Ki, Vi, NT, nq, D // 2, k)
            k, kk = self.layernorm(k2, p + ".norm4", M, D, 1e-5, pe=kpe_tab, pe_rows=NT)
            if l != 2:
                hs.append((q, k))
        hs.append((q, k))

        def lanes_begin():
            self._in_lanes = True
        h_join = self._xrec(T)
        self._xwait(h_join, None, on_bwd=lanes_begin)
        return q0, hs

    def _gates(self, cx, xr, q0, hs):
        B, NT, M, nq, D = cx.B, cx.NT, cx.M, cx.nq, self.D
        q_out = Var(self._new(B * nq, D))
        ops.add4(q0.t, hs[0][0].t, hs[1][0].t, hs[2][0].t, q_out.t, B * nq * D)
        if cx.training:
            def bwd_qout():
                if q_out.g is None:
                    return
                vs = (q0, hs[0][0], hs[1][0], hs[2][0])
                had = [v.g is not None for v in vs]
                for v, h_ in zip(vs, had):
                    if h_:
                        self._writable(v.g)
                    else:
                        v.g = torch.empty_like(q_out.g)
                ops.fanout_add(q_out.g, [v.g for v in vs], had, q_out.g.numel())
            self.tape.append(bwd_qout)
        ng = len(hs)
        cg, sg = self._new(ng, B, D, dtype=torch.float32), self._new(ng, B, NT, dtype=torch.float32)
        aq, ac = self._new(ng, B, D, dtype=torch.int32), self._new(ng, B, NT, dtype=torch.int32)
        xgs = [Var(self._new(M, D)) for _ in range(ng)]
        ops.gate_fwd_n([qi.t for qi, _ in hs], [ki.t for _, ki in hs], xr.t, [v.t for v in xgs], cg, aq, sg, ac, B, nq, NT, D)
        if cx.training:
            def bwd_gates():
                live = [i for i in range(ng) if xgs[i].g is not None]
                if not live:
                    return
                if any(v.g is None for i in live for v in hs[i]):
                    pend = [v for i in live for v in hs[i] if v.g is None]
                    pool = ops.zero_(torch.empty(sum(v.t.numel() for v in pend), device=self.dev, dtype=self.td))
                    o_ = 0
                    for v in pend:
                        v.g = pool[o_:o_ + v.t.numel()].view_as(v.t)
                        o_ += v.t.numel()
                accum = xr.g is not None
                if not accum:
                    xr.g = torch.empty_like(xr.t)
                for t_ in [xr.g] + [v.g for i in live for v in hs[i]]:
                    self._writable(t_)
                part = self._new(ng, B, 64, D, dtype=torch.float32)
                if len(live) == ng:
                    ops.gate_bwd_n([v.g for v in xgs], xr.t, cg, aq, sg, ac, xr.g, accum, [hs[i][0].g for i in live],
                                   [hs[i][1].g for i in live], part, B, nq, NT, D)
                else:
                    for i in live:
                        ops.gate_bwd(xgs[i].g, xr.t, cg[i], aq[i], sg[i], ac[i], xr.g, accum, hs[i][0].g, hs[i][1].g, part[i], B, nq,
                                     NT, D)
                        accum = True
            self.tape.append(bwd_gates)
        if cx.taps is not None:
            cx.taps["q_out"] = q_out.t
        return q_out, [xr] + xgs

    def _fpn(self, cx, maps):
        B, g, NT, M, D, o = cx.B, cx.g, cx.NT, cx.M, self.D, self.out_dims
        c4 = max(o[0] * 2, D // 2)
        a = self.conv_t2(maps[0], "neck.down_4.0", B, g, g, D, c4, gn_next=True)
        a = self.groupnorm(a, "neck.down_4.1", B, 4 * NT, c4, True)
        a = self.conv_t2(a, "neck.down_4.3", B, 2 * g, 2 * g, c4, c4 // 2, gn_next=True)
        a = self.groupnorm(a, "neck.down_4.4", B, 16 * NT, c4 // 2, False)
        a = self.linear(a, "neck.down_4.5.weight", "neck.down_4.5.bias", B * 16 * NT, o[0], c4 // 2)
        d4 = self.groupnorm(a, "neck.down_4.6", B, 16 * NT, o[0], True)
        c8 = max(o[1], D // 2)
        a = self.conv_t2(maps[1], "neck.down_8.0", B, g, g, D, c8, gn_next=True)
        a = self.groupnorm(a, "neck.down_8.1", B, 4 * NT, c8, False)
        a = self.linear(a, "neck.down_8.2.weight", "neck.down_8.2.bias", B * 4 * NT, o[1], c8)
        d8 = self.groupnorm(a, "neck.down_8.3", B, 4 * NT, o[1], True)
        a = self.linear(maps[2], "neck.down_16.0.weight", "neck.down_16.0.bias", M, o[2], D)
        d16 = self.groupnorm(a, "neck.down_16.1", B, NT, o[2], True)
        c32 = max(o[3], D * 2)
        h32 = g // 2
        a = self.conv_s2(maps[3], "neck.down_32.0", B, h32, h32, D, c32, g=g)
        a = self.groupnorm(a, "neck.down_32.1", B, h32 * h32, c32, False)
        a = self.linear(a, "neck.down_32.2.weight", "neck.down_32.2.bias", B * h32 * h32, o[3], c32)
        d32 = self.groupnorm(a, "neck.down_32.3", B, h32 * h32, o[3], True)
        feats = [(d4, 4 * g), (d8, 2 * g), (d16, g), (d32, h32)]
        if cx.taps is not None:
            for i, (f, s) in enumerate(feats):
                cx.taps[f"fpn{i}"] = f.t
        return feats

    def _head(self, cx, feats, q_out, drop_mask, materialize_aux):
        B, H, W_, nq, o, tape = cx.B, cx.H, cx.W, cx.nq, self.out_dims, self.tape
        Cc, Hs = self.C, 4 * cx.g
        HW4 = Hs * Hs
        wf, ldf = self.W("head.fusion_conv.conv.weight"), 4 * Cc
        gf = self.G("head.fusion_conv.conv.weight")
        relu_done, ymask = [False], [[False] for _ in range(4)]
        ys, zs = [], []
        for i in range(4):
            f, s = feats[i]
            ys.append(self.linear(f, f"head.convs.{i}.conv.weight", f"head.convs.{i}.conv.bias", B * s * s, Cc, o[i],
                                  act="relu", pre_masked=ymask[i]))
        fused = Var(self._new(B * HW4, Cc))
        ops.gemm(ys[0].t, wf, fused.t, B * HW4, Cc, Cc, Cc, ldf, Cc, self.dt, flags=EPI_BIAS,
                 bias=self.Pm("head.fusion_conv.conv.bias"))
        for i in (1, 2, 3):
            s = feats[i][1]
            z = self._new(B * s * s, Cc)
            ops.gemm(ys[i].t, (wf[0], wf[1] + i * Cc), z, B * s * s, Cc, Cc, Cc, ldf, Cc, self.dt)
            zs.append((z, s, s))
        ops.upsum_relu(fused.t, zs, B, Hs, Hs, Cc, self.dt)
        if cx.training:
            def bwd_fusion():
                if fused.g is None:
                    return
                if relu_done[0]:
                    dt_ = fused.g
                else:
                    dt_ = self._new(B * HW4, Cc)
                    ops.act_bwd(fused.g, Cc, fused.t, Cc, dt_, Cc, B * HW4, Cc, 0, self.dt)
                self._wgrad(dt_, Cc, ys[0].t, Cc, gf, Cc, Cc, B * HW4, ldc=ldf, bias="head.fusion_conv.conv.bias")
                fuse_mask = self.dt == BF16
# ... 213 lines not shown
                    t = self._k2_tiles(e)
                    if len(take) >= 16:
                        break
                    if t <= room:
                        take.append(e); room -= t
            q = take
        elif ride:
            anchors = [e for e in q if not self._is_rider(e)]
            T = sum(self._k2_tiles(e) for e in anchors)
            room, slots, take = 256 * ((T + 255) // 256) - T, 16 - len(anchors), []
            for e in q:
                if self._is_rider(e) and slots > 0 and self._k2_tiles(e) <= room:
                    take.append(e); slots -= 1; room -= self._k2_tiles(e)
            q = anchors + take
        elif keep_riders:
            q = [e for e in q if not self._is_rider(e)]
        if not q:
            return
        chosen = set(id(e) for e in q)
        self._wq = [e for e in self._wq if id(e) not in chosen]
        parts = {}
        for e in q:
            parts.setdefault(kind_of(e), []).append(e)
        for red, part in parts.items():
            nk = (red + 63) // 64
            tiles = sum(e[2] for e in part)
            elig = [e for e in part if e[0][8] == e[0][4] and e[1].get("batch", 1) == 1 and not e[1].get("cs_tn")
                    and (e[1].get("flags", 0) & EPI_ACCUM)]
            etiles = sum(e[2] for e in elig)
            if self.split_wgrad and 2048 < red <= 16384 and len(elig) >= 2 and etiles < 200:
                self._wgrad_sliced(elig, red, etiles)
                taken = set(id(e) for e in elig)
                part = [e for e in part if id(e) not in taken]
                tiles -= etiles
            if not part:
                pass
            elif len(part) >= 2 and (red == 0 or tiles >= 200 or nk * 0.6 < len(part) * 35.0):
                for i in range(0, len(part), 16):
                    chunk = part[i:i + 16]
                    if len(chunk) == 1 and chunk[0][1].get("batch", 1) == 1 and not chunk[0][1].get("cs_tn"):
                        ops.gemm(*chunk[0][0], **self._pub(chunk[0][1]))
                    else:
                        ops.gemm_grouped([(e[0], self._pub(e[1])) for e in chunk])
            else:
                for args, kw, _, _ in part:
                    if kw.get("batch", 1) > 1 or kw.get("cs_tn"):
                        ops.gemm_grouped([(args, self._pub(kw))])
                    else:
                        ops.gemm(*args, **self._pub(kw))
            for e in part:
                self._csq.extend(e[1].get("_post", ()))
        if not self.use_side:
            self._frozen = set()
            for args, _, _, _ in self._wq:
                for t in (args[0], args[1]):
                    self._frozen.add((t[0] if isinstance(t, tuple) else t).data_ptr())
        if self._pending_reports and not self._reporting:
            self._reporting = True
            try:
                self._report_ready()
            finally:
                self._reporting = False

    @staticmethod
    def _pub(kw):
        return {k: v for k, v in kw.items() if not k.startswith("_")} if any(k.startswith("_") for k in kw) else kw

    @staticmethod
    def _targets(e):
        args, kw = e[0], e[1]
        if "_target" in kw:
            return list(kw["_target"])
        out = [args[2]]
        if kw.get("colsum") is not None:
            out.append(kw["colsum"])
        return out

    def _wgrad_sliced(self, part, red, tiles):
        S = max(2, min(8, 288 // tiles, 16 // len(part)))
        kchunk = ((red + S - 1) // S + 63) // 64 * 64
        S = (red + kchunk - 1) // kchunk
        slab = self._new(sum(S * e[0][3] * e[0][4] for e in part), dtype=torch.float32)
        nb = sum(S * e[0][3] for e in part if e[1].get("colsum") is not None)
        bslab = ops.zero_(torch.empty(max(nb, 1), device=self.dev, dtype=torch.float32))
        sub, jobs, so, bo = [], [], 0, 0
        adv = lambda t, n: (t[0], t[1] + n) if isinstance(t, tuple) else (t, n)
        for args, kw, _, _ in part:
            dy, x, g, N, K, M, ld_dy, ld_x, ldc, dt = args
            cs = kw.get("colsum")
            for s in range(S):
                k0 = s * kchunk
                k1 = min(red, k0 + kchunk)
                kw_s = dict(kw, flags=EPI_OUT_F32, colsum=None if cs is None else (bslab, bo + s * N))
                sub.append(((adv(dy, k0 * ld_dy), adv(x, k0 * ld_x), (slab, so + s * N * K), N, K, k1 - k0, ld_dy, ld_x, K, dt), kw_s))
            jobs.append(((slab, so), g, S, N * K))
            so += S * N * K
            if cs is not None:
                jobs.append(((bslab, bo), cs, S, N))
                bo += S * N
        for i in range(0, len(sub), 16):
            ops.gemm_grouped(sub[i:i + 16])
        ops.colsum_batched(jobs)

    def flush_colsums(self):
        q, self._csq = self._csq, []
        if q:
            ops.colsum_batched(q)

    def join_side(self):
        self.flush_wgrads()
        if self.side is not None:
            torch.cuda.current_stream(self.dev).wait_stream(self.side)
        self._frozen.clear()

    def abort_pass(self):
        self._wq, self._csq, self._gq = [], [], []
        self._lazy_finish()
        self._gq_out, self._frozen = set(), set()
        self._pending_reports, self._reporting = [], False
        self._pack_seen = {}
        self._in_lanes = False
        self.tape = Tape()
        self.last_tape = None

    def _writable(self, t):
        if t is not None and t.data_ptr() in self._frozen:
            if self.use_side:
                self.join_side()
            else:
                self.flush_wgrads(touching=t.data_ptr())

    def backward(self, d_inst, d_aux, d_sim_low=None, tape=None):
        tape = self.last_tape if tape is None else tape
        if tape is None or tape.done or len(tape) == 0:
            raise RuntimeError("Engine.backward: no pending training-mode forward to back-propagate (its tape was "
                               "already run, or forward ran with training=False)")
        self.attach_grads()
        tape.out_grads[:] = [None if d_inst is None else d_inst.contiguous(), None if d_aux is None else d_aux.contiguous(),
                             None if d_sim_low is None else d_sim_low.contiguous()]
        self._pack_seen = {}
        for fn in reversed(tape.fns):
            fn()
        self._pack_total = self._pack_seen
        tape.fns = []
        tape.done = True
        if tape is self.last_tape:
            self.last_tape = None
        self.tape = Tape()
        self.join_side()
        self.flush_colsums()
        self._lazy_finish()
        self._report_ready(final=True)
        if self.grad_ready_hook is not None:
            self.grad_ready_hook(0, self.names["backbone.blocks.0.norm1.weight"][0])
```

### pvpuformer_amd/ops.py

```python
import ctypes as C

import torch

from . import _lib
from ._lib import (BF16, F32, EPI_BIAS, EPI_PREACT, EPI_GELU, EPI_RELU, EPI_DGELU, EPI_DRELU, EPI_RESID, EPI_AFFINE,
                   EPI_ACCUM, EPI_OUT_F32, EPI_SAVE_DGELU, EPI_MULAUX, GemmDesc)

TORCH_DTYPE = {BF16: torch.bfloat16, F32: torch.float32}


def code_of(t):
    if isinstance(t, tuple):
        t = t[0]
    if t.dtype == torch.bfloat16:
        return BF16
    if t.dtype == torch.float32:
        return F32
    raise TypeError(f"unsupported dtype {t.dtype}")


_raw_stream = getattr(torch._C, "_cuda_getCurrentRawStream", None)
_cur_device = getattr(torch._C, "_cuda_getDevice", None)


# ... 27 lines not shown
        _WORKSPACE[key] = ws
    return ws


def _fill_desc(d, A, B, Cout, M, N, K, lda, ldb, ldc, dtype, transA=False, transB=False, flags=0, bias=None, resid=None,
               ldr=0, aux=None, ldaux=0, preact=None, alpha=1.0, post_mul=1.0, post_add=0.0, batch=1, inner=1,
               sA=(0, 0), sB=(0, 0), sC=(0, 0), sR=(0, 0), resid_period=0, workspace="auto", colsum=None,
               cs_tn=0, cs_t0=0, cs_ld=0):
    d.A, d.B, d.C = ptr(A), ptr(B), ptr(Cout)
    d.bias, d.resid, d.aux, d.preact = ptr(bias), ptr(resid), ptr(aux), ptr(preact)
    d.M, d.N, d.K = M, N, K
    d.lda, d.ldb, d.ldc, d.ldr, d.ldaux = lda, ldb, ldc, ldr, ldaux
    d.batch, d.inner = batch, inner
    d.sAo, d.sAi = sA
    d.sBo, d.sBi = sB
    d.sCo, d.sCi = sC
    d.sRo, d.sRi = sR
    d.transA, d.transB = int(transA), int(transB)
    d.dtype, d.flags = dtype, flags
    d.resid_period = resid_period
    d.alpha, d.post_mul, d.post_add = alpha, post_mul, post_add
    d.colsum = ptr(colsum)
    d.cs_tn, d.cs_t0, d.cs_ld = int(cs_tn), int(cs_t0), int(cs_ld)
    if workspace == "auto":
        c0 = Cout[0] if isinstance(Cout, tuple) else Cout
        workspace = split_k_workspace(c0.device)
    if workspace is not None:
        d.workspace, d.workspace_bytes = workspace.data_ptr(), workspace.numel() * workspace.element_size()


def gemm(A, B, Cout, M, N, K, lda, ldb, ldc, dtype, **kw):
    d = GemmDesc()
    _fill_desc(d, A, B, Cout, M, N, K, lda, ldb, ldc, dtype, **kw)
    _lib.call("vpu_gemm", C.byref(d), _stream())


def gemm_grouped(problems):
    n = len(problems)
    arr = (GemmDesc * n)()
    for d, (args, kw) in zip(arr, problems):
        kw = dict(kw)
        kw["workspace"] = None
        _fill_desc(d, *args, **kw)
    _lib.call("vpu_gemm_grouped", arr, n, _stream())


def gemm_last_kernel():
    return _lib.load().vpu_gemm_last_kernel().decode()


def attn_last_kernel():
    return _lib.load().vpu_attn_last_kernel().decode()


def attn_set_option(name, value):
    _lib.call("vpu_attn_set_option", name.encode(), int(value))


def gemm_set_option(name, value):
    _lib.call("vpu_gemm_set_option", name.encode(), int(value))


def gemm_get_option(name):
    import ctypes
    v = ctypes.c_int32(0)
    _lib.call("vpu_gemm_get_option", name.encode(), ctypes.byref(v))
    return int(v.value)


def layernorm_fwd(x, w, b, y, mean, rstd, rows, Cdim, eps):
    _lib.call("vpu_layernorm_fwd", ptr(x), ptr(w), ptr(b), ptr(y), ptr(mean), ptr(rstd), rows, Cdim, eps, code_of(x),
              _stream())


def layernorm_fwd_pe(x, w, b, y, mean, rstd, rows, Cdim, eps, pe, pe_rows, y2):
    _lib.call("vpu_layernorm_fwd_pe", ptr(x), ptr(w), ptr(b), ptr(y), ptr(mean), ptr(rstd), rows, Cdim, eps, ptr(pe),
              int(pe_rows), ptr(y2), code_of(x), _stream())


def layernorm_bwd_nblk(rows):
    return _lib.load().vpu_layernorm_bwd_nblk(rows)


def layernorm_bwd(dy, x, w, mean, rstd, dres, dx, part, rows, Cdim, dy2=None):
    if dy2 is None:
        _lib.call("vpu_layernorm_bwd", ptr(dy), ptr(x), ptr(w), ptr(mean), ptr(rstd), ptr(dres), ptr(dx), ptr(part), rows,
                  Cdim, code_of(x), _stream())
    else:
        _lib.call("vpu_layernorm_bwd2", ptr(dy), ptr(dy2), ptr(x), ptr(w), ptr(mean), ptr(rstd), ptr(dres), ptr(dx),
                  ptr(part), rows, Cdim, code_of(x), _stream())


def edt(mask_u8, zero_border=True):
    B, H, W = mask_u8.shape
    mask_u8 = mask_u8.contiguous()
    scratch = torch.empty(B, H, W, device=mask_u8.device, dtype=torch.int32)
    dist = torch.empty(B, H, W, device=mask_u8.device, dtype=torch.float32)
    _lib.call("vpu_edt", ptr(mask_u8), ptr(scratch), ptr(dist), B, H, W, int(zero_border), _stream())
    return dist


def chamfer5(mask_u8, zero_border=True):
    B, H, W = mask_u8.shape
    mask_u8 = mask_u8.contiguous()
    scratch = torch.empty(B, H + 2, W + 2, device=mask_u8.device, dtype=torch.int32)
    dist = torch.empty(B, H, W, device=mask_u8.device, dtype=torch.float32)
    _lib.call("vpu_chamfer5", ptr(mask_u8), ptr(scratch), ptr(dist), B, H, W, int(zero_border), _stream())
    return dist


def cc_roots(mask_u8):
    B, H, W = mask_u8.shape
    mask_u8 = mask_u8.contiguous()
    roots = torch.empty(B, H, W, device=mask_u8.device, dtype=torch.int32)
    _lib.call("vpu_cc_roots", ptr(mask_u8), ptr(roots), B, H, W, _stream())
    return roots


def cc_table(roots, kmax=4096):
    B, H, W = roots.shape
    slots = torch.empty(B, H, W, device=roots.device, dtype=torch.int32)
    table = torch.empty(kmax * 6 + 1, device=roots.device, dtype=torch.int32)
    _lib.call("vpu_cc_table", ptr(roots), ptr(slots), ptr(table), kmax, B, H, W, _stream())
    return table


def colsum_batched(jobs):
    for i in range(0, len(jobs), 64):
        chunk = jobs[i:i + 64]
        arr = (_lib.ColsumJob * len(chunk))()
        for j, job in zip(arr, chunk):
            inp, out, rows, Cdim = job[:4]
            j.inp, j.out, j.nrows, j.ncols = ptr(inp), ptr(out), rows, Cdim
            j.row_len, j.out_ld = (job[4], job[5]) if len(job) > 4 and job[4] and job[5] != job[4] else (0, 0)
        _lib.call("vpu_colsum_batched", arr, len(chunk), _stream())


def colsum_f32(inp, out, rows, Cdim, beta=0.0):
    _lib.call("vpu_colsum_f32", ptr(inp), ptr(out), rows, Cdim, beta, _stream())


def colsum(inp, ld, out, part, rows, Cdim, beta=0.0):
    _lib.call("vpu_colsum", ptr(inp), ld, ptr(out), ptr(part), rows, Cdim, beta, code_of(inp[0] if isinstance(inp, tuple) else inp),
              _stream())


def softmax_fwd(S, lds, P, ldp, rows, ncols):
    _lib.call("vpu_softmax_fwd", ptr(S), lds, ptr(P), ldp, rows, ncols, code_of(P), _stream())


def softmax_bwd(P, ldp, dP, lddp, dS, rows, ncols, scale):
    _lib.call("vpu_softmax_bwd", ptr(P), ldp, ptr(dP), lddp, ptr(dS), rows, ncols, scale, code_of(P), _stream())


def l2norm_fwd(x, y, inv, rows, Cdim):
    _lib.call("vpu_l2norm_fwd", ptr(x), ptr(y), ptr(inv), rows, Cdim, code_of(x), _stream())


def l2norm_bwd(dy, y, inv, dx, rows, Cdim):
    _lib.call("vpu_l2norm_bwd", ptr(dy), ptr(y), ptr(inv), ptr(dx), rows, Cdim, code_of(y), _stream())


def attn_fwd(q, k, v, out, lse, nb, H, n, hd, ld, ldo, scale):
    _lib.call("vpu_attn_fwd", ptr(q), ptr(k), ptr(v), ptr(out), ptr(lse), nb, H, n, hd, ld, ldo, scale, _stream())


def xattn_fwd(q, k, v, out, lse, nb, H, nq, nk, hd, ldq, ldk, ldo, scale):
    _lib.call("vpu_xattn_fwd", ptr(q), ptr(k), ptr(v), ptr(out), ptr(lse), nb, H, nq, nk, hd, ldq, ldk, ldo, scale,
# ... 38 lines not shown

def fanout_add(src, dsts, accum, n):
    arr = (C.c_void_p * len(dsts))(*[ptr(t) for t in dsts])
    acc = (C.c_int32 * len(dsts))(*[int(bool(a)) for a in accum])
    _lib.call("vpu_fanout_add", ptr(src), arr, acc, len(dsts), n, code_of(src), _stream())


def cast2d(src, ld_src, dst, ld_dst, rows, cols, cols_pad=None):
    s = src[0] if isinstance(src, tuple) else src
    d = dst[0] if isinstance(dst, tuple) else dst
    _lib.call("vpu_cast2d", ptr(src), code_of(s), ld_src, ptr(dst), code_of(d), ld_dst, rows, cols,
              cols if cols_pad is None else cols_pad, _stream())


def cast2d_batched(jobs):
    arr = (_lib.CastJob * len(jobs))()
    for j, q in zip(arr, jobs):
        d = q["dst"][0] if isinstance(q["dst"], tuple) else q["dst"]
        j.src, j.src2, j.dst = ptr(q["src"]), ptr(q.get("src2")), ptr(q["dst"])
        j.ld_src, j.ld_dst, j.rows = q["ld_src"], q["ld_dst"], q["rows"]
        j.cols, j.cols_pad, j.dst_dtype = q["cols"], q.get("cols_pad", q["cols"]), code_of(d)
        j.perm_g, j.perm_wg = q.get("perm", (0, 0))
    _lib.call("vpu_cast2d_batched", arr, len(jobs), _stream())


def act_bwd(dy, ld_dy, aux, ld_aux, dz, ld_dz, rows, cols, kind, dtype):
    _lib.call("vpu_act_bwd", ptr(dy), ld_dy, ptr(aux), ld_aux, ptr(dz), ld_dz, rows, cols, kind, dtype, _stream())


def sigmoid_to_channel(logits, out, B, HW, channels, channel):
    _lib.call("vpu_sigmoid_to_channel", ptr(logits), ptr(out), B, HW, channels, channel, _stream())


def debug_spin(sink, wgs, cycles):
    _lib.call("vpu_debug_spin", ptr(sink), int(wgs), int(cycles), _stream())


_drop_state = {}


def _drop_key(device):
    key = torch.device(device)
    if key.type == "cuda" and key.index is None:
        key = torch.device("cuda", torch.cuda.current_device())
    return key


def _drop_entry(key, seed=None):
    if key not in _drop_state:
        sd = int(torch.initial_seed() if seed is None else seed) & (2 ** 63 - 1)
        _drop_state[key] = torch.tensor([0, sd], dtype=torch.int64, device=key)
    return _drop_state[key]


def dropout_mask(B, channels, keep, device, seed=None):
    key = _drop_key(device)
    state = _drop_entry(key, seed)
    out = torch.empty(B, channels, device=key, dtype=torch.float32)
    _lib.call("vpu_dropout_mask", ptr(out), B * channels, float(keep), 0, ptr(state), _stream())
    return out


def dropout_seed(device, seed):
    set_dropout_state(device, {"seed": int(seed) & (2 ** 63 - 1), "calls": 0})


def dropout_state(device):
    st = _drop_entry(_drop_key(device)).cpu()
    return {"seed": int(st[1]), "calls": int(st[0])}


def set_dropout_state(device, d):
    st = _drop_entry(_drop_key(device))
    st.copy_(torch.tensor([int(d["calls"]), int(d["seed"]) & (2 ** 63 - 1)], dtype=torch.int64))


def zero_(t):
    nbytes = t.numel() * t.element_size()
    assert t.is_contiguous() and nbytes % 4 == 0
    _lib.call("vpu_fill_f32", ptr(t), 0.0, nbytes // 4, _stream())
    return t


def zero_ranges_(t, ranges):
    assert t.dtype == torch.float32 and t.is_contiguous()
    for i in range(0, len(ranges), 160):
        chunk = ranges[i:i + 160]
        offs = (C.c_int64 * len(chunk))(*[int(o) for o, _ in chunk])
        lens = (C.c_int64 * len(chunk))(*[int(n) for _, n in chunk])
        _lib.call("vpu_fill_ranges_f32", ptr(t), offs, lens, len(chunk), 0.0, _stream())
    return t


def fill_f32(t, v, n=None):
    _lib.call("vpu_fill_f32", ptr(t), v, t.numel() if n is None else n, _stream())


def pue_encode(points, boxes, lut, out, out64, B, n, num_max, img, ld):
    _lib.call("vpu_pue_encode", ptr(points), ptr(boxes), ptr(lut), ptr(out), ptr(out64), B, n, num_max, img, ld,
              code_of(out), _stream())


def pue_scribble_rows(points, vec64, out, out64, B, n, num_max, img, ld):
    _lib.call("vpu_pue_scribble_rows", ptr(points), ptr(vec64), ptr(out), ptr(out64), B, n, num_max, img, ld, code_of(out),
              _stream())


def draw_polyline(curve_i32, disks, B, P, H, W):
    _lib.call("vpu_draw_polyline", ptr(curve_i32), ptr(disks), B, P, H, W, _stream())


def pue_encode_rows(points, kinds_i32, boxes, vec64, lut, out, out64, B, n, num_max, img, ld):
    _lib.call("vpu_pue_encode_rows", ptr(points), ptr(kinds_i32), ptr(boxes), ptr(vec64), ptr(lut), ptr(out), ptr(out64),
              B, n, num_max, img, ld, code_of(out), _stream())


def draw_prompt_rows(kinds_i32, boxes, curve_i32, counts_i32, disks, B, Pmax, n, H, W):
    _lib.call("vpu_draw_prompt_rows", ptr(kinds_i32), ptr(boxes), ptr(curve_i32), ptr(counts_i32), ptr(disks), B, Pmax, n,
              H, W, _stream())


def mask_bbox(prob, thr, pos_clicks=None):
    B, H, W = prob.shape
    out = torch.empty(B, 5, device=prob.device, dtype=torch.int32)
    n = 0 if pos_clicks is None else int(pos_clicks.shape[0])
    _lib.call("vpu_mask_bbox", ptr(prob), float(thr), ptr(pos_clicks) if n else None, n, ptr(out), B, H, W, _stream())
    return out


def error_masks(pred_u8, gt_u8, valid_u8):
    H, W = gt_u8.shape
    out = torch.empty(2, H, W, device=gt_u8.device, dtype=torch.uint8)
    _lib.call("vpu_error_masks", ptr(pred_u8), ptr(gt_u8), ptr(valid_u8), ptr(out), H, W, _stream())
    return out


def masked_argmax(dist, keep_u8):
    P, H, W = dist.shape
    out = torch.empty(P, device=dist.device, dtype=torch.int64)
    _lib.call("vpu_masked_argmax", ptr(dist), ptr(keep_u8), ptr(out), P, H, W, _stream())
    return out


def roi_resize_batched(objs, n, out, S_h, S_w, flip, channels):
    _lib.call("vpu_roi_resize_batched", ptr(objs), n, ptr(out), S_h, S_w, int(flip), channels, _stream())


def roi_paste_batched(objs, n, probs, S_h, S_w, pred_thr, box_thr, max_hw):
    _lib.call("vpu_roi_paste_batched", ptr(objs), n, ptr(probs), S_h, S_w, float(pred_thr), float(box_thr), max_hw, _stream())


SESSION_PASTE_FORM = 1


def session_paste_batched(objs, n, probs, S_h, S_w, pred_thr, box_thr, max_hw, form=None):
    assert probs.dtype == torch.float32 and probs.is_contiguous()
    _lib.call("vpu_session_paste_batched", ptr(objs), n, ptr(probs), S_h, S_w, float(pred_thr), float(box_thr), max_hw,
              SESSION_PASTE_FORM if form is None else int(form), _stream())


def annot_compose_batched(objs, n, thr, max_hw):
    _lib.call("vpu_annot_compose_batched", ptr(objs), n, float(thr), max_hw, _stream())


def label_extract(labels, label, out, rec):
    H, W = labels.shape
    assert labels.element_size() == 2 and labels.is_contiguous()
    assert out.dtype == torch.float32 and out.is_contiguous() and tuple(out.shape) == (H, W)
    assert rec.dtype == torch.int32 and rec.is_contiguous() and rec.numel() >= 8
    _lib.call("vpu_label_extract", ptr(labels), ptr(out), ptr(rec), H, W, int(label), _stream())


RUNS_BAND_ROWS = 64
# ... 340 lines not shown
```

Baseline: 1011.

## Fuse layernorm backward with residual/PE grad accumulation, enable in-launch split-K reduction

Adds a layernorm backward variant that also accumulates the residual gradient and positional-embedding gradient in the same pass, which removes separate elementwise accumulation kernels in the decoder/neck. Extends the in-launch split-K reduction to generic GEMM kernels, adds a strided partial-sum order for large split counts, and turns in-launch reduction on by default. Zero-fills of extra buffers are batched into the range-fill kernel, and some allocations are moved onto an arena. These changes cut launches and memory passes, but they add atomic/fence overhead in GEMMs and extra reads in the layernorm backward.

```diff
diff --git a/include/vpu_hip.h b/include/vpu_hip.h
--- a/include/vpu_hip.h
+++ b/include/vpu_hip.h
@@ -72,6 +72,9 @@
 int vpu_layernorm_bwd2(const void* dy, const void* dy2, const void* x, const float* w, const float* mean,
                        const float* rstd, const void* dres, void* dx, float* part, int64_t rows, int32_t C,
                        int32_t dtype, void* stream);
+int vpu_layernorm_bwd3(const void* dy, const void* dy2, const void* x, const float* w, const float* mean,
+                       const float* rstd, const void* dres, void* dx, float* part, void* dpe, void* dacc, int64_t rows,
+                       int32_t C, int32_t dtype, void* stream);
 #define VPU_COLSUM_BATCH_MAX 64
 typedef struct vpu_colsum_job { const float* in; float* out; int32_t nrows, ncols, row_len, out_ld; } vpu_colsum_job;
 typedef struct vpu_colsum_batch { vpu_colsum_job job[VPU_COLSUM_BATCH_MAX]; } vpu_colsum_batch;
@@ -127,6 +130,8 @@
 int vpu_dropout_mask(float* out, int32_t n, float keep, uint64_t seed, uint64_t* state, void* stream);
 int vpu_fill_f32(float* p, float v, int64_t n, void* stream);
 int vpu_fill_ranges_f32(float* base, const int64_t* off, const int64_t* len, int32_t n, float v, void* stream);
+int vpu_fill_ranges2_f32(float* base, const int64_t* off, const int64_t* len, int32_t n, float* const* xptr,
+                         const int64_t* xlen, int32_t nx, float v, void* stream);
 int vpu_debug_spin(float* sink, int32_t wgs, int64_t cycles, void* stream);
 int vpu_debug_gemm_times(void* dev_buf);
 int vpu_sigmoid_to_channel(const float* logits, float* out, int32_t B, int64_t HW, int32_t channels, int32_t channel,
diff --git a/pvpuformer_amd/_lib.py b/pvpuformer_amd/_lib.py
--- a/pvpuformer_amd/_lib.py
+++ b/pvpuformer_amd/_lib.py
@@ -94,6 +94,7 @@
     "vpu_layernorm_bwd": [_P, _P, _P, _P, _P, _P, _P, _P, _L, _I, _I, _P],
     "vpu_layernorm_fwd_pe": [_P, _P, _P, _P, _P, _P, _L, _I, _F, _P, _L, _P, _I, _P],
     "vpu_layernorm_bwd2": [_P, _P, _P, _P, _P, _P, _P, _P, _P, _L, _I, _I, _P],
+    "vpu_layernorm_bwd3": [_P, _P, _P, _P, _P, _P, _P, _P, _P, _P, _P, _L, _I, _I, _P],
     "vpu_colsum_batched": [C.POINTER(ColsumJob), _I, _P],
     "vpu_colsum_f32": [_P, _P, _L, _I, _F, _P],
     "vpu_colsum": [_P, _I, _P, _P, _L, _I, _F, _I, _P],
@@ -117,6 +118,7 @@
     "vpu_dropout_mask": [_P, _I, _F, C.c_uint64, _P, _P],
     "vpu_fill_f32": [_P, _F, _L, _P],
     "vpu_fill_ranges_f32": [_P, C.POINTER(C.c_int64), C.POINTER(C.c_int64), _I, _F, _P],
+    "vpu_fill_ranges2_f32": [_P, C.POINTER(C.c_int64), C.POINTER(C.c_int64), _I, C.POINTER(C.c_void_p), C.POINTER(C.c_int64), _I, _F, _P],
     "vpu_debug_spin": [_P, _I, _L, _P],
     "vpu_debug_gemm_times": [_P],
     "vpu_sigmoid_to_channel": [_P, _P, _I, _L, _I, _I, _P],
diff --git a/pvpuformer_amd/csrc/gemm.hip b/pvpuformer_amd/csrc/gemm.hip
--- a/pvpuformer_amd/csrc/gemm.hip
+++ b/pvpuformer_amd/csrc/gemm.hip
@@ -523,8 +523,9 @@
         }
         asm volatile("s_waitcnt lgkmcnt(0)" ::: "memory");
     }
-    if constexpr (SLAB) {
-        if (cnt) {
+    if constexpr (SLAB || GEN) {
+        if (cnt && splitk > 1) {
+            if constexpr (GEN) __builtin_amdgcn_fence(__ATOMIC_RELEASE, "agent");
             asm volatile("s_waitcnt vmcnt(0)" ::: "memory");
             __syncthreads();
             unsigned* flag = reinterpret_cast<unsigned*>(lds);
@@ -536,40 +537,62 @@
                 if (tid == 0) __hip_atomic_store(tc, 0u, __ATOMIC_RELAXED, __HIP_MEMORY_SCOPE_AGENT);
                 __builtin_amdgcn_fence(__ATOMIC_ACQUIRE, "wavefront");
                 const int64_t mn = (int64_t)p.M * p.N;
-#pragma unroll
-                for (int pass = 0; pass < 2; ++pass)
-#pragma unroll
-                    for (int t = 0; t < 4; ++t) {
-                        const int u = lane + 64 * t;
-                        const int row = u >> 3, c8 = (u & 7) * 8;
-                        const int m = m0 + wm * 64 + pass * 32 + row;
-                        const int n = n0 + wn * 64 + c8;
-                        if (m < p.M && n < p.N) {
-                            float v[8] = {0.f, 0.f, 0.f, 0.f, 0.f, 0.f, 0.f, 0.f};
-                            for (int sl = 0; sl < splitk; ++sl) {
-                                const unsigned long long* sp = reinterpret_cast<const unsigned long long*>(
-                                    ws + ((int64_t)z * splitk + sl) * mn + (int64_t)m * p.N + n);
-#pragma unroll
-                                for (int j = 0; j < 4; ++j) {
-                                    const unsigned long long q = __hip_atomic_load(sp + j, __ATOMIC_RELAXED, __HIP_MEMORY_SCOPE_AGENT);
-                                    v[2 * j] += __builtin_bit_cast(float, (unsigned)(q & 0xFFFFFFFFull));
-                                    v[2 * j + 1] += __builtin_bit_cast(float, (unsigned)(q >> 32));
+                const bool v8 = vec != 0 && (p.N & 7) == 0;
+                const bool tree = v8 && splitk >= 16 && (mn >> 3) <= 8 * 65535;
+                for (int it = 0; it < 8; ++it) {
+                    const int u = lane + 64 * (it & 3);
+                    const int row = u >> 3, c8 = (u & 7) * 8;
+                    const int m = m0 + wm * 64 + (it >> 2) * 32 + row;
+                    const int n = n0 + wn * 64 + c8;
+                    if (m < p.M && n < p.N) {
+                        auto add_slices = [&](int sl0, int step, float (&a)[8]) {
+                            for (int sl = sl0; sl < splitk; sl += step) {
+                                const float* sf = ws + ((int64_t)z * splitk + sl) * mn + (int64_t)m * p.N + n;
+                                if (SLAB || v8) {
+                                    const unsigned long long* sp = reinterpret_cast<const unsigned long long*>(sf);
+#pragma unroll
+                                    for (int j = 0; j < 4; ++j) {
+                                        const unsigned long long q = __hip_atomic_load(sp + j, __ATOMIC_RELAXED, __HIP_MEMORY_SCOPE_AGENT);
+                                        a[2 * j] += __builtin_bit_cast(float, (unsigned)(q & 0xFFFFFFFFull));
+                                        a[2 * j + 1] += __builtin_bit_cast(float, (unsigned)(q >> 32));
+                                    }
+                                } else {
+                                    for (int j = 0; j < 8 && n + j < p.N; ++j)
+                                        a[j] += __hip_atomic_load(sf + j, __ATOMIC_RELAXED, __HIP_MEMORY_SCOPE_AGENT);
                                 }
                             }
-                            if (vec) {
-                                EpiPre e;
-                                e.has_pre = false; e.has_bias = false; e.pre = make_uint4(0, 0, 0, 0);
-                                epilogue_store8(p, p.flags, coff, roff, m, n, v, e);
-                            } else {
-                                for (int j = 0; j < 8; ++j) epilogue_store<bf16_t>(p, coff, roff, m, n + j, v[j]);
+                        };
+                        float v[8] = {0.f, 0.f, 0.f, 0.f, 0.f, 0.f, 0.f, 0.f};
+                        if (!tree) add_slices(0, 1, v);
+                        else {
+                            add_slices(0, 32, v);
+                            for (int q = 1; q < 32; ++q) {
+                                float pq[8] = {0.f, 0.f, 0.f, 0.f, 0.f, 0.f, 0.f, 0.f};
+                                add_slices(q, 32, pq);
+#pragma unroll
+                                for (int j = 0; j < 8; ++j) v[j] += pq[j];
                             }
                         }
+                        if (SLAB ? vec != 0 : v8) {
+                            EpiPre e;
+                            e.has_pre = false; e.has_bias = false; e.pre = make_uint4(0, 0, 0, 0);
+                            epilogue_store8(p, p.flags, coff, roff, m, n, v, e);
+                        } else {
+                            for (int j = 0; j < 8 && n + j < p.N; ++j) epilogue_store<bf16_t>(p, coff, roff, m, n + j, v[j]);
+                        }
                     }
+                }
                 if (CS && TA == 1 && p.colsum != nullptr && tile_n == 0 && tid < 128 && m0 + tid < p.M) {
                     const float* wb = ws + (int64_t)nbatch * splitk * mn + (int64_t)z * splitk * p.M + m0 + tid;
                     float t = 0.f;
-                    for (int sl = 0; sl < splitk; ++sl)
+                    for (int sl = 0; sl < splitk; sl += 32)
                         t += __hip_atomic_load(wb + (int64_t)sl * p.M, __ATOMIC_RELAXED, __HIP_MEMORY_SCOPE_AGENT);
+                    for (int q = 1; q < 32; ++q) {
+                        float pq = 0.f;
+                        for (int sl = q; sl < splitk; sl += 32)
+                            pq += __hip_atomic_load(wb + (int64_t)sl * p.M, __ATOMIC_RELAXED, __HIP_MEMORY_SCOPE_AGENT);
+                        t += pq;
+                    }
                     p.colsum[m0 + tid] += t;
                 }
             }
@@ -2124,7 +2147,7 @@
     return left >= 64 ? left : v;
 }
 inline int inlaunch_env0() {
-    static const int v = [] { const char* e = vpu_lab_getenv("VPU_GEMM_INLAUNCH"); return e ? atoi(e) : 0; }();
+    static const int v = [] { const char* e = vpu_lab_getenv("VPU_GEMM_INLAUNCH"); return e ? atoi(e) : 1; }();
     return v;
 }
 constexpr int64_t CNT_BYTES = 256 << 10;
@@ -2412,6 +2435,15 @@
         const bool spec_ok = use_dma && !no_spec && !big && !d->colsum && vec && splitk == 1 && d->N % 8 == 0 && (vec_arg & 255) == 1;
         bool launched = false, inlaunch = false;
         unsigned* cnt_arg = nullptr;
+        if (splitk > 1 && !big && vec_arg <= 1) {
+            const int inl = g_opt_inlaunch.load(std::memory_order_relaxed) >= 0 ? g_opt_inlaunch.load(std::memory_order_relaxed) : inlaunch_env0();
+            const int64_t slab_bytes = (int64_t)d->batch * splitk * d->M * d->N * 4;
+            if (inl && (inl == 1 || slab_bytes <= ((int64_t)inl << 20)) && tiles <= CNT_BYTES / 4 &&
+                (int64_t)d->M * d->N * 4 < 0x7FFFFFF0LL && d->workspace_bytes > 2 * CNT_BYTES) {
+                cnt_arg = reinterpret_cast<unsigned*>(reinterpret_cast<char*>(d->workspace) + d->workspace_bytes - CNT_BYTES);
+                inlaunch = true;
+            }
+        }
 #define VPU_LAUNCH_RING(TA_, TB_, CS_, FL_)                                                                            \
     do {                                                                                                             \
         static VpuDevOnce attr_;                                                                                   \
@@ -2488,13 +2520,6 @@
         const bool slab_ok = use_dma && !no_spec && !big && splitk > 1 && d->N % 8 == 0 && vec_arg <= 1;
         if (!launched && slab_ok) {
             launched = true;
-            const int inl = g_opt_inlaunch.load(std::memory_order_relaxed) >= 0 ? g_opt_inlaunch.load(std::memory_order_relaxed) : inlaunch_env0();
-            const int64_t slab_bytes = (int64_t)d->batch * splitk * d->M * d->N * 4;
-            if (inl && (inl == 1 || slab_bytes <= ((int64_t)inl << 20)) && tiles <= CNT_BYTES / 4 &&
-                (int64_t)d->M * d->N * 4 < 0x7FFFFFF0LL && d->workspace_bytes > 2 * CNT_BYTES) {
-                cnt_arg = reinterpret_cast<unsigned*>(reinterpret_cast<char*>(d->workspace) + d->workspace_bytes - CNT_BYTES);
-                inlaunch = true;
-            }
             if (d->colsum && key == 3) NOTE_KERNEL("gemm_bf16_kernel<1, 1, true, true, 65536, 0>");
             if (d->colsum && key == 3) gemm_bf16_kernel<1, 1, true, true, FL_SLAB><<<pgrid, block, 4 * TILE_BYTES, s>>>(*d, tiles_n, splitk, kchunk, ws, vec_arg, tiles_m, d->batch, cnt_arg);
             else if (d->colsum) launched = false;
@@ -2502,7 +2527,6 @@
             else if (key == 0) VPU_LAUNCH_FL(0, 0, FL_SLAB);
             else if (key == 1) VPU_LAUNCH_FL(0, 1, FL_SLAB);
             else launched = false;
-            if (!launched) { inlaunch = false; cnt_arg = nullptr; }
         }
         if (launched) {
         } else
diff --git a/pvpuformer_amd/csrc/rowops.hip b/pvpuformer_amd/csrc/rowops.hip
--- a/pvpuformer_amd/csrc/rowops.hip
+++ b/pvpuformer_amd/csrc/rowops.hip
@@ -112,14 +112,14 @@
     }
 }
 
-template <typename T, int NCH, int NW, bool PF, bool D2, int RW>
+template <typename T, int NCH, int NW, bool PF, bool D2, int RW, bool ACC = false>
 __global__ __launch_bounds__(64 * NW) void layernorm_bwd_kernel(const T* __restrict__ dy, const T* __restrict__ dy2,
                                                             const T* __restrict__ x,
                                                             const float* __restrict__ w,
                                                             const float* __restrict__ mean,
                                                             const float* __restrict__ rstd, const T* __restrict__ dres,
                                                             T* __restrict__ dx, float* __restrict__ part, int64_t rows,
-                                                            int C, int nblk) {
+                                                            int C, int nblk, T* dpe = nullptr, T* dacc = nullptr) {
     __shared__ float red[NW][8 * 64];
     const int lane = threadIdx.x & 63, wave = threadIdx.x >> 6;
     float dwa[NCH][8], dba[NCH][8];
@@ -164,6 +164,23 @@
     for (; row0 < rows; row0 += stride) {
         if (PF && row0 + stride < rows) request(row0 + stride, nx, nd, nres, nd2, nmu, nrs);
         if (!PF) request(row0, cx, cd, cr, cd2, mu, rs);
+        Raw8<T> ca[RW][ACC ? NCH : 1], cp[RW][ACC && D2 ? NCH : 1];
+        if (ACC) {
+#pragma unroll
+            for (int k = 0; k < RW; ++k) {
+                const int64_t r = row0 + k * half;
+                if (r < rows) {
+#pragma unroll
+                    for (int i = 0; i < NCH; ++i) {
+                        const int c = (lane + i * 64) * 8;
+                        if (c < C) {
+                            if (dacc) ca[k][i].load(dacc + r * C + c);
+                            if (D2 && dpe) cp[k][i].load(dpe + r * C + c);
+                        }
+                    }
+                }
+            }
+        }
         float s1[RW], s2[RW];
 #pragma unroll
         for (int k = 0; k < RW; ++k) {
@@ -224,6 +241,21 @@
                             o[j] += rs[k] * (g - s1[k] - xh * s2[k]);
                         }
                         store8(dx + row * C + c, o);
+                        if (ACC && dacc) {
+                            float a[8];
+                            ca[k][ACC ? i : 0].get(a);
+#pragma unroll
+                            for (int j = 0; j < 8; ++j) a[j] += to_f32(from_f32<T>(o[j]));
+                            store8(dacc + row * C + c, a);
+                        }
+                        if (ACC && D2 && dpe) {
+                            float a[8], d2[8];
+                            cp[k][ACC && D2 ? i : 0].get(a);
+                            cd2[k][D2 ? i : 0].get(d2);
+#pragma unroll
+                            for (int j = 0; j < 8; ++j) a[j] += d2[j];
+                            store8(dpe + row * C + c, a);
+                        }
                     }
                 }
             }
@@ -691,9 +723,10 @@
 struct FillRanges {
     int n;
     int first_chunk[FILL_MAX_RANGES + 1];
-    long long off[FILL_MAX_RANGES], len[FILL_MAX_RANGES];
+    float* ptr[FILL_MAX_RANGES];
+    long long len[FILL_MAX_RANGES];
 };
-__global__ __launch_bounds__(256) void fill_ranges_kernel(float* __restrict__ base, const FillRanges r, const float v) {
+__global__ __launch_bounds__(256) void fill_ranges_kernel(const FillRanges r, const float v) {
     const int c = blockIdx.x;
     int lo = 0, hi = r.n;
     while (hi - lo > 1) {
@@ -702,7 +735,7 @@
     }
     const long long start = (long long)(c - r.first_chunk[lo]) * FILL_CHUNK;
     const long long end = start + FILL_CHUNK < r.len[lo] ? start + FILL_CHUNK : r.len[lo];
-    float4* q = reinterpret_cast<float4*>(base + r.off[lo]);
+    float4* q = reinterpret_cast<float4*>(r.ptr[lo]);
     const float4 v4 = make_float4(v, v, v, v);
     for (long long i = (start >> 2) + threadIdx.x; i < (end >> 2); i += 256) q[i] = v4;
 }
@@ -744,15 +777,25 @@
     static const int cap = [] { const char* e = vpu_lab_getenv("VPU_LN_BWD_WGS"); const int v = e ? atoi(e) : 2; return 256 * (v < 1 ? 1 : (v > 4 ? 4 : v)); }();
     return (int)(n < 1 ? 1 : (n > cap ? cap : n));
 }
-extern "C" int vpu_layernorm_bwd2(const void* dy, const void* dy2, const void* x, const float* w, const float* mean,
-                                  const float* rstd, const void* dres, void* dx, float* part, int64_t rows, int32_t C,
-                                  int32_t dtype, void* stream) {
+extern "C" int vpu_layernorm_bwd3(const void* dy, const void* dy2, const void* x, const float* w, const float* mean,
+                                  const float* rstd, const void* dres, void* dx, float* part, void* dpe, void* dacc,
+                                  int64_t rows, int32_t C, int32_t dtype, void* stream) {
     vpu_clear_stale_error();
     if (C % 8 || C > LN_MAXCH * 512 || rows <= 0) { vpu_set_error("layernorm_bwd: C"); return VPU_ERR_ARG; }
+    if (dpe && !dy2) { vpu_set_error("layernorm_bwd: dpe takes the gradient dy2, which is null"); return VPU_ERR_ARG; }
+    if ((dpe && (dpe == dx || dpe == dres || dpe == dacc || dpe == dy || dpe == dy2)) ||
+        (dacc && (dacc == dx || dacc == dres || dacc == dy || dacc == dy2))) {
+        vpu_set_error("layernorm_bwd: dpe / dacc must not alias another operand");
+        return VPU_ERR_ARG;
+    }
     const int nblk = vpu_layernorm_bwd_nblk(rows);
     static const int rw2 = [] { const char* e = vpu_lab_getenv("VPU_LN_BWD_RW"); return e ? atoi(e) : 2; }();
 #define VPU_LN_BWD_(NCH_, NW_, RW_)                                                                                   \
-    if (dy2) { DISPATCH_T(dtype, (layernorm_bwd_kernel<T, NCH_, NW_, (NCH_ <= 2), true, RW_><<<nblk, 64 * NW_, 0, ST>>>(   \
+    if (dy2 && (dpe || dacc)) { DISPATCH_T(dtype, (layernorm_bwd_kernel<T, NCH_, NW_, (NCH_ <= 2), true, RW_, true><<<nblk, 64 * NW_, 0, ST>>>(   \
+                          (const T*)dy, (const T*)dy2, (const T*)x, w, mean, rstd, (const T*)dres, (T*)dx, part, rows, C, nblk, (T*)dpe, (T*)dacc));) } \
+    else if (dacc) { DISPATCH_T(dtype, (layernorm_bwd_kernel<T, NCH_, NW_, (NCH_ <= 2), false, RW_, true><<<nblk, 64 * NW_, 0, ST>>>(      \
+                          (const T*)dy, (const T*)nullptr, (const T*)x, w, mean, rstd, (const T*)dres, (T*)dx, part, rows, C, nblk, (T*)nullptr, (T*)dacc));) } \
+    else if (dy2) { DISPATCH_T(dtype, (layernorm_bwd_kernel<T, NCH_, NW_, (NCH_ <= 2), true, RW_><<<nblk, 64 * NW_, 0, ST>>>(   \
                           (const T*)dy, (const T*)dy2, (const T*)x, w, mean, rstd, (const T*)dres, (T*)dx, part, rows, C, nblk));) } \
     else { DISPATCH_T(dtype, (layernorm_bwd_kernel<T, NCH_, NW_, (NCH_ <= 2), false, RW_><<<nblk, 64 * NW_, 0, ST>>>(      \
                           (const T*)dy, (const T*)nullptr, (const T*)x, w, mean, rstd, (const T*)dres, (T*)dx, part, rows, C, nblk));) }
@@ -762,6 +805,11 @@
 #undef VPU_LN_BWD
 #undef VPU_LN_BWD_
     return vpu_check_launch("vpu_layernorm_bwd");
+}
+extern "C" int vpu_layernorm_bwd2(const void* dy, const void* dy2, const void* x, const float* w, const float* mean,
+                                  const float* rstd, const void* dres, void* dx, float* part, int64_t rows, int32_t C,
+                                  int32_t dtype, void* stream) {
+    return vpu_layernorm_bwd3(dy, dy2, x, w, mean, rstd, dres, dx, part, nullptr, nullptr, rows, C, dtype, stream);
 }
 extern "C" int vpu_layernorm_bwd(const void* dy, const void* x, const float* w, const float* mean, const float* rstd,
                                  const void* dres, void* dx, float* part, int64_t rows, int32_t C, int32_t dtype,
@@ -979,28 +1027,38 @@
     dropout_mask_kernel<<<1, 256, 0, ST>>>(out, n, keep, 1.0f / keep, (unsigned long long)seed, reinterpret_cast<unsigned long long*>(state));
     return vpu_check_launch("vpu_dropout_mask");
 }
+extern "C" int vpu_fill_ranges2_f32(float* base, const int64_t* off, const int64_t* len, int32_t n, float* const* xptr,
+                                    const int64_t* xlen, int32_t nx, float v, void* stream) {
+    vpu_clear_stale_error();
+    if (n < 0 || nx < 0 || n + nx < 1 || n + nx > FILL_MAX_RANGES || (n && (!base || !off || !len)) || (nx && (!xptr || !xlen)) ||
+        (reinterpret_cast<uintptr_t>(base) & 15)) {
+        vpu_set_error("fill_ranges: 1 <= n + nx <= 160 ranges, 16-byte aligned base");
+        return VPU_ERR_ARG;
+    }
+    FillRanges r;
+    r.n = n + nx;
+    int64_t chunks = 0;
+    for (int i = 0; i < n + nx; ++i) {
+        const bool x = i >= n;
+        const int64_t l = x ? xlen[i - n] : len[i];
+        if (x ? (!xptr[i - n] || (reinterpret_cast<uintptr_t>(xptr[i - n]) & 15) || l <= 0 || (l & 3))
+              : (off[i] < 0 || l <= 0 || (off[i] & 3) || (l & 3))) {
+            vpu_set_error("fill_ranges: offsets and lengths must be positive multiples of 4 floats, extra ranges 16-byte aligned");
+            return VPU_ERR_ARG;
+        }
+        r.first_chunk[i] = (int)chunks;
+        r.ptr[i] = x ? xptr[i - n] : base + off[i];
+        r.len[i] = l;
+        chunks += (l + FILL_CHUNK - 1) / FILL_CHUNK;
+        if (chunks > 0x7FFFFFFF) { vpu_set_error("fill_ranges: too many elements for one launch"); return VPU_ERR_ARG; }
+    }
+    r.first_chunk[n + nx] = (int)chunks;
+    fill_ranges_kernel<<<(unsigned)chunks, 256, 0, ST>>>(r, v);
+    return vpu_check_launch("vpu_fill_ranges_f32");
+}
 extern "C" int vpu_fill_ranges_f32(float* base, const int64_t* off, const int64_t* len, int32_t n, float v, void* stream) {
-    vpu_clear_stale_error();
-    if (!base || !off || !len || n < 1 || n > FILL_MAX_RANGES || (reinterpret_cast<uintptr_t>(base) & 15)) {
-        vpu_set_error("fill_ranges: 1 <= n <= 160 ranges, 16-byte aligned base");
-        return VPU_ERR_ARG;
-    }
-    FillRanges r;
-    r.n = n;
-    int chunks = 0;
-    for (int i = 0; i < n; ++i) {
-        if (off[i] < 0 || len[i] <= 0 || (off[i] & 3) || (len[i] & 3)) {
-            vpu_set_error("fill_ranges: offsets and lengths must be positive multiples of 4 floats");
-            return VPU_ERR_ARG;
-        }
-        r.first_chunk[i] = chunks;
-        r.off[i] = off[i];
-        r.len[i] = len[i];
-        chunks += (int)((len[i] + FILL_CHUNK - 1) / FILL_CHUNK);
-    }
-    r.first_chunk[n] = chunks;
-    fill_ranges_kernel<<<(unsigned)chunks, 256, 0, ST>>>(base, r, v);
-    return vpu_check_launch("vpu_fill_ranges_f32");
+    if (n < 1) { vpu_clear_stale_error(); vpu_set_error("fill_ranges: 1 <= n <= 160 ranges, 16-byte aligned base"); return VPU_ERR_ARG; }
+    return vpu_fill_ranges2_f32(base, off, len, n, nullptr, nullptr, 0, v, stream);
 }
 extern "C" int vpu_fill_f32(float* p, float v, int64_t n, void* stream) {
     vpu_clear_stale_error();
diff --git a/pvpuformer_amd/engine.py b/pvpuformer_amd/engine.py
--- a/pvpuformer_amd/engine.py
+++ b/pvpuformer_amd/engine.py
@@ -37,11 +37,13 @@
 
 
 class Var:
-    __slots__ = ("t", "g", "gn_stats")
+    __slots__ = ("t", "g", "gn_stats", "resid", "resid_done")
 
     def __init__(self, t):
         self.t = t
         self.g = None
+        self.resid = None
+        self.resid_done = False
         self.gn_stats = None
 
 
@@ -118,6 +120,7 @@
         self.use_side = os.environ.get("VPU_WGRAD_STREAM", "0") == "1"
         self.side = None
         self.fuse_ln_pe = True
+        self.fold_ln_adds = True
         self.group_wgrad = True
         self.ride_wgrad = True
         self.wgrad_fill = 0.8
@@ -133,6 +136,9 @@
         self.wgrad_tn = 256 if self.k4_wgrad else 128
         self.unify_wgrad = True
         self.lazy_zero = True
+        self.zero_arena = True
+        self._arena, self._arena_old = None, []
+        self._arena_clean, self._arena_pos, self._arena_req, self._arena_ask = False, 0, 0, 0
         self.xattn_split = max(1, int(os.environ.get("VPU_XATTN_SPLIT", "1")))
         self.neck_lanes = int(os.environ.get("VPU_NECK_LANES", "0"))
         self._tok_stream = None
@@ -247,12 +253,35 @@
 
     def zero_grad(self, lazy=False):
         self._lazy = set()
+        self._arena_clean, self._arena_pos = False, 0
         if (lazy and self.lazy_zero and self.group_wgrad and self.dt == BF16 and not self.use_side and self.pack_wgrad
                 and self._lazy_ranges is not None):
-            ops.zero_ranges_(self.gflat, self._lazy_ranges)
+            arena = None
+            if self.zero_arena and self._arena_req:
+                if self._arena is None or self._arena.numel() < self._arena_req:
+                    if self._arena is not None:
+                        self._arena_old.append(self._arena)
+                    self._arena = torch.empty(self._arena_req, device=self.dev, dtype=torch.float32)
+                arena, self._arena_clean = self._arena[:self._arena_req], True
+            ops.zero_ranges_(self.gflat, self._lazy_ranges, extra=(arena,))
             self._lazy = set(self._lazy_names)
         else:
             ops.zero_(self.gflat)
+
+    def _zeros(self, numel, dtype):
+        esz = torch.empty((), dtype=dtype).element_size()
+        n32 = _rup(numel * esz, 256) // 4
+        self._arena_ask += n32
+        if self._arena_clean and self._arena_pos + n32 <= self._arena_req and self._arena_pos + n32 <= self._arena.numel():
+            piece = self._arena[self._arena_pos:self._arena_pos + n32]
+            self._arena_pos += n32
+            return piece.view(dtype)[:numel]
+        return ops.zero_(torch.empty(_rup(numel * esz, 4) // esz, device=self.dev, dtype=dtype))[:numel]
+
+    def _arena_finish(self):
+        if self._arena_ask:
+            self._arena_req = self._arena_ask
+        self._arena_clean, self._arena_pos, self._arena_ask = False, 0, 0
 
     def _lazy_plan(self):
         names = [n for n in self.names if n.startswith("backbone.blocks.") and
@@ -350,7 +379,7 @@
                     cs = (self._new(S * ctn * N, dtype=torch.float32), 0)
                     post.append((cs, self.G(bias), S * ctn, N))
                 elif fuse:
-                    cs = (ops.zero_(self._new(S * N, dtype=torch.float32)), 0)
+                    cs = (self._zeros(S * N, torch.float32), 0)
                     post.append((cs, self.G(bias), S, N))
                 args = (dy, x, (slab, 0), N, K, L, ld_dy, ld_x, K, self.dt)
                 kw = dict(transA=True, transB=True, flags=EPI_OUT_F32, colsum=cs, batch=S, sA=(L * ld_dy, 0), sB=(L * ld_x, 0),
@@ -498,11 +527,16 @@
         else:
             ops.gemm(*g_args, **g_kw)
         if self.training:
+            if out is None:
+                y.resid = resid
+
             def bwd():
                 if y.g is None:
                     return
                 dy = (y.g, yoff)
-                if resid is not None:
+                if resid is not None and y.resid_done:
+                    y.resid_done = False
+                elif resid is not None:
                     assert out is None
                     self.acc(resid, y.g, take=True)
                 if act == "relu" and not (pre_masked is not None and pre_masked[0]):
@@ -550,7 +584,7 @@
             self.tape.append(bwd)
         return y
 
-    def layernorm(self, x, prefix, rows, Cdim, eps, pe=None, pe_rows=0, pe_var=None):
+    def layernorm(self, x, prefix, rows, Cdim, eps, pe=None, pe_rows=0, pe_var=None, last_use=False):
         if pe is not None and not self.fuse_ln_pe:
             y = self.layernorm(x, prefix, rows, Cdim, eps)
             return y, self.add_pe(y, pe, rows * Cdim, pe_rows * Cdim, pe_var=pe_var)
@@ -567,16 +601,27 @@
                 dy, dy2 = y.g, (yy.g if yy is not None else None)
                 if dy is None and dy2 is None:
                     return
+                dpe = dacc = None
                 if dy2 is not None and pe_var is not None:
-                    self.acc(pe_var, dy2)
+                    if (self.fold_ln_adds and dy is not None and pe_var.g is not None and pe_rows == rows
+                            and pe_var.g.is_contiguous()):
+                        self._writable(pe_var.g)
+                        dpe = pe_var.g
+                    else:
+                        self.acc(pe_var, dy2)
                 if dy is None:
                     dy, dy2 = dy2, None
+                r = x.resid if (last_use and self.fold_ln_adds) else None
+                if r is not None and r.g is not None and r.g.is_contiguous() and r.g.numel() == rows * Cdim:
+                    self._writable(r.g)
+                    dacc, x.resid_done = r.g, True
                 nblk = ops.layernorm_bwd_nblk(rows)
                 part = self._new(nblk, 2, Cdim, dtype=torch.float32)
                 dres = x.g
                 if x.g is None or x.g.data_ptr() in self._frozen:
                     x.g = torch.empty_like(x.t)
-                ops.layernorm_bwd(dy, x.t, self.Pm(prefix + ".weight"), mean, rstd, dres, x.g, part, rows, Cdim, dy2=dy2)
+                ops.layernorm_bwd(dy, x.t, self.Pm(prefix + ".weight"), mean, rstd, dres, x.g, part, rows, Cdim, dy2=dy2,
+                                  dpe=dpe, dacc=dacc)
                 self._reduce_wb(part, nblk, prefix, Cdim)
             self.tape.append(bwd)
         return y if pe is None else (y, yy)
@@ -955,7 +1000,7 @@
             q = self.mha(p + ".self_attn", q, q, q, B, nq, nq, D)
         else:
             q = self.mha(p + ".self_attn", qq, qq, q, B, nq, nq, D, resid=q)
-        return self.layernorm(q, p + ".norm1", B * nq, D, 1e-5, pe=q0.t, pe_rows=B * nq, pe_var=q0)
+        return self.layernorm(q, p + ".norm1", B * nq, D, 1e-5, pe=q0.t, pe_rows=B * nq, pe_var=q0, last_use=True)
 
     def _neck(self, cx, prompts, xr, kpe_tab):
         B, NT, M, nq, D = cx.B, cx.NT, cx.M, cx.nq, self.D
@@ -970,7 +1015,7 @@
             q = self.mlp(q, p + ".mlp.lin1", p + ".mlp.lin2", B * nq, D, 1024, D, "relu", resid=q)
             q, qq = self.layernorm(q, p + ".norm3", B * nq, D, 1e-5, pe=q0.t, pe_rows=B * nq, pe_var=q0)
             k2 = self.mha(p + ".cross_attn_image_to_token", kk, qq, q, B, NT, nq, D // 2, resid=k)
-            k, kk = self.layernorm(k2, p + ".norm4", M, D, 1e-5, pe=kpe_tab, pe_rows=NT)
+            k, kk = self.layernorm(k2, p + ".norm4", M, D, 1e-5, pe=kpe_tab, pe_rows=NT, last_use=True)
             if l != 2:
                 hs.append((q, k))
         q = self.mha("neck.att.final_attn_token_to_image", qq, kk, k, B, nq, NT, D // 2, resid=q)
@@ -1036,7 +1081,7 @@
             h_tok = self._xrec(T)
             self._xwait(h_tok, None)
             k2 = self._attend(B, i2t, Qi, Ki, Vi, NT, nq, D // 2, k)
-            k, kk = self.layernorm(k2, p + ".norm4", M, D, 1e-5, pe=kpe_tab, pe_rows=NT)
+            k, kk = self.layernorm(k2, p + ".norm4", M, D, 1e-5, pe=kpe_tab, pe_rows=NT, last_use=True)
             if l != 2:
                 hs.append((q, k))
         hs.append((q, k))
@@ -1076,7 +1121,7 @@
                     return
                 if any(v.g is None for i in live for v in hs[i]):
                     pend = [v for i in live for v in hs[i] if v.g is None]
-                    pool = ops.zero_(torch.empty(sum(v.t.numel() for v in pend), device=self.dev, dtype=self.td))
+                    pool = self._zeros(sum(v.t.numel() for v in pend), self.td)
                     o_ = 0
                     for v in pend:
                         v.g = pool[o_:o_ + v.t.numel()].view_as(v.t)
@@ -1456,7 +1501,7 @@
         S = (red + kchunk - 1) // kchunk
         slab = self._new(sum(S * e[0][3] * e[0][4] for e in part), dtype=torch.float32)
         nb = sum(S * e[0][3] for e in part if e[1].get("colsum") is not None)
-        bslab = ops.zero_(torch.empty(max(nb, 1), device=self.dev, dtype=torch.float32))
+        bslab = self._zeros(max(nb, 1), torch.float32)
         sub, jobs, so, bo = [], [], 0, 0
         adv = lambda t, n: (t[0], t[1] + n) if isinstance(t, tuple) else (t, n)
         for args, kw, _, _ in part:
@@ -1490,6 +1535,7 @@
     def abort_pass(self):
         self._wq, self._csq, self._gq = [], [], []
         self._lazy_finish()
+        self._arena_finish()
         self._gq_out, self._frozen = set(), set()
         self._pending_reports, self._reporting = [], False
         self._pack_seen = {}
@@ -1524,6 +1570,7 @@
         self.join_side()
         self.flush_colsums()
         self._lazy_finish()
+        self._arena_finish()
         self._report_ready(final=True)
         if self.grad_ready_hook is not None:
             self.grad_ready_hook(0, self.names["backbone.blocks.0.norm1.weight"][0])
diff --git a/pvpuformer_amd/ops.py b/pvpuformer_amd/ops.py
--- a/pvpuformer_amd/ops.py
+++ b/pvpuformer_amd/ops.py
@@ -133,8 +133,11 @@
     return _lib.load().vpu_layernorm_bwd_nblk(rows)
 
 
-def layernorm_bwd(dy, x, w, mean, rstd, dres, dx, part, rows, Cdim, dy2=None):
-    if dy2 is None:
+def layernorm_bwd(dy, x, w, mean, rstd, dres, dx, part, rows, Cdim, dy2=None, dpe=None, dacc=None):
+    if dpe is not None or dacc is not None:
+        _lib.call("vpu_layernorm_bwd3", ptr(dy), ptr(dy2), ptr(x), ptr(w), ptr(mean), ptr(rstd), ptr(dres), ptr(dx),
+                  ptr(part), ptr(dpe), ptr(dacc), rows, Cdim, code_of(x), _stream())
+    elif dy2 is None:
         _lib.call("vpu_layernorm_bwd", ptr(dy), ptr(x), ptr(w), ptr(mean), ptr(rstd), ptr(dres), ptr(dx), ptr(part), rows,
                   Cdim, code_of(x), _stream())
     else:
@@ -339,13 +342,24 @@
     return t
 
 
-def zero_ranges_(t, ranges):
+def zero_ranges_(t, ranges, extra=()):
     assert t.dtype == torch.float32 and t.is_contiguous()
-    for i in range(0, len(ranges), 160):
-        chunk = ranges[i:i + 160]
-        offs = (C.c_int64 * len(chunk))(*[int(o) for o, _ in chunk])
-        lens = (C.c_int64 * len(chunk))(*[int(n) for _, n in chunk])
-        _lib.call("vpu_fill_ranges_f32", ptr(t), offs, lens, len(chunk), 0.0, _stream())
+    extra = [e for e in extra if e is not None and e.numel()]
+    for e in extra:
+        assert e.dtype == torch.float32 and e.is_contiguous() and e.numel() % 4 == 0 and e.data_ptr() % 16 == 0
+    nx = len(extra)
+    assert nx <= 80
+    for i in range(0, max(len(ranges), 1), 160 - nx):
+        chunk = ranges[i:i + 160 - nx]
+        offs = (C.c_int64 * max(len(chunk), 1))(*[int(o) for o, _ in chunk])
+        lens = (C.c_int64 * max(len(chunk), 1))(*[int(n) for _, n in chunk])
+        if extra:
+            xp = (C.c_void_p * len(extra))(*[e.data_ptr() for e in extra])
+            xl = (C.c_int64 * len(extra))(*[e.numel() for e in extra])
+            _lib.call("vpu_fill_ranges2_f32", ptr(t), offs, lens, len(chunk), xp, xl, len(extra), 0.0, _stream())
+            extra = []
+        elif chunk:
+            _lib.call("vpu_fill_ranges_f32", ptr(t), offs, lens, len(chunk), 0.0, _stream())
     return t
 
 
```

New measurement: 995.1. -1.6%, worse.
